# myshell-ai/OpenVoice

Measured on AMD Instinct MI355X. Metric: real_time_factor, higher is better.
Workload: dtype f32; 1 GPU; ToneColorConverter.convert path, 32 x 10 s @ 22.05 kHz per GPU (T=861 frames), fp32, calibrated random weights; batch_per_gpu=32, global_batch=32, parallelism=dp1 (utterance sharding, RCCL broadcast of src/tgt se)

## Files before the change

include/openvoice_amd.h:

```cpp
#ifndef OPENVOICE_AMD_H
#define OPENVOICE_AMD_H

#include <stddef.h>
#include <stdint.h>

#ifdef __cplusplus
extern "C" {
#endif

typedef void* ov_stream_t;

enum {
  OV_OK = 0,
  OV_E_BADARG = -1,
  OV_E_UNSUPPORTED = -2,
  OV_E_ALIGN = -3,
  OV_E_LAUNCH = -4
};

enum {
  OV_EPI_LINEAR = 0,
  OV_EPI_GATE = 1,
  OV_EPI_RESSKIP = 2,
  OV_EPI_COUPLE = 3,
  OV_EPI_POSTERIOR = 4,
  OV_EPI_CONVT = 5,
  OV_EPI_MAGNITUDE = 6
};

enum {
  OV_F_MASK_V = 1,
  OV_F_OUT2_INIT = 2,
  OV_F_CONVT_GROUPED = 4,
  OV_F_NO_XCD_MAP = 8
};

typedef struct ov_conv1d_params {
  const float* x;
  const float* w;
  const float* bias;
  const float* bias_b;
  float* out;
  const float* res;
  const float* add;
  float* out2;
  const float* mask;
  int64_t x_bstride;
  int64_t out_bstride;
  int64_t res_bstride;
  int64_t add_bstride;
  int64_t out2_bstride;
  int64_t bias_b_bstride;
  int64_t mask_bstride;
  int32_t B, Cin, L;
  int32_t x_ld;
  int32_t out_ld;
  int32_t M;
  int32_t Cout;
  int32_t K, dil;
  int32_t epi, flags, split, phase_s;
  int32_t tiles_per_wg;
  int32_t tile;
  int32_t loaders;
  int32_t chunk;
  float in_slope;
  float scale;
  const int32_t* col_limit;
  int32_t col_limit_scale;
  int32_t reserved0;
} ov_conv1d_params;


size_t ov_conv1d_pack_size(int Cout, int Cin, int K);
int ov_conv1d_pack_rows(int Cout);
int ov_conv1d_pack_f32(const float* w, int Cout, int Cin, int K, float* dst);


int ov_conv1d_f32(const ov_conv1d_params* p, ov_stream_t stream);

typedef struct ov_respair_params {
  const float* x;
  const float* w1;
  const float* b1;
  const float* w2;
  const float* b2;
  float* out;
  const float* add;
  int64_t x_bstride, out_bstride, add_bstride;
  int32_t B, C, L;
  int32_t ld;
  int32_t K, dil;
  int32_t nwg;
  float slope;
  float scale;
  unsigned long long* dbg;
  const int32_t* col_limit;
  int32_t col_limit_scale;
  int32_t reserved0;
} ov_respair_params;
int ov_resblock_pair_f32(const ov_respair_params* p, ov_stream_t stream);
int ov_resblock_pair_supported(int C, int K, int dil);

typedef struct ov_wn_layer_params {
  const float* x;
  float* out;
  float* skip;
  const float* w_in;
  const float* b_in;
  const float* cond;
  const float* w_rs;
  const float* b_rs;
  const float* mask;
  int64_t bstride;
  int64_t cond_bstride;
  int64_t mask_bstride;
  int32_t B, H, T;
  int32_t ld;
  int32_t K;
  int32_t first;
  int32_t last;
  int32_t width;
  int32_t ntile;
  int32_t row_split;
  unsigned long long* dbg;
  float* acts;
} ov_wn_layer_params;
int ov_wn_layer_f32(const ov_wn_layer_params* p, ov_stream_t stream);
int ov_wn_layer_supported(int H, int K);
size_t ov_wn_pack_size(int rows, int cin, int K);
int ov_wn_pack_f32(const float* w, int rows, int cin, int K, float* dst);
int ov_wn_layer_tile(int B, int T, int width);

int ov_wn_layer_wino_f32(const ov_wn_layer_params* p, ov_stream_t stream);
int ov_wn_layer_wino_tile(void);
size_t ov_wn_wino_pack_size(int rows, int cin, int K);
int ov_wn_wino_pack_f32(const float* w, int rows, int cin, int K, float* dst);

int ov_frame_hops_f32(const float* wave, float* hops, int B, int N, int hop, int pad, int U, int ld,
                      ov_stream_t stream);

int ov_frame_hops_windows_f32(const float* wave, int64_t n_samples, const int64_t* first_frame, int W, int hop, int pad,
                              int U, int ld, float* hops, ov_stream_t stream);
int ov_frame_hops_multi_f32(const float* pool, int64_t pool_len, const int64_t* records, int W, int hop, int pad, int U,
                            int ld, float* hops, ov_stream_t stream);
int ov_stitch_window_cores_f32(const float* o_hat, const int64_t* windows, int W, int Tw, int spf, float* out,
                               int64_t out_len, int64_t out_frame0, ov_stream_t stream);
int ov_carry_rows_f32(const int64_t* records, int n_records, const float* src_base, int64_t src_elems, float* dst_base,
                      int64_t dst_elems, ov_stream_t stream);
int ov_rows_f32_to_cl_bf16(const float* src, int64_t src_bs, int src_ld, uint16_t* dst, int B, int C, int L,
                           ov_stream_t stream);
int ov_cl_bf16_to_rows_f32(const uint16_t* src, float* dst, int64_t dst_bs, int dst_ld, int B, int C, int L,
                           ov_stream_t stream);

int ov_vad_frame_energy_f32(const float* pool, int64_t pool_len, const int64_t* records, int R, int H, int ldT,
                            float* energy, ov_stream_t stream);
int ov_vad_segments_i32(const float* energy, const int64_t* records, int R, int H, int ldT, float floor_lin,
                        float range_lin, int min_silence_frames, int min_speech_frames, int pad_frames, int32_t* mask,
                        int64_t* offsets, int64_t* n_active, ov_stream_t stream);
int ov_vad_compact_f32(const float* pool, int64_t pool_len, const int64_t* records, int R, int H, int ldT,
                       const int32_t* mask, const int64_t* offsets, const int64_t* out_bases, float* out,
                       int64_t out_len, ov_stream_t stream);

int ov_join_segments_f32(const float* src, int64_t src_elems, const int64_t* records, int R, float* dst,
                         int64_t dst_elems, int64_t max_span, ov_stream_t stream);

int ov_pack_groups_cl_bf16(const float* src, int64_t src_len, const int64_t* records, int n, int C, uint16_t* dst,
                           int64_t dst_len, ov_stream_t stream);
int ov_unpack_groups_f32(const float* src, int64_t src_len, const int64_t* records, int n, float* dst, int64_t dst_len,
                         ov_stream_t stream);

int ov_normal_philox_f32(const int64_t* records, int R, int C, float* dst, int64_t dst_elems, int64_t max_frames,
                         ov_stream_t stream);

int ov_polyphase_fir_f32(const float* x, const double* h, float* y, int64_t n_in, int64_t n_out, int P, int Q, int taps,
                         ov_stream_t stream);

int ov_polyphase_fir_rows_f32(const int64_t* records, int n_records, const float* src_base, int64_t src_elems,
                              const double* h_base, int64_t h_elems, float* dst_base, int64_t dst_elems, int64_t max_out,
                              ov_stream_t stream);

int ov_conv_post_tanh_f32(const float* x, const float* w, float* out, int B, int C, int L, int K,
                          float in_slope, ov_stream_t stream);
int ov_conv_post_tanh_limited_f32(const float* x, const float* w, float* out, int B, int C, int L, int K,
                                  float in_slope, const int32_t* col_limit, int col_limit_scale, ov_stream_t stream);
int ov_frame_limits_i32(const int64_t* lengths, int32_t* limits, int B, int T, int margin, ov_stream_t stream);

int ov_linear_f32(const float* x, const float* w, const float* bias, float* y, int B, int M, int Kdim,
                  ov_stream_t stream);

int ov_sequence_mask_f32(const int64_t* lengths, float* mask, int B, int T, int ld, ov_stream_t stream);
int ov_unpad_rows_f32(const float* src, float* dst, int rows, int T, int ld, ov_stream_t stream);


int ov_layernorm_freq_f32(const float* x, const float* gamma, const float* beta, float* y, int N, int F, int T,
                          float eps, ov_stream_t stream);

int ov_conv2d_s2_relu_f32(const float* x, const float* w, const float* bias, float* y, int N, int Cin, int Cout,
                          int Fi, int Ti, ov_stream_t stream);

int ov_gru_f32(const float* gi, const float* whh_t, const float* bhh, float* h_out, int N, int H, int T,
               ov_stream_t stream);


int ov_layernorm_freq_ragged_f32(const float* x, const float* gamma, const float* beta, const int32_t* lens, float* y,
                                 int N, int F, int ld, float eps, ov_stream_t stream);

int ov_conv2d_s2_relu_ragged_f32(const float* x, const float* w, const float* bias, const int32_t* lens_in, float* y,
                                 int N, int Cin, int Cout, int Fi, int ld_in, int ld_out, ov_stream_t stream);

int ov_gru_ragged_f32(const float* gi, const float* whh_t, const float* bhh, const int32_t* lens, float* h_out, int N,
                      int H, int ld, ov_stream_t stream);


int ov_embed_f32(const int64_t* tokens, const float* emb, const int64_t* lengths, float* out, int B, int T, int H,
                 int V, int ld, float scale, ov_stream_t stream);

enum {
  OV_LN_PRE_RELU = 1,
  OV_LN_POST_GELU = 2
};
int ov_layernorm_ch_f32(const float* x, const float* res, const float* gamma, const float* beta, const float* res2,
                        const float* mask, float* out, int B, int C, int T, int ld, float eps, int flags,
                        ov_stream_t stream);

int ov_rel_attention_f32(const float* q, const float* k, const float* v, const float* emb_k, const float* emb_v,
                         const float* mask, float* out, int64_t qkv_bstride, int64_t out_bstride, int B, int n_heads,
                         int dk, int T, int ld, int window, ov_stream_t stream);

int ov_dwconv1d_f32(const float* x, const float* w, const float* bias, const float* mask, float* out, int B, int C,
                    int T, int ld, int K, int dil, ov_stream_t stream);

int ov_expand1_f32(const float* x0, int64_t x0_bstride, const float* w, const float* bias, const float* g, float* out,
                   int B, int C, int T, int ld, ov_stream_t stream);

int ov_add_bias_mask_f32(const float* x, const float* bias_b, const float* mask, float* out, int B, int C, int T,
                         int ld, ov_stream_t stream);

int ov_rq_spline_inverse_f32(float* z, int64_t z_bstride, int c0, int c1, const float* h, int64_t h_bstride,
                             const float* mask, int B, int T, int ld, int num_bins, int filter_channels,
                             float tail_bound, ov_stream_t stream);

int ov_duration_f32(const float* z_sdp, int64_t z_bstride, float ea_m, float ea_logs, const float* dp,
                    int64_t dp_bstride, const float* mask, float* logw, int32_t* cum, int64_t* y_len, int B, int T,
                    int ld, float sdp_ratio, float length_scale, ov_stream_t stream);

int ov_expand_prior_f32(const float* m_tok, const float* logs_tok, int64_t tok_bstride, int ldx, const int32_t* cum,
                        const int64_t* x_len, const int64_t* y_len, const float* noise, int64_t noise_bstride, int ldn, float* z_p,
                        float* m_p, float* logs_p, float* attn, int B, int C, int Tx, int Ty, int ldy,
                        float noise_scale, ov_stream_t stream);

typedef struct ov_conv1d_bf16_params {
  const uint16_t* x;
  const uint16_t* w;
  const float* bias;
  uint16_t* out;
  const uint16_t* res;
  const uint16_t* add;
  int32_t B, L, Cin, Cout, K, dil;
  int32_t phase_s;
  int32_t bias_bstride;
  int32_t layout;
  float in_slope;
  float scale;
  float out_slope;
  unsigned long long* dbg;
} ov_conv1d_bf16_params;

size_t ov_conv1d_bf16_pack_size(int Cout, int Cin, int K);
int ov_conv1d_bf16_pack(const float* w, int Cout, int Cin, int K, uint16_t* dst);
int ov_conv1d_bf16cl(const ov_conv1d_bf16_params* p, ov_stream_t stream);
int ov_conv_post_tanh_bf16(const uint16_t* x, const float* w, float* out, int B, int C, int L, int K, float in_slope,
                           ov_stream_t stream);

typedef struct ov_respair_bf16_params {
  const uint16_t* x;
  const uint16_t* w1;
  const float* b1;
  const uint16_t* w2;
  const float* b2;
  uint16_t* out;
  const uint16_t* add;
  int32_t B, L, C, K, dil;
  int32_t nwg;
  float slope, scale;
  unsigned long long* dbg;
} ov_respair_bf16_params;
int ov_resblock_pair_bf16cl(const ov_respair_bf16_params* p, ov_stream_t stream);
int ov_resblock_pair_bf16_supported(int C, int K, int dil);

typedef struct ov_respair2_bf16_params {
  const uint16_t* x;
  const uint16_t* w1;
  const float* b1;
  const uint16_t* w2;
  const float* b2;
  uint16_t* out;
  const uint16_t* add;
  int32_t B, L, C, K, dil;
  int32_t nwg;
  float slope;
  float scale;
  float out_slope;
  int32_t exp_flags;
  unsigned long long* dbg;
} ov_respair2_bf16_params;
int ov_resblock_pair2_bf16cl(const ov_respair2_bf16_params* p, ov_stream_t stream);
int ov_conv1d_bf16_pack16(const float* w, int Cout, int Cin, int K, uint16_t* dst);
int ov_resblock_pair2_bf16_supported(int C, int K, int dil);

typedef struct ov_conv1d_split3_params {
  const uint16_t* x;
  const uint16_t* w;
  const float* bias;
  uint16_t* out;
  const uint16_t* res;
  int64_t x_plane, out_plane, res_plane;
  int32_t B, L, Cin, Cout, K, dil;
  int32_t nwg;
  int32_t products;
  float res_slope;
  float out_slope;
  float scale;
  int32_t col_limit_scale;
  unsigned long long* dbg;
  const int32_t* col_limit;
} ov_conv1d_split3_params;
int ov_conv1d_split3(const ov_conv1d_split3_params* p, ov_stream_t stream);
size_t ov_conv1d_split3_pack_size(int Cout, int Cin, int K);
int ov_conv1d_split3_pack(const float* w, int Cout, int Cin, int K, uint16_t* dst);
int ov_conv1d_split3_supported(int Cin, int Cout, int K, int dil);
int ov_split3_from_f32(const float* x, uint16_t* planes, int64_t plane_stride, int B, int C, int L, float slope,
                       ov_stream_t stream);
int ov_split3_to_f32(const uint16_t* a, const uint16_t* b, const uint16_t* c, int64_t plane_stride, float* out, int B,
                     int C, int L, float in_slope, float scale, ov_stream_t stream);

typedef struct ov_conv1d_wino_params {
  const float* x;
  const float* w;
  const float* bias;
  float* out;
  const float* res;
  const float* add;
  int64_t x_bstride, out_bstride, res_bstride, add_bstride;
  int32_t B, Cin, Cout, L;
  int32_t x_ld, out_ld;
  int32_t K, dil;
  int32_t nwg;
  int32_t frags;
  float in_slope;
  float scale;
  unsigned long long* dbg;
  const int32_t* col_limit;
  int32_t col_limit_scale;
  float out_slope;
} ov_conv1d_wino_params;
int ov_conv1d_wino_f32(const ov_conv1d_wino_params* p, ov_stream_t stream);
int ov_conv1d_wino_supported(int Cin, int Cout, int K, int dil);
int ov_conv1d_wino_chunk(int K, int Cout);
size_t ov_conv1d_wino_pack_size(int Cout, int Cin, int K);
int ov_conv1d_wino_pack_f32(const float* w, int Cout, int Cin, int K, float* dst);

int ov_version(void);
#define OV_ABI_VERSION 212
int ov_build_experiment(void);

#ifdef __cplusplus
}
#endif
#endif
```

openvoice_amd/_lib.py:

```python
import ctypes
import os

_HERE = os.path.dirname(os.path.abspath(__file__))
LIB_PATH = os.environ.get("OPENVOICE_AMD_LIB") or os.path.join(_HERE, "libopenvoice_amd.so")

OV_OK = 0
MIN_VERSION = 212
OV_ERRORS = {-1: "OV_E_BADARG", -2: "OV_E_UNSUPPORTED", -3: "OV_E_ALIGN", -4: "OV_E_LAUNCH"}

EPI_LINEAR, EPI_GATE, EPI_RESSKIP, EPI_COUPLE, EPI_POSTERIOR, EPI_CONVT, EPI_MAGNITUDE = range(7)
F_MASK_V = 1
F_OUT2_INIT = 2
F_CONVT_GROUPED = 4
F_NO_XCD_MAP = 8

_fp = ctypes.c_void_p
_i = ctypes.c_int
_i64 = ctypes.c_int64
LN_PRE_RELU, LN_POST_GELU = 1, 2


class ConvParams(ctypes.Structure):
    _fields_ = [
        ("x", _fp), ("w", _fp), ("bias", _fp), ("bias_b", _fp), ("out", _fp), ("res", _fp),
        ("add", _fp), ("out2", _fp), ("mask", _fp),
        ("x_bstride", ctypes.c_int64), ("out_bstride", ctypes.c_int64), ("res_bstride", ctypes.c_int64),
        ("add_bstride", ctypes.c_int64), ("out2_bstride", ctypes.c_int64), ("bias_b_bstride", ctypes.c_int64),
        ("mask_bstride", ctypes.c_int64),
        ("B", ctypes.c_int32), ("Cin", ctypes.c_int32), ("L", ctypes.c_int32),
        ("x_ld", ctypes.c_int32), ("out_ld", ctypes.c_int32), ("M", ctypes.c_int32),
        ("Cout", ctypes.c_int32), ("K", ctypes.c_int32), ("dil", ctypes.c_int32), ("epi", ctypes.c_int32),
        ("flags", ctypes.c_int32), ("split", ctypes.c_int32), ("phase_s", ctypes.c_int32),
        ("tiles_per_wg", ctypes.c_int32), ("tile", ctypes.c_int32), ("loaders", ctypes.c_int32),
        ("chunk", ctypes.c_int32),
        ("in_slope", ctypes.c_float), ("scale", ctypes.c_float),
        ("col_limit", _fp), ("col_limit_scale", ctypes.c_int32), ("reserved0", ctypes.c_int32),
    ]


class ConvBf16Params(ctypes.Structure):
    _fields_ = [("x", _fp), ("w", _fp), ("bias", _fp), ("out", _fp), ("res", _fp), ("add", _fp),
                ("B", ctypes.c_int32), ("L", ctypes.c_int32), ("Cin", ctypes.c_int32), ("Cout", ctypes.c_int32),
                ("K", ctypes.c_int32), ("dil", ctypes.c_int32), ("phase_s", ctypes.c_int32), ("bias_bstride", ctypes.c_int32), ("layout", ctypes.c_int32),
                ("in_slope", ctypes.c_float), ("scale", ctypes.c_float), ("out_slope", ctypes.c_float), ("dbg", _fp)]


class RespairParams(ctypes.Structure):
    _fields_ = [("x", _fp), ("w1", _fp), ("b1", _fp), ("w2", _fp), ("b2", _fp), ("out", _fp), ("add", _fp),
                ("x_bstride", ctypes.c_int64), ("out_bstride", ctypes.c_int64), ("add_bstride", ctypes.c_int64),
                ("B", ctypes.c_int32), ("C", ctypes.c_int32), ("L", ctypes.c_int32), ("ld", ctypes.c_int32),
                ("K", ctypes.c_int32), ("dil", ctypes.c_int32), ("nwg", ctypes.c_int32),
                ("slope", ctypes.c_float), ("scale", ctypes.c_float), ("dbg", _fp),
                ("col_limit", _fp), ("col_limit_scale", ctypes.c_int32), ("reserved0", ctypes.c_int32)]


class RespairBf16Params(ctypes.Structure):
    _fields_ = [("x", _fp), ("w1", _fp), ("b1", _fp), ("w2", _fp), ("b2", _fp), ("out", _fp), ("add", _fp),
                ("B", ctypes.c_int32), ("L", ctypes.c_int32), ("C", ctypes.c_int32), ("K", ctypes.c_int32),
                ("dil", ctypes.c_int32), ("nwg", ctypes.c_int32), ("slope", ctypes.c_float), ("scale", ctypes.c_float),
                ("dbg", _fp)]


class Respair2Bf16Params(ctypes.Structure):
    _fields_ = [("x", _fp), ("w1", _fp), ("b1", _fp), ("w2", _fp), ("b2", _fp), ("out", _fp), ("add", _fp),
                ("B", ctypes.c_int32), ("L", ctypes.c_int32), ("C", ctypes.c_int32), ("K", ctypes.c_int32),
                ("dil", ctypes.c_int32), ("nwg", ctypes.c_int32), ("slope", ctypes.c_float), ("scale", ctypes.c_float),
                ("out_slope", ctypes.c_float), ("exp_flags", ctypes.c_int32), ("dbg", _fp)]


class ConvSplit3Params(ctypes.Structure):
    _fields_ = [("x", _fp), ("w", _fp), ("bias", _fp), ("out", _fp), ("res", _fp),
                ("x_plane", ctypes.c_int64), ("out_plane", ctypes.c_int64), ("res_plane", ctypes.c_int64),
                ("B", ctypes.c_int32), ("L", ctypes.c_int32), ("Cin", ctypes.c_int32), ("Cout", ctypes.c_int32),
                ("K", ctypes.c_int32), ("dil", ctypes.c_int32), ("nwg", ctypes.c_int32), ("products", ctypes.c_int32),
                ("res_slope", ctypes.c_float), ("out_slope", ctypes.c_float), ("scale", ctypes.c_float),
                ("col_limit_scale", ctypes.c_int32), ("dbg", _fp), ("col_limit", _fp)]


class ConvWinoParams(ctypes.Structure):
    _fields_ = [("x", _fp), ("w", _fp), ("bias", _fp), ("out", _fp), ("res", _fp), ("add", _fp),
                ("x_bstride", ctypes.c_int64), ("out_bstride", ctypes.c_int64), ("res_bstride", ctypes.c_int64),
                ("add_bstride", ctypes.c_int64),
                ("B", ctypes.c_int32), ("Cin", ctypes.c_int32), ("Cout", ctypes.c_int32), ("L", ctypes.c_int32),
                ("x_ld", ctypes.c_int32), ("out_ld", ctypes.c_int32), ("K", ctypes.c_int32), ("dil", ctypes.c_int32),
                ("nwg", ctypes.c_int32), ("frags", ctypes.c_int32),
                ("in_slope", ctypes.c_float), ("scale", ctypes.c_float), ("dbg", _fp),
                ("col_limit", _fp), ("col_limit_scale", ctypes.c_int32), ("out_slope", ctypes.c_float)]


class WnLayerParams(ctypes.Structure):
    _fields_ = [("x", _fp), ("out", _fp), ("skip", _fp), ("w_in", _fp), ("b_in", _fp), ("cond", _fp), ("w_rs", _fp),
                ("b_rs", _fp), ("mask", _fp),
                ("bstride", ctypes.c_int64), ("cond_bstride", ctypes.c_int64), ("mask_bstride", ctypes.c_int64),
                ("B", ctypes.c_int32), ("H", ctypes.c_int32), ("T", ctypes.c_int32), ("ld", ctypes.c_int32),
                ("K", ctypes.c_int32), ("first", ctypes.c_int32), ("last", ctypes.c_int32), ("width", ctypes.c_int32),
                ("ntile", ctypes.c_int32), ("row_split", ctypes.c_int32), ("dbg", _fp), ("acts", _fp)]


SIGNATURES = {
    "ov_version": (ctypes.c_int, []),
    "ov_build_experiment": (ctypes.c_int, []),
    "ov_conv1d_pack_size": (ctypes.c_size_t, [ctypes.c_int, ctypes.c_int, ctypes.c_int]),
    "ov_conv1d_pack_rows": (ctypes.c_int, [ctypes.c_int]),
    "ov_conv1d_pack_f32": (ctypes.c_int, [_fp, ctypes.c_int, ctypes.c_int, ctypes.c_int, _fp]),
    "ov_conv1d_f32": (ctypes.c_int, [ctypes.POINTER(ConvParams), _fp]),
    "ov_resblock_pair_f32": (ctypes.c_int, [ctypes.POINTER(RespairParams), _fp]),
    "ov_resblock_pair_supported": (ctypes.c_int, [_i, _i, _i]),
    "ov_wn_layer_f32": (ctypes.c_int, [ctypes.POINTER(WnLayerParams), _fp]),
    "ov_wn_layer_supported": (ctypes.c_int, [_i, _i]),
    "ov_wn_pack_size": (ctypes.c_size_t, [_i, _i, _i]),
    "ov_wn_pack_f32": (ctypes.c_int, [_fp, _i, _i, _i, _fp]),
    "ov_wn_layer_tile": (ctypes.c_int, [_i, _i, _i]),
    "ov_wn_layer_wino_f32": (ctypes.c_int, [ctypes.POINTER(WnLayerParams), _fp]),
    "ov_wn_layer_wino_tile": (ctypes.c_int, []),
    "ov_wn_wino_pack_size": (ctypes.c_size_t, [_i, _i, _i]),
    "ov_wn_wino_pack_f32": (ctypes.c_int, [_fp, _i, _i, _i, _fp]),
    "ov_conv_post_tanh_f32": (ctypes.c_int, [_fp, _fp, _fp, ctypes.c_int, ctypes.c_int, ctypes.c_int,
                                             ctypes.c_int, ctypes.c_float, _fp]),
    "ov_conv_post_tanh_limited_f32": (ctypes.c_int, [_fp, _fp, _fp, ctypes.c_int, ctypes.c_int, ctypes.c_int,
                                                     ctypes.c_int, ctypes.c_float, _fp, ctypes.c_int, _fp]),
    "ov_frame_limits_i32": (ctypes.c_int, [_fp, _fp, _i, _i, _i, _fp]),
    "ov_linear_f32": (ctypes.c_int, [_fp, _fp, _fp, _fp, ctypes.c_int, ctypes.c_int, ctypes.c_int, _fp]),
    "ov_sequence_mask_f32": (ctypes.c_int, [_fp, _fp, ctypes.c_int, ctypes.c_int, ctypes.c_int, _fp]),
    "ov_unpad_rows_f32": (ctypes.c_int, [_fp, _fp, ctypes.c_int, ctypes.c_int, ctypes.c_int, _fp]),
    "ov_polyphase_fir_f32": (ctypes.c_int, [_fp, _fp, _fp, ctypes.c_int64, ctypes.c_int64, _i, _i, _i, _fp]),
    "ov_polyphase_fir_rows_f32": (ctypes.c_int, [_fp, _i, _fp, _i64, _fp, _i64, _fp, _i64, _i64, _fp]),
    "ov_layernorm_freq_f32": (ctypes.c_int, [_fp, _fp, _fp, _fp, ctypes.c_int, ctypes.c_int, ctypes.c_int,
                                             ctypes.c_float, _fp]),
    "ov_conv2d_s2_relu_f32": (ctypes.c_int, [_fp, _fp, _fp, _fp, ctypes.c_int, ctypes.c_int, ctypes.c_int,
                                             ctypes.c_int, ctypes.c_int, _fp]),
    "ov_gru_f32": (ctypes.c_int, [_fp, _fp, _fp, _fp, ctypes.c_int, ctypes.c_int, ctypes.c_int, _fp]),
    "ov_layernorm_freq_ragged_f32": (ctypes.c_int, [_fp, _fp, _fp, _fp, _fp, _i, _i, _i, ctypes.c_float, _fp]),
    "ov_conv2d_s2_relu_ragged_f32": (ctypes.c_int, [_fp, _fp, _fp, _fp, _fp, _i, _i, _i, _i, _i, _i, _fp]),
    "ov_gru_ragged_f32": (ctypes.c_int, [_fp, _fp, _fp, _fp, _fp, _i, _i, _i, _fp]),
    "ov_conv1d_bf16_pack_size": (ctypes.c_size_t, [_i, _i, _i]),
    "ov_conv1d_bf16_pack": (ctypes.c_int, [_fp, _i, _i, _i, _fp]),
    "ov_conv1d_bf16_pack16": (ctypes.c_int, [_fp, _i, _i, _i, _fp]),
    "ov_conv1d_bf16cl": (ctypes.c_int, [ctypes.POINTER(ConvBf16Params), _fp]),
    "ov_resblock_pair_bf16cl": (ctypes.c_int, [ctypes.POINTER(RespairBf16Params), _fp]),
    "ov_resblock_pair_bf16_supported": (ctypes.c_int, [_i, _i, _i]),
    "ov_resblock_pair2_bf16cl": (ctypes.c_int, [ctypes.POINTER(Respair2Bf16Params), _fp]),
    "ov_resblock_pair2_bf16_supported": (ctypes.c_int, [_i, _i, _i]),
    "ov_conv_post_tanh_bf16": (ctypes.c_int, [_fp, _fp, _fp, _i, _i, _i, _i, ctypes.c_float, _fp]),
    "ov_conv1d_split3": (ctypes.c_int, [ctypes.POINTER(ConvSplit3Params), _fp]),
    "ov_conv1d_split3_pack_size": (ctypes.c_size_t, [_i, _i, _i]),
    "ov_conv1d_split3_pack": (ctypes.c_int, [_fp, _i, _i, _i, _fp]),
    "ov_conv1d_split3_supported": (ctypes.c_int, [_i, _i, _i, _i]),
    "ov_split3_from_f32": (ctypes.c_int, [_fp, _fp, _i64, _i, _i, _i, ctypes.c_float, _fp]),
    "ov_split3_to_f32": (ctypes.c_int, [_fp, _fp, _fp, _i64, _fp, _i, _i, _i, ctypes.c_float, ctypes.c_float, _fp]),
    "ov_conv1d_wino_f32": (ctypes.c_int, [ctypes.POINTER(ConvWinoParams), _fp]),
    "ov_conv1d_wino_supported": (ctypes.c_int, [_i, _i, _i, _i]),
    "ov_conv1d_wino_chunk": (ctypes.c_int, [_i, _i]),
    "ov_conv1d_wino_pack_size": (ctypes.c_size_t, [_i, _i, _i]),
    "ov_conv1d_wino_pack_f32": (ctypes.c_int, [_fp, _i, _i, _i, _fp]),
    "ov_frame_hops_f32": (ctypes.c_int, [_fp, _fp, _i, _i, _i, _i, _i, _i, _fp]),
    "ov_frame_hops_windows_f32": (ctypes.c_int, [_fp, _i64, _fp, _i, _i, _i, _i, _i, _fp, _fp]),
    "ov_frame_hops_multi_f32": (ctypes.c_int, [_fp, _i64, _fp, _i, _i, _i, _i, _i, _fp, _fp]),
    "ov_stitch_window_cores_f32": (ctypes.c_int, [_fp, _fp, _i, _i, _i, _fp, _i64, _i64, _fp]),
    "ov_carry_rows_f32": (ctypes.c_int, [_fp, _i, _fp, _i64, _fp, _i64, _fp]),
    "ov_rows_f32_to_cl_bf16": (ctypes.c_int, [_fp, _i64, _i, _fp, _i, _i, _i, _fp]),
    "ov_cl_bf16_to_rows_f32": (ctypes.c_int, [_fp, _fp, _i64, _i, _i, _i, _i, _fp]),
    "ov_vad_frame_energy_f32": (ctypes.c_int, [_fp, _i64, _fp, _i, _i, _i, _fp, _fp]),
    "ov_vad_segments_i32": (ctypes.c_int, [_fp, _fp, _i, _i, _i, ctypes.c_float, ctypes.c_float, _i, _i, _i, _fp, _fp, _fp,
                                           _fp]),
    "ov_vad_compact_f32": (ctypes.c_int, [_fp, _i64, _fp, _i, _i, _i, _fp, _fp, _fp, _fp, _i64, _fp]),
    "ov_join_segments_f32": (ctypes.c_int, [_fp, _i64, _fp, _i, _fp, _i64, _i64, _fp]),
    "ov_pack_groups_cl_bf16": (ctypes.c_int, [_fp, _i64, _fp, _i, _i, _fp, _i64, _fp]),
    "ov_unpack_groups_f32": (ctypes.c_int, [_fp, _i64, _fp, _i, _fp, _i64, _fp]),
    "ov_normal_philox_f32": (ctypes.c_int, [_fp, _i, _i, _fp, _i64, _i64, _fp]),
    "ov_embed_f32": (ctypes.c_int, [_fp, _fp, _fp, _fp, _i, _i, _i, _i, _i, ctypes.c_float, _fp]),
    "ov_layernorm_ch_f32": (ctypes.c_int, [_fp, _fp, _fp, _fp, _fp, _fp, _fp, _i, _i, _i, _i, ctypes.c_float, _i, _fp]),
    "ov_rel_attention_f32": (ctypes.c_int, [_fp, _fp, _fp, _fp, _fp, _fp, _fp, _i64, _i64, _i, _i, _i, _i, _i, _i,
                                            _fp]),
    "ov_add_bias_mask_f32": (ctypes.c_int, [_fp, _fp, _fp, _fp, _i, _i, _i, _i, _fp]),
    "ov_dwconv1d_f32": (ctypes.c_int, [_fp, _fp, _fp, _fp, _fp, _i, _i, _i, _i, _i, _i, _fp]),
    "ov_expand1_f32": (ctypes.c_int, [_fp, _i64, _fp, _fp, _fp, _fp, _i, _i, _i, _i, _fp]),
    "ov_rq_spline_inverse_f32": (ctypes.c_int, [_fp, _i64, _i, _i, _fp, _i64, _fp, _i, _i, _i, _i, _i,
                                                ctypes.c_float, _fp]),
    "ov_duration_f32": (ctypes.c_int, [_fp, _i64, ctypes.c_float, ctypes.c_float, _fp, _i64, _fp, _fp, _fp, _fp,
                                       _i, _i, _i, ctypes.c_float, ctypes.c_float, _fp]),
    "ov_expand_prior_f32": (ctypes.c_int, [_fp, _fp, _i64, _i, _fp, _fp, _fp, _fp, _i64, _i, _fp, _fp, _fp, _fp,
                                           _i, _i, _i, _i, _i, ctypes.c_float, _fp]),
}

_lib = None


class OvError(RuntimeError):
    pass


GENERATORS = ("fp32", "bf16")


def check_generator(generator, optional=False):
    if generator is None and optional:
        return None
    if not isinstance(generator, str) or generator not in GENERATORS:
        raise OvError(f"generator must be 'fp32' or 'bf16'{' (or None)' if optional else ''}, got {generator!r}")
    return generator


def generator_kw(generator):
    return {} if generator is None else {"generator": generator}


def load():
    global _lib
    if _lib is None:
        if not os.path.exists(LIB_PATH):
            raise OvError(f"{LIB_PATH} not found: build the HIP extension first "
                          f"(python -c 'import __graft_entry__ as g; g.build()'); there is no CPU fallback")
        lib = ctypes.CDLL(LIB_PATH)
        lib.ov_version.restype, lib.ov_version.argtypes = ctypes.c_int, []
        if lib.ov_version() < MIN_VERSION:
            raise OvError(f"{LIB_PATH} is version {lib.ov_version()}, this package needs >= {MIN_VERSION}: rebuild it "
                          f"(make -C openvoice_amd/csrc)")
        for name, (restype, argtypes) in SIGNATURES.items():
            try:
                fn = getattr(lib, name)
            except AttributeError:
                raise OvError(f"{LIB_PATH} lacks {name}: it was built from older source, rebuild it "
                              f"(make -C openvoice_amd/csrc)") from None
            fn.restype = restype
            fn.argtypes = argtypes
        exp = lib.ov_build_experiment()
        if exp != 0 and os.environ.get("OPENVOICE_AMD_ALLOW_EXPERIMENT") != "1":
            raise OvError(f"{LIB_PATH} is a measurement build (OV_EXP={exp}: kernels with loads / barriers compiled "
                          f"out, results meaningless); rebuild with `make -C openvoice_amd/csrc clean all`")
        _lib = lib
    return _lib


def torch_op(name, *args):
    try:
        return getattr(torch_ops(), name)(*args)
    except RuntimeError as exc:
        if isinstance(exc, OvError):
            raise
        raise OvError(str(exc).split("\n")[0]) from None


def check(code, what):
    if code != OV_OK:
        raise OvError(f"{what} failed: {OV_ERRORS.get(code, code)}")


SHIM_PATH = os.path.join(_HERE, "libopenvoice_amd_torch.so")
_ops = None
VALUE_FUNCS = {"ov_version", "ov_build_experiment", "ov_conv1d_pack_size", "ov_conv1d_pack_rows", "ov_wn_pack_size",
               "ov_conv1d_bf16_pack_size", "ov_resblock_pair_supported", "ov_wn_layer_supported", "ov_wn_layer_tile",
               "ov_resblock_pair_bf16_supported", "ov_resblock_pair2_bf16_supported", "ov_conv1d_split3_pack_size",
               "ov_conv1d_split3_supported", "ov_conv1d_wino_supported", "ov_conv1d_wino_chunk", "ov_conv1d_wino_pack_size",
               "ov_wn_layer_wino_tile", "ov_wn_wino_pack_size"}


def binding():
    b = os.environ.get("OPENVOICE_AMD_BINDING", "ctypes" if os.environ.get("OPENVOICE_AMD_LIB") else "torch")
    if b not in ("torch", "ctypes"):
        raise OvError(f"OPENVOICE_AMD_BINDING={b!r}: expected 'torch' or 'ctypes'")
    return b


def use_torch_binding():
    return binding() == "torch"


def torch_ops():
    global _ops
    if _ops is None:
        import torch
        for path in (LIB_PATH, SHIM_PATH):
            if not os.path.exists(path):
                raise OvError(f"{path} not found: build the HIP extension first (python -c 'import __graft_entry__ "
                              f"as g; g.build()'); there is no CPU fallback (OPENVOICE_AMD_BINDING=ctypes needs only "
                              f"libopenvoice_amd.so)")
        torch.ops.load_library(SHIM_PATH)
        ops = torch.ops.openvoice_amd
        if ops.version() < MIN_VERSION:
            raise OvError(f"{LIB_PATH} is version {ops.version()}, this package needs >= {MIN_VERSION}: rebuild it "
                          f"(make -C openvoice_amd/csrc)")
        exp = ops.build_experiment()
        if exp != 0 and os.environ.get("OPENVOICE_AMD_ALLOW_EXPERIMENT") != "1":
            raise OvError(f"{LIB_PATH} is a measurement build (OV_EXP={exp}); rebuild with "
                          f"`make -C openvoice_amd/csrc clean all`")
        _ops = ops
    return _ops


def _flat_view(t, off):
    start = t.storage_offset() + off
    n = t.untyped_storage().nbytes() // t.element_size() - start
    return t.as_strided((n,), (1,), start)


def call(name, *args):
    if use_torch_binding():
        targs = [_flat_view(*a) if type(a) is tuple else a for a in args]
        try:
            return getattr(torch_ops(), name[3:])(*targs)
        except RuntimeError as exc:
            if isinstance(exc, OvError):
                raise
            raise OvError(str(exc).split("\n")[0]) from None
    import torch
    lib = load()
    fn = getattr(lib, name)
    cargs, dev = [], None
    for a in args:
        off = 0
        if type(a) is tuple:
            a, off = a
        if isinstance(a, torch.Tensor):
            if dev is None and a.is_cuda:
                dev = a.device
            a = ctypes.c_void_p(a.data_ptr() + off * a.element_size())
        cargs.append(a)
    if len(fn.argtypes) == len(cargs) + 1:
        if dev is None:
            raise OvError(f"{name}: no device tensor among the arguments")
        cargs.append(ctypes.c_void_p(torch.cuda.current_stream(dev).cuda_stream))
    rc = fn(*cargs)
    if name in VALUE_FUNCS:
        return rc
    check(rc, name)
```

openvoice_amd/csrc/conv1d_wino.h:

```cpp
#pragma once
#include <hip/hip_runtime.h>

#include <atomic>
#include <type_traits>

#include "conv1d_mfma.h"
#include "openvoice_amd.h"

namespace ovkw {

using ovk::f32x16;
using ovk::f32x2;
using ovk::f32x4;

__device__ __forceinline__ uint32_t lds_addr(const void* ptr) {
  return (uint32_t)(uintptr_t)(const __attribute__((address_space(3))) void*)ptr;
}

__device__ __forceinline__ void lds_barrier() { asm volatile("s_waitcnt lgkmcnt(0)\n\ts_barrier" ::: "memory"); }

template <int OFF>
__device__ __forceinline__ void lds_write_b32(uint32_t addr, float v) {
  static_assert(OFF >= 0 && OFF < 65536, "DS immediate offset");
  asm volatile("ds_write_b32 %0, %1 offset:%2" ::"v"(addr), "v"(v), "n"(OFF) : "memory");
}
template <int O0, int O1>
__device__ __forceinline__ void lds_write2st64_b32(uint32_t addr, float a, float b) {
  static_assert(O0 >= 0 && O0 < 256 && O1 >= 0 && O1 < 256, "DS write2st64 offsets are 8-bit, in units of 64 dwords");
  asm volatile("ds_write2st64_b32 %0, %1, %2 offset0:%3 offset1:%4" ::"v"(addr), "v"(a), "v"(b), "n"(O0), "n"(O1) : "memory");
}
template <int I, int N, class F>
__device__ __forceinline__ void static_for(F&& f) {
  if constexpr (I < N) {
    f(std::integral_constant<int, I>{});
    static_for<I + 1, N>(f);
  }
}

constexpr int REC = 256;

constexpr int wino_lead(int K) { return K == 7 ? 1 : 0; }
constexpr int wino_trail(int K) { return (K + 2) / 3 * 3 - K - wino_lead(K); }
constexpr bool wino_zero_product(int K, int g, int pt) {
  return (pt == 0 && g == 0 && wino_lead(K) >= 1) || (pt == 5 && g == (K + 2) / 3 - 1 && wino_trail(K) >= 1);
}
constexpr int wino_products(int K) {
  int n = 0;
  for (int g = 0; g < (K + 2) / 3; ++g)
    for (int pt = 0; pt < 6; ++pt) n += wino_zero_product(K, g, pt) ? 0 : 1;
  return n;
}
static_assert(wino_products(3) == 6 && wino_products(7) == 16 && wino_products(11) == 23, "executed products per tile");
constexpr int MAX_COUT = 512;

template <int K, int DIL, int NF>
struct GeoD {
  static constexpr int G = (K + 2) / 3;
  static constexpr int NT = 32 * NF;
  static constexpr int J = NT / DIL;
  static constexpr int NCOL = 4 * J * DIL;
  static constexpr int PADD = ((K - 1) / 2 + wino_lead(K)) * DIL;
  static constexpr int PADA = (PADD + 3) / 4 * 4;
  static constexpr int NV = 3 * (G - 1) + 6;
  static constexpr int RW = (PADA - PADD + DIL - 1 + DIL * (4 * (J - 1) + NV - 1) + 1 + 3) / 4 * 4;
  static_assert(DIL == 3 || DIL == 5, "dilated instances: 3 and 5");
};

template <int K>
struct Geo {
  static constexpr int G = (K + 2) / 3;
  static constexpr int PAD = (K - 1) / 2 + wino_lead(K);
  static constexpr int OFF0 = 8 - PAD;
  static constexpr int WSTART = OFF0 / 4 * 4;
  static constexpr int WLEN = OFF0 - WSTART + 3 * (G - 1) + 6;
  static constexpr int NB128 = (WLEN + 3) / 4;
  static_assert(PAD <= 8 && WSTART + 4 * NB128 <= 20, "input window exceeds the raw row (128 NF + 16 floats)");
};

__host__ __device__ inline size_t wino_pack_floats(int Cout, int Cin, int K, int CI) {
  const int G = (K + 2) / 3;
  return ((size_t)(Cout / 32) * (Cin / CI) * (CI * G / 4) * 3 + 3) * REC;
}

#ifndef OVW_EXP
#define OVW_EXP 0
#endif
#define OVW_MARK(q)                                                \
  if constexpr (DBG) {                                             \
    const unsigned long long now_ = __builtin_readcyclecounter(); \
    tph[q] += now_ - tlast;                                        \
    tlast = now_;                                                  \
  }

template <int K, int DIL, int CI, int NF, int MW, bool DBG>
__global__ __launch_bounds__(64 * (4 + 2 * NF), NF == 1 ? 3 : 2) void conv1d_wino_kernel(const ov_conv1d_wino_params p) {
  using Ge = Geo<K>;
  using Gd = GeoD<K, DIL == 1 ? 3 : DIL, NF>;
  constexpr int G = Ge::G, KR = CI * G, NSTEP = KR / 2, NPAIR = NSTEP / 2;
  constexpr int NB = 4 / MW;
  constexpr int NTS = 32 * NF;
  constexpr int NT = NTS * NB;
  constexpr int NCOLS = DIL == 1 ? 4 * NTS : Gd::NCOL;
  constexpr int NCOL = NCOLS * NB;
  constexpr int RW = (DIL == 1 ? NCOLS + 16 : Gd::RW) + (NB - 1) * NCOLS;
  static_assert(MW == 4 || ((MW == 2 || MW == 1) && NF == 2), "two- and one-row-fragment workgroups run two fragments per wave");
  constexpr int ORG = DIL == 1 ? 8 : Gd::PADA;
  constexpr int RW4 = RW / 4;
  constexpr int NHELP = 2 * NF;
  static_assert(DIL == 1 || NF == 2, "dilated instances run two fragments per wave");
  static_assert(KR % 4 == 0 && CI % 2 == 0, "k-rows in whole k-step pairs");
  constexpr int NPR = CI / 2;
  constexpr int NITEM = NPR * RW4;
  constexpr int RAWBUF = CI * RW;
  constexpr int VBUF = KR * NT * 6;
  __shared__ __attribute__((aligned(16))) float raw[2 * RAWBUF];
  __shared__ __attribute__((aligned(16))) float Vs[2 * VBUF];
  __shared__ __attribute__((aligned(16))) float bias_s[MAX_COUT];
  constexpr int OST = 256;
  __shared__ __attribute__((aligned(16))) float ostage[DIL == 1 ? 4 : 4 * 8 * OST];

  const int tid = threadIdx.x;
  const int lane = tid & 63;
  const int wave = __builtin_amdgcn_readfirstlane(tid >> 6);
  const int L = p.L;
  const int nchunks = p.Cin / CI;
  const int ntiles = (L + NCOL - 1) / NCOL;
  const int mblocks = p.Cout / (32 * MW);
  int total = ntiles * mblocks * p.B;
  __shared__ int lim_pref[ovk::LIMIT_MAX_BATCH + 1];
  const bool limited = p.col_limit != nullptr;
  if (limited) {
    if (wave == 0) {
      int carry = 0;
      for (int base = 0; base < p.B; base += 64) {
        const int bb = base + lane;
        int nb = 0;
        if (bb < p.B) {
          long long c = (long long)p.col_limit[bb] * p.col_limit_scale;
          c = c < 0 ? 0 : (c > L ? L : c);
          nb = ((int)c + NCOL - 1) / NCOL;
        }
        int sc = nb;
#pragma unroll
        for (int d = 1; d < 64; d <<= 1) {
          const int v = __shfl_up(sc, d, 64);
          if (lane >= d) sc += v;
        }
        if (bb < p.B) lim_pref[bb + 1] = carry + sc;
        carry += __shfl(sc, 63, 64);
      }
      if (lane == 0) lim_pref[0] = 0;
    }
    __syncthreads();
    total = __builtin_amdgcn_readfirstlane(lim_pref[p.B]) * mblocks;
  }
  auto decode = [&](int w, int& ub, int& utile, int& umblk) {
    const int g = w / mblocks;
    umblk = w - g * mblocks;
    if (!limited) {
      ub = g / ntiles;
      utile = g - ub * ntiles;
      return;
    }
    int lo = 0, hi = p.B;
    while (hi - lo > 1) {
      const int mid = (lo + hi) >> 1;
      if (__builtin_amdgcn_readfirstlane(lim_pref[mid]) <= g) lo = mid; else hi = mid;
    }
    ub = lo;
    utile = g - __builtin_amdgcn_readfirstlane(lim_pref[lo]);
  };
  int wid0 = blockIdx.x, wend = total, wstride = gridDim.x;
  if ((gridDim.x & 7u) == 0) {
    const int xcd = blockIdx.x & 7;
    const int lo = (int)(((long long)xcd * total) >> 3);
    wend = (int)(((long long)(xcd + 1) * total) >> 3);
    wid0 = lo + (int)(blockIdx.x >> 3);
    wstride = gridDim.x >> 3;
  }
  if (wid0 >= wend) return;
  const int nitems = (wend - wid0 + wstride - 1) / wstride;
  const int nstream = nitems * nchunks;
  for (int i = tid; i < p.Cout; i += 64 * (4 + NHELP)) bias_s[i] = p.bias[i];

  const bool is_helper = wave >= 4;
  if (is_helper) {
    __builtin_amdgcn_s_setprio(3);
    const float slope = p.in_slope;
    const uint32_t ldx = (uint32_t)p.x_ld;
    const int hl = (wave - 4) * 64 + lane;
    constexpr int NLOAD = (NITEM + 64 * NHELP - 1) / (64 * NHELP);
    f32x4 sa[2][NLOAD], sb[2][NLOAD];
    uint32_t sbyte[NLOAD];
    int scol[NLOAD];
    uint32_t hasbits = 0, okbits[2] = {0, 0};
    bool edge[2] = {false, false};
#pragma unroll
    for (int i = 0; i < NLOAD; ++i) {
      const int idx = i * (64 * NHELP) + hl;
      const int pr = idx / RW4, c4 = idx - pr * RW4;
      const bool has = idx < NITEM;
      hasbits |= (has ? 1u : 0u) << i;
      scol[i] = 4 * c4;
      sbyte[i] = has ? 4u * (2u * (uint32_t)pr * ldx + 4u * (uint32_t)c4) : 0u;
    }
    const uint32_t raw_lds = lds_addr(raw) + 32u * (uint32_t)hl;
    const uint32_t v_lds = lds_addr(Vs);
    int lwid = wid0, lchunk = 0, lpos = 0;
    int lb, ltile, lmblk;
    decode(lwid, lb, ltile, lmblk);

    auto issue_loads = [&](auto setc) {
      constexpr int S = decltype(setc)::value;
      const bool live = lpos < nstream;
      const int tb = ltile * NCOL - ORG;
      const float* __restrict__ xrow = p.x + (int64_t)lb * p.x_bstride + (int64_t)(lchunk * CI) * ldx;
      edge[S] = !(live && tb >= 0 && tb + RW <= L);
      if (!edge[S]) {
        const char* b0 = reinterpret_cast<const char*>(xrow + tb);
        const char* b1 = reinterpret_cast<const char*>(xrow + tb + ldx);
#pragma unroll
        for (int i = 0; i < NLOAD; ++i) {
          sa[S][i] = *reinterpret_cast<const f32x4*>(b0 + sbyte[i]);
          sb[S][i] = *reinterpret_cast<const f32x4*>(b1 + sbyte[i]);
        }
      } else {
        const char* b0 = reinterpret_cast<const char*>(xrow);
        const char* b1 = reinterpret_cast<const char*>(xrow + ldx);
        uint32_t okb = 0;
#pragma unroll
        for (int i = 0; i < NLOAD; ++i) {
          const int t = tb + scol[i];
          const bool ok = live && ((hasbits >> i) & 1u) && t >= 0 && t < L;
          const uint32_t off = ok ? sbyte[i] + 4u * (uint32_t)tb : 0u;
          okb |= (ok ? 1u : 0u) << i;
          sa[S][i] = *reinterpret_cast<const f32x4*>(b0 + off);
          sb[S][i] = *reinterpret_cast<const f32x4*>(b1 + off);
        }
        okbits[S] = okb;
      }
      ++lpos;
      if (++lchunk == nchunks) {
        lchunk = 0;
        lwid += wstride;
        if (lwid < wend) decode(lwid, lb, ltile, lmblk);
      }
    };
    auto act2 = [&](f32x2 v) {
      const f32x2 sv = v * f32x2{slope, slope};
      f32x2 r;
      asm("v_max_f32 %0, %1, %2" : "=v"(r[0]) : "v"(v[0]), "v"(sv[0]));
      asm("v_max_f32 %0, %1, %2" : "=v"(r[1]) : "v"(v[1]), "v"(sv[1]));
      return r;
    };
    auto write_raw = [&](int buf, auto setc) {
      constexpr int S = decltype(setc)::value;
      const uint32_t base = raw_lds + (uint32_t)buf * (RAWBUF * 4);
#pragma unroll
      for (int i = 0; i < NLOAD; ++i) {
        if ((hasbits >> i) & 1u) {
          f32x2 a01 = {sa[S][i][0], sa[S][i][1]}, a23 = {sa[S][i][2], sa[S][i][3]};
          f32x2 b01 = {sb[S][i][0], sb[S][i][1]}, b23 = {sb[S][i][2], sb[S][i][3]};
          if (slope != 1.f) {
            a01 = act2(a01); a23 = act2(a23); b01 = act2(b01); b23 = act2(b23);
          }
          if (edge[S] && !((okbits[S] >> i) & 1u)) a01 = a23 = b01 = b23 = f32x2{0.f, 0.f};
          const uint32_t ad = base + (uint32_t)i * (64 * NHELP * 32);
          asm volatile("ds_write2_b32 %0, %1, %2 offset1:1" ::"v"(ad), "v"(a01[0]), "v"(b01[0]) : "memory");
          asm volatile("ds_write2_b32 %0, %1, %2 offset0:2 offset1:3" ::"v"(ad), "v"(a01[1]), "v"(b01[1]) : "memory");
          asm volatile("ds_write2_b32 %0, %1, %2 offset0:4 offset1:5" ::"v"(ad), "v"(a23[0]), "v"(b23[0]) : "memory");
          asm volatile("ds_write2_b32 %0, %1, %2 offset0:6 offset1:7" ::"v"(ad), "v"(a23[1]), "v"(b23[1]) : "memory");
        }
      }
    };
    constexpr int ROUNDS = NPR * NT / (64 * NHELP);
    static_assert(NPR * NT % (64 * NHELP) == 0, "whole rounds of helper lanes");
    uint32_t tsrc[ROUNDS], vadr[2][ROUNDS][6];
    static_assert((NT * 24) % 256 == 0 && (CI * NT * 24) % 256 == 0, "channel / group record distances in 256-byte units");
#pragma unroll
    for (int r = 0; r < ROUNDS; ++r) {
      const int idx = r * (64 * NHELP) + hl;
      const int tile = idx & (NT - 1), pr = idx / NT;
      if constexpr (DIL == 1) {
        tsrc[r] = 8u * (uint32_t)(pr * RW + Ge::WSTART + 4 * tile);
      } else {
        const int sub = tile / NTS, tl = tile - sub * NTS;
        const int rc0 = tl / Gd::J, rc = rc0 < DIL ? rc0 : 0, jt = rc0 < DIL ? tl - rc0 * Gd::J : 0;
        tsrc[r] = 8u * (uint32_t)(pr * RW + (Gd::PADA - Gd::PADD) + sub * NCOLS + rc + 4 * DIL * jt);
      }
#pragma unroll
      for (int bf = 0; bf < 2; ++bf)
#pragma unroll
        for (int q = 0; q < 6; ++q) vadr[bf][r][q] = v_lds + (uint32_t)bf * (VBUF * 4) + 24u * (uint32_t)(2 * pr * NT + tile) + 4u * q;
    }
    auto transform = [&](auto bufc) {
      constexpr int buf = decltype(bufc)::value;
      const char* src = reinterpret_cast<const char*>(raw) + buf * (RAWBUF * 4);
#pragma unroll
      for (int r = 0; r < ROUNDS; ++r) {
        constexpr int NWIN = DIL == 1 ? 4 * Ge::NB128 : Gd::NV;
        f32x2 win[NWIN];
        if constexpr (DIL == 1) {
#pragma unroll
          for (int q = 0; q < 2 * Ge::NB128; ++q) {
            const f32x4 v = *reinterpret_cast<const f32x4*>(src + tsrc[r] + 16 * q);
            win[2 * q] = f32x2{v[0], v[1]};
            win[2 * q + 1] = f32x2{v[2], v[3]};
          }
        } else {
#pragma unroll
          for (int u = 0; u < Gd::NV; ++u) win[u] = *reinterpret_cast<const f32x2*>(src + tsrc[r] + 8 * DIL * u);
        }
        static_for<0, G>([&](auto gc) {
          constexpr int g = decltype(gc)::value;
          constexpr int o = (DIL == 1 ? Ge::OFF0 - Ge::WSTART : 0) + 3 * g;
          const f32x2 d0 = win[o], d1 = win[o + 1], d2 = win[o + 2], d3 = win[o + 3], d4 = win[o + 4], d5 = win[o + 5];
          const f32x2 c4 = {4.f, 4.f}, m4 = {-4.f, -4.f}, m5 = {-5.f, -5.f}, c2 = {2.f, 2.f}, m2 = {-2.f, -2.f};
          const f32x2 t1 = __builtin_elementwise_fma(m4, d2, d4), t2 = __builtin_elementwise_fma(m4, d1, d3);
          const f32x2 t3 = d4 - d2, t4 = d3 - d1;
          constexpr bool Z0 = wino_zero_product(K, g, 0), Z5 = wino_zero_product(K, g, 5);
          const f32x2 v1 = t1 + t2;
          const f32x2 v2 = t1 - t2;
          const f32x2 v3 = __builtin_elementwise_fma(c2, t4, t3);
          const f32x2 v4 = __builtin_elementwise_fma(m2, t4, t3);
          constexpr int OA = g * CI * NT * 24 / 256, OB = OA + NT * 24 / 256;
          constexpr int bf = buf;
          if constexpr (!Z0) {
            const f32x2 v0 = __builtin_elementwise_fma(c4, d0, __builtin_elementwise_fma(m5, d2, d4));
            lds_write2st64_b32<OA, OB>(vadr[bf][r][0], v0[0], v0[1]);
          }
          lds_write2st64_b32<OA, OB>(vadr[bf][r][1], v1[0], v1[1]);
          lds_write2st64_b32<OA, OB>(vadr[bf][r][2], v2[0], v2[1]);
          lds_write2st64_b32<OA, OB>(vadr[bf][r][3], v3[0], v3[1]);
          lds_write2st64_b32<OA, OB>(vadr[bf][r][4], v4[0], v4[1]);
          if constexpr (!Z5) {
            const f32x2 v5 = __builtin_elementwise_fma(c4, d1, __builtin_elementwise_fma(m5, d3, d5));
            lds_write2st64_b32<OA, OB>(vadr[bf][r][5], v5[0], v5[1]);
          }
        });
      }
    };
    auto hand_over = [&]() { lds_barrier(); };

    unsigned long long tph[8] = {0, 0, 0, 0, 0, 0, 0, 0};
    unsigned long long tlast = DBG ? __builtin_readcyclecounter() : 0ull;
    using S0 = std::integral_constant<int, 0>;
    using S1 = std::integral_constant<int, 1>;
    issue_loads(S0{});
    write_raw(0, S0{});
    issue_loads(S1{});
    hand_over();
    transform(std::integral_constant<int, 0>{});
    write_raw(1, S1{});
    issue_loads(S0{});
    hand_over();
    OVW_MARK(4)
    auto period = [&](int i, auto par) {
      constexpr int P = decltype(par)::value;
      if (OVW_EXP < 6) issue_loads(std::integral_constant<int, 1 - P>{});
      OVW_MARK(0)
      if (OVW_EXP != 2 && OVW_EXP < 6 && i + 1 < nstream) transform(std::integral_constant<int, 1 - P>{});
      OVW_MARK(1)
      if (OVW_EXP < 6) write_raw(P, par);
      OVW_MARK(2)
      if (OVW_EXP < 7) hand_over();
      OVW_MARK(3)
    };
    for (int i = 0; i < nstream; i += 2) {
      period(i, S0{});
      if (i + 1 < nstream) period(i + 1, S1{});
    }
    if constexpr (DBG) {
      if (lane == 0) {
        unsigned long long* d = p.dbg + ((size_t)blockIdx.x * 8 + wave) * 8;
        tph[7] = (unsigned long long)nstream;
#pragma unroll
        for (int q = 0; q < 8; ++q) d[q] = tph[q];
      }
    }
    return;
  }

  const int half = lane >> 5, n = lane & 31;
  const f32x4* __restrict__ wbase = reinterpret_cast<const f32x4*>(p.w);
  const uint32_t LD = (uint32_t)p.out_ld;
  int wid = wid0, b, tile, mblk;
  decode(wid, b, tile, mblk);
  const int wrow = MW == 4 ? wave : (MW == 2 ? (wave & 1) : 0), wsub = MW == 4 ? 0 : (MW == 2 ? (wave >> 1) : wave);
  int mtile = mblk * MW + wrow;
  uint32_t rec = (uint32_t)mtile * (uint32_t)nchunks * (uint32_t)(NPAIR * 3);
  f32x4 a_cur[3], a_nxt[3];
#pragma unroll
  for (int j = 0; j < 3; ++j) a_cur[j] = wbase[(size_t)(rec + j) * 64 + lane];
  const int voffB = (half * NT + wsub * NTS + n) * 6;

  __syncthreads();
  __syncthreads();
  unsigned long long tph[8] = {0, 0, 0, 0, 0, 0, 0, 0};
  unsigned long long tlast = DBG ? __builtin_readcyclecounter() : 0ull;
  int it = 0;
  while (true) {
    f32x16 acc[6][NF];
#pragma unroll
    for (int q = 0; q < 6; ++q)
#pragma unroll
      for (int f = 0; f < NF; ++f)
#pragma unroll
        for (int r = 0; r < 16; ++r) acc[q][f][r] = 0.f;
#pragma unroll
    for (int i = 0; i < 4; ++i) {
      const f32x4 bq = *reinterpret_cast<const f32x4*>(bias_s + mtile * 32 + 4 * half + 8 * i);
#pragma unroll
      for (int f = 0; f < NF; ++f) {
        acc[1][f][4 * i] = bq[0]; acc[1][f][4 * i + 1] = bq[1]; acc[1][f][4 * i + 2] = bq[2]; acc[1][f][4 * i + 3] = bq[3];
      }
    }

    OVW_MARK(3)
    f32x2 bq[NF][3];
#pragma unroll
    for (int f = 0; f < NF; ++f)
#pragma unroll
      for (int qq = 0; qq < 3; ++qq) bq[f][qq] = *reinterpret_cast<const f32x2*>(Vs + (it & 1) * VBUF + voffB + f * (32 * 6) + 2 * qq);
    for (int chunk = 0; chunk < nchunks; ++chunk, ++it) {
      const float* vb = Vs + (it & 1) * VBUF + voffB;
      const float* vbn = Vs + ((it + 1) & 1) * VBUF + voffB;
      const bool more_chunks = chunk + 1 < nchunks;
#pragma unroll
      for (int s = 0; s < NSTEP; ++s) {
        const int s2 = s & 1;
        if (s == NSTEP - 1) {
          OVW_MARK(0)
          if (OVW_EXP < 7) lds_barrier();
          OVW_MARK(1)
        }
        if (s2 == 0) {
          rec += 3;
#pragma unroll
          for (int j = 0; j < 3; ++j) a_nxt[j] = (OVW_EXP == 3 || OVW_EXP == 8) ? a_cur[j] : wbase[(size_t)(rec + j) * 64 + lane];
        }
#pragma unroll
        for (int qq = 0; qq < 3; ++qq) {
          __builtin_amdgcn_sched_barrier(0);
#pragma unroll
          for (int t = 0; t < 2; ++t) {
            const int q = 2 * qq + t, e = s2 * 6 + q;
            if (wino_zero_product(K, 2 * s / CI, q)) continue;
#pragma unroll
            for (int f = 0; f < NF; ++f) {
#if OVW_EXP == 1
              acc[q][f][0] += a_cur[e >> 2][e & 3] * bq[f][qq][t];
#else
              acc[q][f] = __builtin_amdgcn_mfma_f32_32x32x2f32(a_cur[e >> 2][e & 3], bq[f][qq][t], acc[q][f], 0, 0, 0);
#endif
            }
          }
          __builtin_amdgcn_sched_barrier(0);
          if (OVW_EXP != 5 && OVW_EXP != 8 && (s + 1 < NSTEP || more_chunks)) {
#pragma unroll
            for (int f = 0; f < NF; ++f)
              bq[f][qq] = *reinterpret_cast<const f32x2*>((s + 1 < NSTEP ? vb + (s + 1) * (2 * NT * 6) : vbn) + f * (32 * 6) + 2 * qq);
          }
        }
        if (s2 == 1) {
#pragma unroll
          for (int j = 0; j < 3; ++j) a_cur[j] = a_nxt[j];
        }
      }
    }

    const int nwid = wid + wstride;
    const bool more = nwid < wend;
    int nb = 0, ntile = 0, nmblk = 0;
    if (more) decode(nwid, nb, ntile, nmblk);
    const int nmtile = nmblk * MW + wrow;
    const int ob = b, otile = tile, omtile = mtile;
    if (more) {
      rec = (uint32_t)nmtile * (uint32_t)nchunks * (uint32_t)(NPAIR * 3);
#pragma unroll
      for (int j = 0; j < 3; ++j) a_cur[j] = wbase[(size_t)(rec + j) * 64 + lane];
      wid = nwid; b = nb; tile = ntile; mblk = nmblk; mtile = nmtile;
    }

    {
      const float scale = p.scale;
      const float oslope = p.out_slope;
      const bool act_out = oslope < 1.f;
      float* outb = p.out + (int64_t)ob * p.out_bstride;
      const float* resb = p.res ? p.res + (int64_t)ob * p.res_bstride : nullptr;
      const float* addb = p.add ? p.add + (int64_t)ob * p.add_bstride : nullptr;
      const uint32_t rbase = (uint32_t)omtile * 32u + 4u * (uint32_t)half;
      auto at4 = [&](int f, int r) {
        const float y0 = acc[0][f][r], y1 = acc[1][f][r], y2 = acc[2][f][r], y3 = acc[3][f][r], y4 = acc[4][f][r],
                    y5 = acc[5][f][r];
        const float s1 = y1 + y2, d1 = y1 - y2, s2 = y3 + y4, d2 = y3 - y4;
        f32x4 o;
        o[0] = (y0 + s1) + s2;
        o[1] = __builtin_fmaf(2.f, d2, d1);
        o[2] = __builtin_fmaf(4.f, s2, s1);
        o[3] = __builtin_fmaf(8.f, d2, d1) + y5;
        return o;
      };
      if constexpr (DIL == 1) {
        auto run = [&](auto has_res, auto has_add) {
          constexpr bool HR = decltype(has_res)::value, HA = decltype(has_add)::value;
          constexpr int NGRP = 16 * NF;
          uint32_t voff[NF];
          bool colok[NF];
#pragma unroll
          for (int f = 0; f < NF; ++f) {
            const uint32_t col = (uint32_t)otile * NCOL + (uint32_t)(wsub * NCOLS) + 128u * f + 4u * (uint32_t)n;
            colok[f] = col < (uint32_t)L;
            voff[f] = 4u * (uint32_t)half * LD + (colok[f] ? col : 0u);
          }
          const size_t mrow = (size_t)omtile * 32u;
          constexpr int DEPTH = (HR && HA) ? 4 : 8;
          f32x4 rv[HR ? DEPTH : 1], av[HA ? DEPTH : 1];
          auto load = [&](int g) {
            const int f = g / 16, r = g % 16;
            const size_t rowb = (mrow + (size_t)((r & 3) + 8 * (r >> 2))) * LD;
            if constexpr (HR) rv[g % DEPTH] = *reinterpret_cast<const f32x4*>(resb + rowb + voff[f]);
            if constexpr (HA) av[g % DEPTH] = *reinterpret_cast<const f32x4*>(addb + rowb + voff[f]);
          };
          if constexpr (HR || HA) {
#pragma unroll
            for (int g = 0; g < DEPTH - 1; ++g) load(g);
          }
#pragma unroll
          for (int g = 0; g < NGRP; ++g) {
            if constexpr (HR || HA) {
              if (g + DEPTH - 1 < NGRP) load(g + DEPTH - 1);
            }
            const int f = g / 16, r = g % 16;
            f32x4 o = at4(f, r);
            if constexpr (HR) o += rv[g % DEPTH];
            if constexpr (HA) o += av[g % DEPTH];
            o *= scale;
            if constexpr (!HR && !HA) {
              if (act_out) {
#pragma unroll
                for (int e = 0; e < 4; ++e) o[e] = ovk::lrelu(o[e], oslope);
              }
            }
            if (colok[f] && (OVW_EXP != 4 || o[0] == 12345.f))
              *reinterpret_cast<f32x4*>(outb + (mrow + (size_t)((r & 3) + 8 * (r >> 2))) * LD + voff[f]) = o;
          }
        };
        using T = std::true_type;
        using F = std::false_type;
        if (resb && addb) run(T{}, T{});
        else if (resb) run(T{}, F{});
        else if (addb) run(F{}, T{});
        else run(F{}, F{});
      } else {
        float* ost = ostage + wave * (8 * OST);
        const uint32_t c0 = (uint32_t)otile * NCOL + (uint32_t)(wsub * NCOLS);
        int cbase[NF];
#pragma unroll
        for (int f = 0; f < NF; ++f) {
          const int tl = 32 * f + n, rc0 = tl / Gd::J;
          cbase[f] = rc0 < DIL ? rc0 + 4 * DIL * (tl - rc0 * Gd::J) : -1;
        }
        const uint32_t col = c0 + 4u * (uint32_t)lane;
        const bool colok = 4 * lane < NCOLS && col < (uint32_t)L;
        const uint32_t ccol = colok ? col : 0u;
        auto run = [&](auto has_res, auto has_add) {
          constexpr bool HR = decltype(has_res)::value, HA = decltype(has_add)::value;
          constexpr int DEPTH = (HR && HA) ? 2 : 3;
          f32x4 rv[HR ? DEPTH : 1][2], av[HA ? DEPTH : 1][2];
          auto row0 = [&](int g) { return (uint32_t)omtile * 32u + 8u * (g / 4) + 2u * (g % 4); };
          auto load = [&](int g) {
#pragma unroll
            for (int j = 0; j < 2; ++j) {
              if constexpr (HR) rv[g % DEPTH][j] = *reinterpret_cast<const f32x4*>(resb + (size_t)(row0(g) + j) * LD + ccol);
              if constexpr (HA) av[g % DEPTH][j] = *reinterpret_cast<const f32x4*>(addb + (size_t)(row0(g) + j) * LD + ccol);
            }
          };
          if constexpr (HR || HA) {
#pragma unroll
            for (int g = 0; g < DEPTH - 1; ++g) load(g);
          }
#pragma unroll
          for (int rg = 0; rg < 4; ++rg) {
#pragma unroll
            for (int j = 0; j < 4; ++j)
#pragma unroll
              for (int f = 0; f < NF; ++f) {
                const f32x4 o = at4(f, 4 * rg + j);
                if (cbase[f] >= 0) {
                  float* od = ost + (4 * half + j) * OST + cbase[f];
                  od[0] = o[0]; od[DIL] = o[1]; od[2 * DIL] = o[2]; od[3 * DIL] = o[3];
                }
              }
#pragma unroll
            for (int q = 0; q < 4; ++q) {
              const int g = 4 * rg + q;
              if constexpr (HR || HA) {
                if (g + DEPTH - 1 < 16) load(g + DEPTH - 1);
              }
#pragma unroll
              for (int j = 0; j < 2; ++j) {
                f32x4 o = *reinterpret_cast<const f32x4*>(ost + (2 * q + j) * OST + 4 * lane);
                if constexpr (HR) o += rv[g % DEPTH][j];
                if constexpr (HA) o += av[g % DEPTH][j];
                o *= scale;
                if constexpr (!HR && !HA) {
                  if (act_out) {
#pragma unroll
                    for (int e = 0; e < 4; ++e) o[e] = ovk::lrelu(o[e], oslope);
                  }
                }
                if (colok) *reinterpret_cast<f32x4*>(outb + (size_t)(row0(g) + j) * LD + col) = o;
              }
            }
          }
        };
        using T = std::true_type;
        using F = std::false_type;
        if (resb && addb) run(T{}, T{});
        else if (resb) run(T{}, F{});
        else if (addb) run(F{}, T{});
        else run(F{}, F{});
      }
    }
    OVW_MARK(2)
    if (!more) break;
  }
  if constexpr (DBG) {
    if (lane == 0) {
      unsigned long long* d = p.dbg + ((size_t)blockIdx.x * 8 + wave) * 8;
      tph[7] = (unsigned long long)it;
#pragma unroll
      for (int q = 0; q < 8; ++q) d[q] = tph[q];
    }
  }
}

template <int K, int DIL, int CI, int NF, int MW, bool DBG>
int wino_launch(const ov_conv1d_wino_params* p, hipStream_t stream) {
  constexpr int NCOL = (DIL == 1 ? 128 * NF : GeoD<K, DIL == 1 ? 3 : DIL, NF>::NCOL) * (4 / MW), NHELP = 2 * NF;
  const int ntiles = (p->L + NCOL - 1) / NCOL;
  const long total = (long)ntiles * (p->Cout / (32 * MW)) * p->B;
  auto kernel = conv1d_wino_kernel<K, DIL, CI, NF, MW, DBG>;
  static std::atomic<int> slot_cache[ovk::OV_MAX_DEVICES];
  const int slots = ovk::resident_workgroups(reinterpret_cast<const void*>(kernel), 64 * (4 + NHELP), slot_cache);
  long nwg = p->nwg > 0 ? p->nwg : slots;
  if (nwg > total) nwg = total;
  if (nwg >= 8) nwg = (nwg + 7) / 8 * 8;
  hipLaunchKernelGGL(kernel, dim3((unsigned)nwg), dim3(64 * (4 + NHELP)), 0, stream, *p);
  return hipGetLastError() == hipSuccess ? OV_OK : OV_E_LAUNCH;
}

constexpr int wino_ci(int K, int mw = 4) {
  return mw == 1 ? (K == 11 ? 2 : 0) : K == 3 ? (mw == 4 ? 16 : 8) : (K == 7 || K == 11) ? (mw == 4 ? 8 : 4) : 0;
}
constexpr int wino_mw(int Cout) { return Cout % 128 == 0 ? 4 : (Cout % 64 == 0 ? 2 : (Cout % 32 == 0 ? 1 : 0)); }

int wino_dispatch_k3(const ov_conv1d_wino_params* p, int nf, hipStream_t stream);
int wino_dispatch_k7(const ov_conv1d_wino_params* p, int nf, hipStream_t stream);
int wino_dispatch_k11(const ov_conv1d_wino_params* p, int nf, hipStream_t stream);

#define OVW_DISPATCH_MW(KK, MWV)                                                                                        \
  {                                                                                                                      \
    constexpr int CI = ovkw::wino_ci(KK, MWV);                                                                           \
    if constexpr (MWV == 4) {                                                                                            \
      if (p->dil == 1 && nf == 1)                                                                                        \
        return dbg ? wino_launch<KK, 1, CI, 1, 4, true>(p, st) : wino_launch<KK, 1, CI, 1, 4, false>(p, st);              \
    }                                                                                                                    \
    if (p->dil == 1) return dbg ? wino_launch<KK, 1, CI, 2, MWV, true>(p, st) : wino_launch<KK, 1, CI, 2, MWV, false>(p, st); \
    if (p->dil == 3) return dbg ? wino_launch<KK, 3, CI, 2, MWV, true>(p, st) : wino_launch<KK, 3, CI, 2, MWV, false>(p, st); \
    if (p->dil == 5) return dbg ? wino_launch<KK, 5, CI, 2, MWV, true>(p, st) : wino_launch<KK, 5, CI, 2, MWV, false>(p, st); \
    return OV_E_UNSUPPORTED;                                                                                             \
  }
#define OVW_DEFINE_DISPATCH(KK)                                                                                          \
  int ovkw::wino_dispatch_k##KK(const ov_conv1d_wino_params* p, int nf, hipStream_t st) {                                \
    const bool dbg = p->dbg != nullptr;                                                                                  \
    if (ovkw::wino_mw(p->Cout) == 4) OVW_DISPATCH_MW(KK, 4)                                                              \
    if (nf != 2) return OV_E_UNSUPPORTED;                                                                                \
    if (ovkw::wino_mw(p->Cout) == 2) OVW_DISPATCH_MW(KK, 2)                                                              \
    if constexpr (ovkw::wino_ci(KK, 1) != 0) OVW_DISPATCH_MW(KK, 1)                                                      \
    return OV_E_UNSUPPORTED;                                                                                             \
  }

}
```

openvoice_amd/csrc/conv1d_wino.hip:

```cpp
#include "conv1d_wino.h"

#include <cstring>

using namespace ovkw;

namespace {

const double kG[6][3] = {{1.0 / 4, 0, 0},           {-1.0 / 6, -1.0 / 6, -1.0 / 6}, {-1.0 / 6, 1.0 / 6, -1.0 / 6},
                         {1.0 / 24, 1.0 / 12, 1.0 / 6}, {1.0 / 24, -1.0 / 12, 1.0 / 6},  {0, 0, 1}};

}

extern "C" {

int ov_conv1d_wino_chunk(int K, int Cout) { return Cout > 0 && wino_mw(Cout) ? wino_ci(K, wino_mw(Cout)) : 0; }

int ov_conv1d_wino_supported(int Cin, int Cout, int K, int dil) {
  const int ci = ov_conv1d_wino_chunk(K, Cout);
  if (ci == 0 || (dil != 1 && dil != 3 && dil != 5)) return 0;
  return (Cin > 0 && Cin % ci == 0 && Cout <= MAX_COUT) ? 1 : 0;
}

size_t ov_conv1d_wino_pack_size(int Cout, int Cin, int K) {
  const int ci = ov_conv1d_wino_chunk(K, Cout);
  if (ci == 0 || Cin <= 0 || Cin % ci != 0) return 0;
  return wino_pack_floats(Cout, Cin, K, ci);
}

int ov_conv1d_wino_pack_f32(const float* w, int Cout, int Cin, int K, float* dst) {
  const size_t nfl = ov_conv1d_wino_pack_size(Cout, Cin, K);
  if (!w || !dst || nfl == 0) return OV_E_BADARG;
  const int CI = ov_conv1d_wino_chunk(K, Cout), G = (K + 2) / 3, KR = CI * G, NPAIR = KR / 4, nchunks = Cin / CI;
  std::memset(dst, 0, nfl * sizeof(float));
  for (int mt = 0; mt < Cout / 32; ++mt)
    for (int c = 0; c < nchunks; ++c)
      for (int sp = 0; sp < NPAIR; ++sp)
        for (int lane = 0; lane < 64; ++lane)
          for (int e = 0; e < 12; ++e) {
            const int kstep = 2 * sp + e / 6, pt = e % 6;
            const int kk = 2 * kstep + (lane >> 5);
            const int g = kk / CI, ci = c * CI + kk % CI;
            const int co = 32 * mt + (lane & 31);
            double u = 0.0;
            for (int k = 0; k < 3; ++k) {
              const int tap = 3 * g + k - wino_lead(K);
              if (tap >= 0 && tap < K) u += kG[pt][k] * (double)w[((size_t)co * Cin + ci) * K + tap];
            }
            const size_t sub = (((size_t)mt * nchunks + c) * NPAIR + sp) * 3 + e / 4;
            dst[sub * REC + (size_t)lane * 4 + e % 4] = (float)u;
          }
  return OV_OK;
}

int ov_conv1d_wino_f32(const ov_conv1d_wino_params* pin, ov_stream_t stream) {
  if (!pin) return OV_E_BADARG;
  ov_conv1d_wino_params q = *pin;
  if (!q.x || !q.w || !q.bias || !q.out) return OV_E_BADARG;
  if (q.B <= 0 || q.L <= 0 || q.nwg < 0) return OV_E_BADARG;
  if (q.col_limit && (q.col_limit_scale <= 0 || (reinterpret_cast<uintptr_t>(q.col_limit) & 3))) return OV_E_BADARG;
  if (q.col_limit && q.B > ovk::LIMIT_MAX_BATCH) q.col_limit = nullptr;
  if (q.x_ld == 0) q.x_ld = q.L;
  if (q.out_ld == 0) q.out_ld = q.L;
  if (q.x_ld < q.L || q.out_ld < q.L) return OV_E_BADARG;
  if (!ov_conv1d_wino_supported(q.Cin, q.Cout, q.K, q.dil)) return OV_E_UNSUPPORTED;
  if (!(q.in_slope > 0.f && q.in_slope <= 1.f)) return OV_E_UNSUPPORTED;
  if (q.out_slope == 0.f) q.out_slope = 1.f;
  if (!(q.out_slope > 0.f && q.out_slope <= 1.f)) return OV_E_UNSUPPORTED;
  if (q.out_slope != 1.f && (q.res || q.add)) return OV_E_UNSUPPORTED;
  if (q.out == q.x) return OV_E_BADARG;
  auto mis = [](const void* ptr) { return (reinterpret_cast<uintptr_t>(ptr) & 15) != 0; };
  if (mis(q.x) || mis(q.w) || mis(q.out) || (q.res && mis(q.res)) || (q.add && mis(q.add)) || (q.L & 3) || (q.x_ld & 3) ||
      (q.out_ld & 3) || (q.x_bstride & 3) || (q.out_bstride & 3) || (q.res && (q.res_bstride & 3)) ||
      (q.add && (q.add_bstride & 3)))
    return OV_E_ALIGN;
  if ((int64_t)q.Cin * q.x_ld >= (1LL << 31) || (int64_t)q.Cout * q.out_ld >= (1LL << 31)) return OV_E_BADARG;
  if ((int64_t)ov_conv1d_wino_chunk(q.K, q.Cout) * q.x_ld >= (1LL << 30)) return OV_E_BADARG;
  if (q.B > 1 && (q.x_bstride < (int64_t)q.Cin * q.x_ld || q.out_bstride < (int64_t)q.Cout * q.out_ld ||
                  (q.res && q.res_bstride < (int64_t)q.Cout * q.out_ld) || (q.add && q.add_bstride < (int64_t)q.Cout * q.out_ld)))
    return OV_E_BADARG;
  hipStream_t st = static_cast<hipStream_t>(stream);
  if (q.frags < 0 || q.frags > 2) return OV_E_BADARG;
  const int nf = q.frags ? q.frags : 2;
  if (q.dil != 1 && nf != 2) return OV_E_UNSUPPORTED;
  switch (q.K) {
    case 3: return wino_dispatch_k3(&q, nf, st);
    case 7: return wino_dispatch_k7(&q, nf, st);
    case 11: return wino_dispatch_k11(&q, nf, st);
  }
  return OV_E_UNSUPPORTED;
}

}
```

openvoice_amd/csrc/torch_shim.cpp:

```cpp
#include <ATen/ATen.h>
#include <ATen/hip/impl/HIPGuardImplMasqueradingAsCUDA.h>
#include <c10/hip/HIPStream.h>
#include <torch/library.h>

#include <string>
#include <type_traits>

#include "openvoice_amd.h"

namespace {

const char* ov_strerror(int rc) {
  switch (rc) {
    case OV_E_BADARG: return "OV_E_BADARG";
    case OV_E_UNSUPPORTED: return "OV_E_UNSUPPORTED";
    case OV_E_ALIGN: return "OV_E_ALIGN";
    case OV_E_LAUNCH: return "OV_E_LAUNCH";
    default: return "unknown error";
  }
}

using OptTensor = c10::optional<at::Tensor>;

struct Ctx {
  const char* name;
  bool host;
  bool have_dev = false;
  c10::Device dev{c10::kCPU};
  void see(const at::Tensor& t, int index) {
    if (host) {
      TORCH_CHECK(t.device().is_cpu(), name, ": argument ", index, " must be a HOST (CPU) tensor");
      return;
    }
    TORCH_CHECK(t.is_cuda(), name, ": argument ", index, " must be on a ROCm device (there is no CPU path)");
    if (!have_dev) { dev = t.device(); have_dev = true; }
    TORCH_CHECK(t.device() == dev, name, ": argument ", index, " is on ", t.device(), ", expected ", dev);
  }
  ov_stream_t stream() const {
    TORCH_CHECK(have_dev, name, ": no device tensor among the arguments");
    return static_cast<ov_stream_t>(c10::hip::getCurrentHIPStream(dev.index()).stream());
  }
};

struct DeviceScope {
  c10::hip::OptionalHIPGuardMasqueradingAsCUDA guard;
  explicit DeviceScope(const Ctx& c) { if (c.have_dev) guard.set_device(c.dev); }
};

template <typename E> bool dtype_ok(at::ScalarType s);
template <> bool dtype_ok<float>(at::ScalarType s) { return s == at::kFloat; }
template <> bool dtype_ok<double>(at::ScalarType s) { return s == at::kDouble; }
template <> bool dtype_ok<int64_t>(at::ScalarType s) { return s == at::kLong; }
template <> bool dtype_ok<int32_t>(at::ScalarType s) { return s == at::kInt; }
template <> bool dtype_ok<uint16_t>(at::ScalarType s) { return s == at::kBFloat16 || s == at::kShort || s == at::kUInt16; }
template <> bool dtype_ok<unsigned long long>(at::ScalarType s) { return s == at::kLong || s == at::kUInt64; }
template <typename E> const char* dtype_name();
template <> const char* dtype_name<float>() { return "float32"; }
template <> const char* dtype_name<double>() { return "float64"; }
template <> const char* dtype_name<int64_t>() { return "int64"; }
template <> const char* dtype_name<int32_t>() { return "int32"; }
template <> const char* dtype_name<uint16_t>() { return "bfloat16 (or int16 bit patterns)"; }
template <> const char* dtype_name<unsigned long long>() { return "int64 (tick counters)"; }

template <typename E> E* tensor_ptr(const OptTensor& t, Ctx& c, int index) {
  if (!t.has_value() || !t->defined()) return nullptr;
  c.see(*t, index);
  TORCH_CHECK(dtype_ok<E>(t->scalar_type()), c.name, ": argument ", index, " must be ", dtype_name<E>(), ", got ",
              t->scalar_type());
  return static_cast<E*>(t->data_ptr());
}

template <typename C, typename = void> struct Arg;
template <typename E> struct Arg<const E*> {
  using torch_t = const OptTensor&;
  static std::string schema(int i) { return "Tensor? a" + std::to_string(i); }
  static const E* get(const OptTensor& t, Ctx& c, int i) { return tensor_ptr<E>(t, c, i); }
};
template <typename E> struct Arg<E*, std::enable_if_t<!std::is_const<E>::value>> {
  using torch_t = const OptTensor&;
  static std::string schema(int i) { return "Tensor(a" + std::to_string(i) + "!)? a" + std::to_string(i); }
  static E* get(const OptTensor& t, Ctx& c, int i) { return tensor_ptr<E>(t, c, i); }
};
template <> struct Arg<int> {
  using torch_t = int64_t;
  static std::string schema(int i) { return "int a" + std::to_string(i); }
  static int get(int64_t v, Ctx& c, int i) {
    TORCH_CHECK(v >= INT32_MIN && v <= INT32_MAX, c.name, ": argument ", i, " does not fit a 32-bit int");
    return static_cast<int>(v);
  }
};
template <> struct Arg<int64_t> {
  using torch_t = int64_t;
  static std::string schema(int i) { return "int a" + std::to_string(i); }
  static int64_t get(int64_t v, Ctx&, int) { return v; }
};
template <> struct Arg<float> {
  using torch_t = double;
  static std::string schema(int i) { return "float a" + std::to_string(i); }
  static float get(double v, Ctx&, int) { return static_cast<float>(v); }
};

template <typename... T> struct List {};
template <typename L, typename... Acc> struct DropLast;
template <typename T, typename... Acc> struct DropLast<List<T>, Acc...> { using type = List<Acc...>; using last = T; };
template <typename T, typename U, typename... R, typename... Acc>
struct DropLast<List<T, U, R...>, Acc...> : DropLast<List<U, R...>, Acc..., T> {};

template <typename... C> std::string schema_of(const char* name, bool returns_int) {
  std::string s = std::string(name) + "(";
  int i = 0;
  bool first = true;
  ((s += (first ? "" : ", ") + Arg<C>::schema(i++), first = false), ...);
  return s + (returns_int ? ") -> int" : ") -> ()");
}

template <int Kind, typename R, typename L> struct Wrap;
template <typename R, typename... C> struct Wrap<0, R, List<C...>> {
  template <R (*Fn)(C..., ov_stream_t)> struct On {
    static inline const char* name = "";
    static void call(typename Arg<C>::torch_t... a) {
      Ctx c{name, false};
      int i = 0;
      std::tuple<C...> v{Arg<C>::get(a, c, i++)...};
      DeviceScope scope(c);
      const int rc = std::apply([&](C... x) { return Fn(x..., c.stream()); }, v);
      TORCH_CHECK(rc == OV_OK, "ov_", name, " failed: ", ov_strerror(rc));
    }
    static void def(torch::Library& m, const char* n) { name = n; m.def(schema_of<C...>(n, false).c_str(), &call); }
  };
};
template <typename R, typename... C> struct Wrap<1, R, List<C...>> {
  template <R (*Fn)(C...)> struct On {
    static inline const char* name = "";
    static void call(typename Arg<C>::torch_t... a) {
      Ctx c{name, true};
      int i = 0;
      std::tuple<C...> v{Arg<C>::get(a, c, i++)...};
      const int rc = std::apply(Fn, v);
      TORCH_CHECK(rc == OV_OK, "ov_", name, " failed: ", ov_strerror(rc));
    }
    static void def(torch::Library& m, const char* n) { name = n; m.def(schema_of<C...>(n, false).c_str(), &call); }
  };
};
template <typename R, typename... C> struct Wrap<2, R, List<C...>> {
  template <R (*Fn)(C...)> struct On {
    static inline const char* name = "";
    static int64_t call(typename Arg<C>::torch_t... a) {
      Ctx c{name, true};
      int i = 0;
      std::tuple<C...> v{Arg<C>::get(a, c, i++)...};
      return static_cast<int64_t>(std::apply(Fn, v));
    }
    static void def(torch::Library& m, const char* n) { name = n; m.def(schema_of<C...>(n, true).c_str(), &call); }
  };
};

template <typename F> struct Sig;
template <typename R, typename... C> struct Sig<R (*)(C...)> { using ret = R; using args = List<C...>; };

template <auto Fn> void bind_device(torch::Library& m, const char* name) {
  using S = Sig<decltype(Fn)>;
  using D = DropLast<typename S::args>;
  static_assert(std::is_same<typename D::last, ov_stream_t>::value, "device entry points end with the stream");
  Wrap<0, typename S::ret, typename D::type>::template On<Fn>::def(m, name);
}
template <auto Fn> void bind_host(torch::Library& m, const char* name) {
  using S = Sig<decltype(Fn)>;
  Wrap<1, typename S::ret, typename S::args>::template On<Fn>::def(m, name);
}
template <auto Fn> void bind_value(torch::Library& m, const char* name) {
  using S = Sig<decltype(Fn)>;
  Wrap<2, typename S::ret, typename S::args>::template On<Fn>::def(m, name);
}

template <typename E> E* sptr(const OptTensor& t, Ctx& c, int index, int64_t off = 0) {
  E* p = tensor_ptr<E>(t, c, index);
  return p ? p + off : nullptr;
}
void finish(int rc, const char* what) { TORCH_CHECK(rc == OV_OK, what, " failed: ", ov_strerror(rc)); }

void conv1d_f32(const OptTensor& x, const OptTensor& w, const OptTensor& bias, const OptTensor& out, const OptTensor& res,
                const OptTensor& add, const OptTensor& out2, const OptTensor& mask, const OptTensor& bias_b,
                const OptTensor& col_limit, at::IntArrayRef ip, at::ArrayRef<double> fp) {
  TORCH_CHECK(ip.size() == 29 && fp.size() == 2, "openvoice_amd::conv1d_f32: 29 integer and 2 float parameters");
  Ctx c{"conv1d_f32", false};
  ov_conv1d_params p{};
  p.x = sptr<float>(x, c, 0, ip[24]);
  p.w = sptr<float>(w, c, 1);
  p.bias = sptr<float>(bias, c, 2);
  p.out = sptr<float>(out, c, 3, ip[25]);
  p.res = sptr<float>(res, c, 4, ip[26]);
  p.add = sptr<float>(add, c, 5);
  p.out2 = sptr<float>(out2, c, 6);
  p.mask = sptr<float>(mask, c, 7);
  p.bias_b = sptr<float>(bias_b, c, 8, ip[27]);
  p.col_limit = sptr<int32_t>(col_limit, c, 9);
  p.col_limit_scale = (int32_t)ip[28];
  p.B = (int32_t)ip[0]; p.Cin = (int32_t)ip[1]; p.L = (int32_t)ip[2]; p.x_ld = (int32_t)ip[3]; p.out_ld = (int32_t)ip[4];
  p.M = (int32_t)ip[5]; p.Cout = (int32_t)ip[6]; p.K = (int32_t)ip[7]; p.dil = (int32_t)ip[8]; p.epi = (int32_t)ip[9];
  p.flags = (int32_t)ip[10]; p.split = (int32_t)ip[11]; p.phase_s = (int32_t)ip[12]; p.tiles_per_wg = (int32_t)ip[13];
  p.tile = (int32_t)ip[14]; p.loaders = (int32_t)ip[15]; p.chunk = (int32_t)ip[16];
  p.x_bstride = ip[17]; p.out_bstride = ip[18]; p.res_bstride = ip[19]; p.add_bstride = ip[20];
  p.out2_bstride = ip[21]; p.bias_b_bstride = ip[22]; p.mask_bstride = ip[23];
  p.in_slope = (float)fp[0]; p.scale = (float)fp[1];
  DeviceScope scope(c);
  finish(ov_conv1d_f32(&p, c.stream()), "ov_conv1d_f32");
}

void resblock_pair_f32(const OptTensor& x, const OptTensor& w1, const OptTensor& b1, const OptTensor& w2,
                       const OptTensor& b2, const OptTensor& out, const OptTensor& add, const OptTensor& dbg,
                       const OptTensor& col_limit, at::IntArrayRef ip, at::ArrayRef<double> fp) {
  TORCH_CHECK(ip.size() == 11 && fp.size() == 2, "openvoice_amd::resblock_pair_f32: 11 integer and 2 float parameters");
  Ctx c{"resblock_pair_f32", false};
  ov_respair_params p{};
  p.x = sptr<float>(x, c, 0); p.w1 = sptr<float>(w1, c, 1); p.b1 = sptr<float>(b1, c, 2);
  p.w2 = sptr<float>(w2, c, 3); p.b2 = sptr<float>(b2, c, 4); p.out = sptr<float>(out, c, 5);
  p.add = sptr<float>(add, c, 6);
  p.dbg = sptr<unsigned long long>(dbg, c, 7);
  p.col_limit = sptr<int32_t>(col_limit, c, 8);
  p.B = (int32_t)ip[0]; p.C = (int32_t)ip[1]; p.L = (int32_t)ip[2]; p.ld = (int32_t)ip[3]; p.K = (int32_t)ip[4];
  p.dil = (int32_t)ip[5]; p.nwg = (int32_t)ip[6];
  p.x_bstride = ip[7]; p.out_bstride = ip[8]; p.add_bstride = ip[9]; p.col_limit_scale = (int32_t)ip[10];
  p.slope = (float)fp[0]; p.scale = (float)fp[1];
  DeviceScope scope(c);
  finish(ov_resblock_pair_f32(&p, c.stream()), "ov_resblock_pair_f32");
}

template <int (*FN)(const ov_wn_layer_params*, ov_stream_t)>
void wn_layer_any(const char* op, const char* entry, const OptTensor& x, const OptTensor& out, const OptTensor& skip,
                  const OptTensor& w_in, const OptTensor& b_in, const OptTensor& cond, const OptTensor& w_rs,
                  const OptTensor& b_rs, const OptTensor& mask, const OptTensor& dbg, const OptTensor& acts,
                  at::IntArrayRef ip) {
  TORCH_CHECK(ip.size() == 13, "openvoice_amd::", op, ": 13 integer parameters");
  Ctx c{op, false};
  ov_wn_layer_params p{};
  p.x = sptr<float>(x, c, 0); p.out = sptr<float>(out, c, 1); p.skip = sptr<float>(skip, c, 2);
  p.w_in = sptr<float>(w_in, c, 3); p.b_in = sptr<float>(b_in, c, 4); p.cond = sptr<float>(cond, c, 5, ip[11]);
  p.w_rs = sptr<float>(w_rs, c, 6); p.b_rs = sptr<float>(b_rs, c, 7); p.mask = sptr<float>(mask, c, 8);
  p.dbg = sptr<unsigned long long>(dbg, c, 9);
  p.acts = sptr<float>(acts, c, 10);
  p.B = (int32_t)ip[0]; p.H = (int32_t)ip[1]; p.T = (int32_t)ip[2]; p.ld = (int32_t)ip[3]; p.K = (int32_t)ip[4];
  p.first = (int32_t)ip[5]; p.last = (int32_t)ip[6]; p.width = (int32_t)ip[7];
  p.bstride = ip[8]; p.cond_bstride = ip[9]; p.mask_bstride = ip[10]; p.row_split = (int32_t)ip[12];
  DeviceScope scope(c);
  finish(FN(&p, c.stream()), entry);
}
void wn_layer_f32(const OptTensor& x, const OptTensor& out, const OptTensor& skip, const OptTensor& w_in,
                  const OptTensor& b_in, const OptTensor& cond, const OptTensor& w_rs, const OptTensor& b_rs,
                  const OptTensor& mask, const OptTensor& dbg, const OptTensor& acts, at::IntArrayRef ip) {
  wn_layer_any<&ov_wn_layer_f32>("wn_layer_f32", "ov_wn_layer_f32", x, out, skip, w_in, b_in, cond, w_rs, b_rs, mask, dbg, acts, ip);
}
void wn_layer_wino_f32(const OptTensor& x, const OptTensor& out, const OptTensor& skip, const OptTensor& w_in,
                       const OptTensor& b_in, const OptTensor& cond, const OptTensor& w_rs, const OptTensor& b_rs,
                       const OptTensor& mask, const OptTensor& dbg, const OptTensor& acts, at::IntArrayRef ip) {
  wn_layer_any<&ov_wn_layer_wino_f32>("wn_layer_wino_f32", "ov_wn_layer_wino_f32", x, out, skip, w_in, b_in, cond, w_rs, b_rs, mask, dbg,
                                      acts, ip);
}

void conv1d_bf16cl(const OptTensor& x, const OptTensor& w, const OptTensor& bias, const OptTensor& out,
                   const OptTensor& res, const OptTensor& add, const OptTensor& dbg, at::IntArrayRef ip,
                   at::ArrayRef<double> fp) {
  TORCH_CHECK(ip.size() == 9 && fp.size() == 3, "openvoice_amd::conv1d_bf16cl: 9 integer and 3 float parameters");
  Ctx c{"conv1d_bf16cl", false};
  ov_conv1d_bf16_params p{};
  p.x = sptr<uint16_t>(x, c, 0); p.w = sptr<uint16_t>(w, c, 1); p.bias = sptr<float>(bias, c, 2);
  p.out = sptr<uint16_t>(out, c, 3); p.res = sptr<uint16_t>(res, c, 4); p.add = sptr<uint16_t>(add, c, 5);
  p.dbg = sptr<unsigned long long>(dbg, c, 6);
  p.B = (int32_t)ip[0]; p.L = (int32_t)ip[1]; p.Cin = (int32_t)ip[2]; p.Cout = (int32_t)ip[3]; p.K = (int32_t)ip[4];
  p.dil = (int32_t)ip[5]; p.phase_s = (int32_t)ip[6]; p.bias_bstride = (int32_t)ip[7]; p.layout = (int32_t)ip[8];
  p.in_slope = (float)fp[0]; p.scale = (float)fp[1]; p.out_slope = (float)fp[2];
  DeviceScope scope(c);
  finish(ov_conv1d_bf16cl(&p, c.stream()), "ov_conv1d_bf16cl");
}

void resblock_pair_bf16cl(const OptTensor& x, const OptTensor& w1, const OptTensor& b1, const OptTensor& w2,
                          const OptTensor& b2, const OptTensor& out, const OptTensor& add, const OptTensor& dbg,
                          at::IntArrayRef ip, at::ArrayRef<double> fp) {
  TORCH_CHECK(ip.size() == 6 && fp.size() == 2, "openvoice_amd::resblock_pair_bf16cl: 6 integer and 2 float parameters");
  Ctx c{"resblock_pair_bf16cl", false};
  ov_respair_bf16_params p{};
  p.x = sptr<uint16_t>(x, c, 0); p.w1 = sptr<uint16_t>(w1, c, 1); p.b1 = sptr<float>(b1, c, 2);
  p.w2 = sptr<uint16_t>(w2, c, 3); p.b2 = sptr<float>(b2, c, 4); p.out = sptr<uint16_t>(out, c, 5);
  p.add = sptr<uint16_t>(add, c, 6);
  p.dbg = sptr<unsigned long long>(dbg, c, 7);
  p.B = (int32_t)ip[0]; p.L = (int32_t)ip[1]; p.C = (int32_t)ip[2]; p.K = (int32_t)ip[3]; p.dil = (int32_t)ip[4];
  p.nwg = (int32_t)ip[5];
  p.slope = (float)fp[0]; p.scale = (float)fp[1];
  DeviceScope scope(c);
  finish(ov_resblock_pair_bf16cl(&p, c.stream()), "ov_resblock_pair_bf16cl");
}

void resblock_pair2_bf16cl(const OptTensor& x, const OptTensor& w1, const OptTensor& b1, const OptTensor& w2,
                           const OptTensor& b2, const OptTensor& out, const OptTensor& add, const OptTensor& dbg,
                           at::IntArrayRef ip, at::ArrayRef<double> fp) {
  TORCH_CHECK(ip.size() == 7 && fp.size() == 3, "openvoice_amd::resblock_pair2_bf16cl: 7 integer and 3 float parameters");
  Ctx c{"resblock_pair2_bf16cl", false};
  ov_respair2_bf16_params p{};
  p.x = sptr<uint16_t>(x, c, 0); p.w1 = sptr<uint16_t>(w1, c, 1); p.b1 = sptr<float>(b1, c, 2);
  p.w2 = sptr<uint16_t>(w2, c, 3); p.b2 = sptr<float>(b2, c, 4); p.out = sptr<uint16_t>(out, c, 5);
  p.add = sptr<uint16_t>(add, c, 6);
  p.dbg = sptr<unsigned long long>(dbg, c, 7);
  p.B = (int32_t)ip[0]; p.L = (int32_t)ip[1]; p.C = (int32_t)ip[2]; p.K = (int32_t)ip[3]; p.dil = (int32_t)ip[4];
  p.nwg = (int32_t)ip[5]; p.exp_flags = (int32_t)ip[6];
  p.slope = (float)fp[0]; p.scale = (float)fp[1]; p.out_slope = (float)fp[2];
  DeviceScope scope(c);
  finish(ov_resblock_pair2_bf16cl(&p, c.stream()), "ov_resblock_pair2_bf16cl");
}

void conv1d_split3(const OptTensor& x, const OptTensor& w, const OptTensor& bias, const OptTensor& out, const OptTensor& res,
                   const OptTensor& dbg, const OptTensor& col_limit, at::IntArrayRef ip, at::ArrayRef<double> fp) {
  TORCH_CHECK(ip.size() == 12 && fp.size() == 3, "openvoice_amd::conv1d_split3: 12 integer and 3 float parameters");
  Ctx c{"conv1d_split3", false};
  ov_conv1d_split3_params p{};
  p.x = sptr<uint16_t>(x, c, 0); p.w = sptr<uint16_t>(w, c, 1); p.bias = sptr<float>(bias, c, 2);
  p.out = sptr<uint16_t>(out, c, 3); p.res = sptr<uint16_t>(res, c, 4);
  p.dbg = sptr<unsigned long long>(dbg, c, 5);
  p.col_limit = sptr<int32_t>(col_limit, c, 6);
  p.B = (int32_t)ip[0]; p.L = (int32_t)ip[1]; p.Cin = (int32_t)ip[2]; p.Cout = (int32_t)ip[3]; p.K = (int32_t)ip[4];
  p.dil = (int32_t)ip[5]; p.nwg = (int32_t)ip[6]; p.products = (int32_t)ip[7];
  p.x_plane = ip[8]; p.out_plane = ip[9]; p.res_plane = ip[10]; p.col_limit_scale = (int32_t)ip[11];
  p.res_slope = (float)fp[0]; p.out_slope = (float)fp[1]; p.scale = (float)fp[2];
  DeviceScope scope(c);
  finish(ov_conv1d_split3(&p, c.stream()), "ov_conv1d_split3");
}

void conv1d_wino_f32(const OptTensor& x, const OptTensor& w, const OptTensor& bias, const OptTensor& out, const OptTensor& res,
                     const OptTensor& add, const OptTensor& dbg, const OptTensor& col_limit, at::IntArrayRef ip,
                     at::ArrayRef<double> fp) {
  TORCH_CHECK(ip.size() == 15 && fp.size() == 3, "openvoice_amd::conv1d_wino_f32: 15 integer and 3 float parameters");
  Ctx c{"conv1d_wino_f32", false};
  ov_conv1d_wino_params p{};
  p.x = sptr<float>(x, c, 0); p.w = sptr<float>(w, c, 1); p.bias = sptr<float>(bias, c, 2);
  p.out = sptr<float>(out, c, 3); p.res = sptr<float>(res, c, 4); p.add = sptr<float>(add, c, 5);
  p.dbg = sptr<unsigned long long>(dbg, c, 6);
  p.col_limit = sptr<int32_t>(col_limit, c, 7); p.col_limit_scale = (int32_t)ip[14];
  p.B = (int32_t)ip[0]; p.Cin = (int32_t)ip[1]; p.Cout = (int32_t)ip[2]; p.L = (int32_t)ip[3];
  p.x_ld = (int32_t)ip[4]; p.out_ld = (int32_t)ip[5]; p.K = (int32_t)ip[6]; p.dil = (int32_t)ip[7]; p.nwg = (int32_t)ip[8];
  p.x_bstride = ip[9]; p.out_bstride = ip[10]; p.res_bstride = ip[11]; p.add_bstride = ip[12]; p.frags = (int32_t)ip[13];
  p.in_slope = (float)fp[0]; p.scale = (float)fp[1]; p.out_slope = (float)fp[2];
  DeviceScope scope(c);
  finish(ov_conv1d_wino_f32(&p, c.stream()), "ov_conv1d_wino_f32");
}

}

TORCH_LIBRARY(openvoice_amd, m) {
  m.def("conv1d_f32(Tensor? x, Tensor? w, Tensor? bias, Tensor(a!)? out, Tensor? res, Tensor? add, Tensor(b!)? out2, "
        "Tensor? mask, Tensor? bias_b, Tensor? col_limit, int[] ip, float[] fp) -> ()", &conv1d_f32);
  m.def("resblock_pair_f32(Tensor? x, Tensor? w1, Tensor? b1, Tensor? w2, Tensor? b2, Tensor(a!)? out, Tensor? add, "
        "Tensor(b!)? dbg, Tensor? col_limit, int[] ip, float[] fp) -> ()", &resblock_pair_f32);
  m.def("wn_layer_f32(Tensor? x, Tensor(a!)? out, Tensor(b!)? skip, Tensor? w_in, Tensor? b_in, Tensor? cond, Tensor? w_rs, "
        "Tensor? b_rs, Tensor? mask, Tensor(c!)? dbg, Tensor(d!)? acts, int[] ip) -> ()", &wn_layer_f32);
  m.def("wn_layer_wino_f32(Tensor? x, Tensor(a!)? out, Tensor(b!)? skip, Tensor? w_in, Tensor? b_in, Tensor? cond, Tensor? w_rs, "
        "Tensor? b_rs, Tensor? mask, Tensor(c!)? dbg, Tensor(d!)? acts, int[] ip) -> ()", &wn_layer_wino_f32);
  m.def("conv1d_bf16cl(Tensor? x, Tensor? w, Tensor? bias, Tensor(a!)? out, Tensor? res, Tensor? add, Tensor(b!)? dbg, "
        "int[] ip, float[] fp) -> ()", &conv1d_bf16cl);
  m.def("resblock_pair_bf16cl(Tensor? x, Tensor? w1, Tensor? b1, Tensor? w2, Tensor? b2, Tensor(a!)? out, Tensor? add, "
        "Tensor(b!)? dbg, int[] ip, float[] fp) -> ()", &resblock_pair_bf16cl);
  m.def("resblock_pair2_bf16cl(Tensor? x, Tensor? w1, Tensor? b1, Tensor? w2, Tensor? b2, Tensor(a!)? out, Tensor? add, "
        "Tensor(b!)? dbg, int[] ip, float[] fp) -> ()", &resblock_pair2_bf16cl);
  m.def("conv1d_split3(Tensor? x, Tensor? w, Tensor? bias, Tensor(a!)? out, Tensor? res, Tensor(b!)? dbg, "
        "Tensor? col_limit, int[] ip, float[] fp) -> ()", &conv1d_split3);
  m.def("conv1d_wino_f32(Tensor? x, Tensor? w, Tensor? bias, Tensor(a!)? out, Tensor? res, Tensor? add, Tensor(b!)? dbg, "
        "Tensor? col_limit, int[] ip, float[] fp) -> ()",
        &conv1d_wino_f32);
  bind_device<&ov_frame_hops_f32>(m, "frame_hops_f32");
  bind_device<&ov_frame_hops_windows_f32>(m, "frame_hops_windows_f32");
  bind_device<&ov_frame_hops_multi_f32>(m, "frame_hops_multi_f32");
  bind_device<&ov_carry_rows_f32>(m, "carry_rows_f32");
  bind_device<&ov_rows_f32_to_cl_bf16>(m, "rows_f32_to_cl_bf16");
  bind_device<&ov_cl_bf16_to_rows_f32>(m, "cl_bf16_to_rows_f32");
  bind_device<&ov_vad_frame_energy_f32>(m, "vad_frame_energy_f32");
  bind_device<&ov_vad_segments_i32>(m, "vad_segments_i32");
  bind_device<&ov_vad_compact_f32>(m, "vad_compact_f32");
  bind_device<&ov_join_segments_f32>(m, "join_segments_f32");
  bind_device<&ov_pack_groups_cl_bf16>(m, "pack_groups_cl_bf16");
  bind_device<&ov_unpack_groups_f32>(m, "unpack_groups_f32");
  bind_device<&ov_normal_philox_f32>(m, "normal_philox_f32");
  bind_device<&ov_stitch_window_cores_f32>(m, "stitch_window_cores_f32");
  bind_device<&ov_conv_post_tanh_f32>(m, "conv_post_tanh_f32");
  bind_device<&ov_conv_post_tanh_limited_f32>(m, "conv_post_tanh_limited_f32");
  bind_device<&ov_frame_limits_i32>(m, "frame_limits_i32");
  bind_device<&ov_linear_f32>(m, "linear_f32");
  bind_device<&ov_sequence_mask_f32>(m, "sequence_mask_f32");
  bind_device<&ov_unpad_rows_f32>(m, "unpad_rows_f32");
  bind_device<&ov_polyphase_fir_f32>(m, "polyphase_fir_f32");
  bind_device<&ov_polyphase_fir_rows_f32>(m, "polyphase_fir_rows_f32");
  bind_device<&ov_layernorm_freq_f32>(m, "layernorm_freq_f32");
  bind_device<&ov_conv2d_s2_relu_f32>(m, "conv2d_s2_relu_f32");
  bind_device<&ov_gru_f32>(m, "gru_f32");
  bind_device<&ov_layernorm_freq_ragged_f32>(m, "layernorm_freq_ragged_f32");
  bind_device<&ov_conv2d_s2_relu_ragged_f32>(m, "conv2d_s2_relu_ragged_f32");
  bind_device<&ov_gru_ragged_f32>(m, "gru_ragged_f32");
  bind_device<&ov_embed_f32>(m, "embed_f32");
  bind_device<&ov_layernorm_ch_f32>(m, "layernorm_ch_f32");
  bind_device<&ov_rel_attention_f32>(m, "rel_attention_f32");
  bind_device<&ov_dwconv1d_f32>(m, "dwconv1d_f32");
  bind_device<&ov_expand1_f32>(m, "expand1_f32");
  bind_device<&ov_add_bias_mask_f32>(m, "add_bias_mask_f32");
  bind_device<&ov_rq_spline_inverse_f32>(m, "rq_spline_inverse_f32");
  bind_device<&ov_duration_f32>(m, "duration_f32");
  bind_device<&ov_expand_prior_f32>(m, "expand_prior_f32");
  bind_device<&ov_conv_post_tanh_bf16>(m, "conv_post_tanh_bf16");
  bind_device<&ov_split3_from_f32>(m, "split3_from_f32");
  bind_device<&ov_split3_to_f32>(m, "split3_to_f32");
  bind_host<&ov_conv1d_pack_f32>(m, "conv1d_pack_f32");
  bind_host<&ov_wn_pack_f32>(m, "wn_pack_f32");
  bind_host<&ov_wn_wino_pack_f32>(m, "wn_wino_pack_f32");
  bind_value<&ov_wn_wino_pack_size>(m, "wn_wino_pack_size");
  bind_value<&ov_wn_layer_wino_tile>(m, "wn_layer_wino_tile");
  bind_host<&ov_conv1d_bf16_pack>(m, "conv1d_bf16_pack");
  bind_host<&ov_conv1d_bf16_pack16>(m, "conv1d_bf16_pack16");
  bind_host<&ov_conv1d_split3_pack>(m, "conv1d_split3_pack");
  bind_value<&ov_conv1d_split3_pack_size>(m, "conv1d_split3_pack_size");
  bind_value<&ov_conv1d_split3_supported>(m, "conv1d_split3_supported");
  bind_host<&ov_conv1d_wino_pack_f32>(m, "conv1d_wino_pack_f32");
  bind_value<&ov_conv1d_wino_pack_size>(m, "conv1d_wino_pack_size");
  bind_value<&ov_conv1d_wino_supported>(m, "conv1d_wino_supported");
  bind_value<&ov_conv1d_wino_chunk>(m, "conv1d_wino_chunk");
  bind_value<&ov_conv1d_pack_size>(m, "conv1d_pack_size");
  bind_value<&ov_conv1d_pack_rows>(m, "conv1d_pack_rows");
  bind_value<&ov_wn_pack_size>(m, "wn_pack_size");
  bind_value<&ov_conv1d_bf16_pack_size>(m, "conv1d_bf16_pack_size");
  bind_value<&ov_resblock_pair_supported>(m, "resblock_pair_supported");
  bind_value<&ov_wn_layer_supported>(m, "wn_layer_supported");
  bind_value<&ov_wn_layer_tile>(m, "wn_layer_tile");
  bind_value<&ov_resblock_pair_bf16_supported>(m, "resblock_pair_bf16_supported");
  bind_value<&ov_resblock_pair2_bf16_supported>(m, "resblock_pair2_bf16_supported");
  bind_value<&ov_version>(m, "version");
  bind_value<&ov_build_experiment>(m, "build_experiment");
}
```

openvoice_amd/engine.py:

```python
import ctypes
import os

import torch

from . import _lib
from . import noise as noise_mod
from ._lib import (ConvParams, EPI_CONVT, EPI_COUPLE, EPI_GATE, EPI_LINEAR, EPI_POSTERIOR, EPI_RESSKIP,
                   F_CONVT_GROUPED, F_MASK_V, F_OUT2_INIT)
from .generator import (FINAL_LRELU_SLOPE, GENERATOR_MARGIN, LRELU_SLOPE, conv_transpose_as_conv,
                        generator_margin_frames, generator_stages, resblock_convs, samples_per_frame, scratch_per_frame)
from .params import ENC_Q_LAYERS, FLOW_LAYERS, N_FLOWS, REF_ENC_FILTERS, REF_ENC_GRU, effective_weight

LIMIT_MAX_BATCH = 256


SUPPORTED_RESBLOCK_KERNELS = (3, 7, 11)
SUPPORTED_RESBLOCK_DILATIONS = (1, 3, 5)


def validate_config(cfg):
    def bad(field, value, why):
        raise _lib.OvError(f"config field {field!r} = {value!r} is not supported by the MI355X kernels: {why}")

    rb = str(cfg.get("resblock", "1"))
    if rb != "1":
        bad("resblock", cfg.get("resblock"), "only ResBlock1 ('1') is built (ResBlock2 is not; reference "
            "openvoice/models.py:242, modules.py:312-357)")
    kernels, dils = list(cfg["resblock_kernel_sizes"]), [list(d) for d in cfg["resblock_dilation_sizes"]]
    if len(kernels) != len(dils) or not kernels:
        bad("resblock_dilation_sizes", cfg["resblock_dilation_sizes"], f"one dilation list per entry of "
            f"resblock_kernel_sizes ({len(kernels)}) is required")
    for k in kernels:
        if k not in SUPPORTED_RESBLOCK_KERNELS:
            bad("resblock_kernel_sizes", kernels, f"kernel size {k} has no conv instance (built: "
                f"{SUPPORTED_RESBLOCK_KERNELS})")
    for d in dils:
        for v in d:
            if v not in SUPPORTED_RESBLOCK_DILATIONS:
                bad("resblock_dilation_sizes", dils, f"dilation {v} has no conv instance (built: "
                    f"{SUPPORTED_RESBLOCK_DILATIONS})")
    rates, uk = list(cfg["upsample_rates"]), list(cfg["upsample_kernel_sizes"])
    if len(rates) != len(uk) or not rates:
        bad("upsample_kernel_sizes", uk, f"one kernel size per entry of upsample_rates ({len(rates)}) is required")
    for (i, cin, ch, u, *_), k in zip(generator_stages(cfg), uk):
        if k != 2 * u:
            bad("upsample_kernel_sizes", uk, f"stage {i}: the transposed conv is built as a 3-tap phase conv, which needs "
                f"kernel == 2 * stride (got kernel {k}, stride {u})")
        if u <= 0 or 32 % u != 0:
            bad("upsample_rates", rates, f"stage {i}: stride {u} must divide 32 (phases are interleaved inside one "
                f"32-row fragment)")
        if cin % 2 != 0 or ch % 32 != 0:
            bad("upsample_initial_channel", cfg["upsample_initial_channel"], f"stage {i} would have {ch} channels; "
                f"every stage needs a multiple of 32 (whole MFMA fragments)")
    if cfg["hidden_channels"] % 32 != 0:
        bad("hidden_channels", cfg["hidden_channels"], "must be a multiple of 32 (the WaveNet gate rows are paired in "
            "32-row MFMA fragments)")
    if cfg["inter_channels"] % 64 != 0:
        bad("inter_channels", cfg["inter_channels"], "must be a multiple of 64 (the couplings split the channels in halves "
            "of whole 32-row fragments)")


def on_own_device(method):
    import functools

    @functools.wraps(method)
    def wrapper(self, *args, **kwargs):
        dev = getattr(self, "device", None)
        if dev is None:
            dev = (getattr(self, "engine", None) or kwargs.get("engine") or args[0]).device
        with torch.cuda.device(dev):
            return method(self, *args, **kwargs)
    return wrapper


def _ptr(t, offset_elems=0):
    return ctypes.c_void_p(t.data_ptr() + 4 * offset_elems)


class PackedConv:

    def __init__(self, w_dense, bias, device, K, dil=1, cout=None):
        w_dense = w_dense.detach().to(torch.float32).cpu().contiguous()
        rows, cin, k = w_dense.shape
        assert k == K
        self.rows = rows
        self.cout = rows if cout is None else cout
        self.cin, self.K, self.dil = cin, K, dil
        n = _lib.call("ov_conv1d_pack_size", rows, cin, K)
        packed = torch.empty(n, dtype=torch.float32)
        _lib.call("ov_conv1d_pack_f32", w_dense, rows, cin, K, packed)
        self.w = packed.to(device)
        pack_rows = _lib.call("ov_conv1d_pack_rows", rows)
        b = torch.zeros(pack_rows, dtype=torch.float32)
        if bias is not None:
            b[:rows] = bias.detach().float().cpu()
        self.has_bias = bias is not None
        self.bias = b.to(device)


def padded_frames(T):
    return (T + 3) // 4 * 4


def ref_enc_lengths(T, n_convs=len(REF_ENC_FILTERS)):
    T = int(T)
    if T < 1:
        raise ValueError(f"ref_enc_lengths: T must be >= 1, got {T}")
    out = [T]
    for _ in range(n_convs):
        out.append((out[-1] - 1) // 2 + 1)
    return out


def gate_row_order(hidden):
    assert hidden % 32 == 0
    idx = []
    for q in range(hidden // 32):
        idx += list(range(32 * q, 32 * q + 32)) + list(range(hidden + 32 * q, hidden + 32 * q + 32))
    return torch.tensor(idx, dtype=torch.long)


def convt_row_order(cout, stride):
    s = stride
    if s == 8 and cout % 8 == 0:
        per_tile = 8
    elif s == 2 and cout % 32 == 0:
        per_tile = 32
    else:
        return None
    idx = []
    for q in range(cout // per_tile):
        for grp in range(2):
            for c in range(per_tile):
                for ph in range(s // 2):
                    idx.append((q * per_tile + c) * s + grp * (s // 2) + ph)
    return torch.tensor(idx, dtype=torch.long)


_EXTRA_CONV_FLAGS = int(os.environ.get("OPENVOICE_AMD_CONV_FLAGS", "0"))
if _EXTRA_CONV_FLAGS & ~_lib.F_NO_XCD_MAP:
    raise _lib.OvError(f"OPENVOICE_AMD_CONV_FLAGS={_EXTRA_CONV_FLAGS}: only the measurement bit OV_F_NO_XCD_MAP "
                       f"({_lib.F_NO_XCD_MAP}) may be set from the environment")


def launch_conv(layer, x, x_off, x_bs, out, out_off, out_bs, B, L, epi=EPI_LINEAR, flags=0, in_slope=1.0,
                scale=1.0, res=None, res_off=0, res_bs=0, add=None, add_bs=0, out2=None, out2_bs=0, mask=None,
                bias_b=None, bias_b_off=0, bias_b_bs=0, split=0, phase_s=1, cin=None, rows=None, tiles_per_wg=0,
                x_ld=0, out_ld=0, mask_bs=0, tile=0, loaders=0, chunk=0, col_limit=None, col_limit_scale=1):
    flags |= _EXTRA_CONV_FLAGS
    if _lib.use_torch_binding():
        ip = [B, layer.cin if cin is None else cin, L, x_ld, out_ld, layer.rows if rows is None else rows, layer.cout,
              layer.K, layer.dil, epi, flags, split, phase_s, tiles_per_wg, tile, loaders, chunk,
              x_bs, out_bs, res_bs, add_bs, out2_bs, bias_b_bs, mask_bs, x_off, out_off, res_off, bias_b_off,
              col_limit_scale]
        _lib.torch_op("conv1d_f32", x, layer.w, layer.bias, out, res, add, out2, mask, bias_b, col_limit, ip,
                      [in_slope, scale])
        return
    p = ConvParams()
    p.x, p.w = _ptr(x, x_off), _ptr(layer.w)
    p.bias = _ptr(layer.bias)
    p.bias_b = _ptr(bias_b, bias_b_off) if bias_b is not None else None
    p.out = _ptr(out, out_off)
    p.res = _ptr(res, res_off) if res is not None else None
    p.add = _ptr(add) if add is not None else None
    p.out2 = _ptr(out2) if out2 is not None else None
    p.mask = _ptr(mask) if mask is not None else None
    p.x_bstride, p.out_bstride, p.res_bstride = x_bs, out_bs, res_bs
    p.add_bstride, p.out2_bstride, p.bias_b_bstride = add_bs, out2_bs, bias_b_bs
    p.B, p.Cin, p.L = B, layer.cin if cin is None else cin, L
    p.M = layer.rows if rows is None else rows
    p.Cout = layer.cout
    p.K, p.dil, p.epi, p.flags, p.split, p.phase_s = layer.K, layer.dil, epi, flags, split, phase_s
    p.in_slope, p.scale = in_slope, scale
    p.tiles_per_wg, p.tile, p.loaders, p.chunk = tiles_per_wg, tile, loaders, chunk
    p.x_ld, p.out_ld, p.mask_bstride = x_ld, out_ld, mask_bs
    p.col_limit = ctypes.c_void_p(col_limit.data_ptr()) if col_limit is not None else None
    p.col_limit_scale = col_limit_scale
    stream = ctypes.c_void_p(torch.cuda.current_stream(x.device).cuda_stream)
    _lib.check(_lib.load().ov_conv1d_f32(ctypes.byref(p), stream), "ov_conv1d_f32")


def launch_pair(c1, c2, x, x_bs, out, out_bs, B, L, add=None, add_bs=0, scale=1.0, slope=LRELU_SLOPE, ld=0, nwg=0,
                dbg=None, col_limit=None, col_limit_scale=1):
    if _lib.use_torch_binding():
        _lib.torch_op("resblock_pair_f32", x, c1.w, c1.bias, c2.w, c2.bias, out, add, dbg, col_limit,
                      [B, c1.cin, L, ld, c1.K, c1.dil, nwg, x_bs, out_bs, add_bs, col_limit_scale], [slope, scale])
        return
    p = _lib.RespairParams()
    p.x, p.w1, p.b1, p.w2, p.b2 = _ptr(x), _ptr(c1.w), _ptr(c1.bias), _ptr(c2.w), _ptr(c2.bias)
    p.out = _ptr(out)
    p.add = _ptr(add) if add is not None else None
    p.x_bstride, p.out_bstride, p.add_bstride = x_bs, out_bs, add_bs
    p.B, p.C, p.L, p.ld, p.K, p.dil, p.nwg = B, c1.cin, L, ld, c1.K, c1.dil, nwg
    p.slope, p.scale = slope, scale
    p.dbg = ctypes.c_void_p(dbg.data_ptr()) if dbg is not None else None
    p.col_limit = ctypes.c_void_p(col_limit.data_ptr()) if col_limit is not None else None
    p.col_limit_scale = col_limit_scale
    stream = ctypes.c_void_p(torch.cuda.current_stream(x.device).cuda_stream)
    _lib.check(_lib.load().ov_resblock_pair_f32(ctypes.byref(p), stream), "ov_resblock_pair_f32")


_pair_supported = {}


def pair_supported(C, K, dil):
    key = (C, K, dil)
    if key not in _pair_supported:
        _pair_supported[key] = bool(_lib.call("ov_resblock_pair_supported", C, K, dil))
    return _pair_supported[key]


PAIR_POLICY = {(32, 3), (32, 7)}


def wino_policy(C, K, dil):
    return C >= 64 or dil == 1


WINO_MIN_ITEMS = 136

SPLIT_MIN_CHANNELS = 128


def _wino_mw(cout):
    return 4 if cout % 128 == 0 else (2 if cout % 64 == 0 else 1)


def wino_ncol(cout, dil):
    return (256 if dil == 1 else 4 * (64 // dil) * dil) * (4 // _wino_mw(cout))


def wino_items(cout, dil, B, L):
    ncol = wino_ncol(cout, dil)
    return B * ((L + ncol - 1) // ncol) * (cout // (32 * _wino_mw(cout)))


DIRECT_MIN_NCOL = 128


def conv_reach(family, K, dil=1):
    if family in ("direct", "pair", "split3"):
        r = (K - 1) // 2 * dil
        return r, r
    if family == "wino":
        from . import wino
        G = (K + 2) // 3
        pad = (K - 1) // 2 + wino.LEAD_TAPS[K]
        return (pad + 2) * dil, (3 * (G - 1) + 4 - pad) * dil
    raise ValueError(f"unknown conv family {family!r}")


def resblock_families(C, K, dils, B, L, use_winograd=True, fuse_pairs=True):
    from . import wino
    if fuse_pairs and L % 4 == 0 and all((C, K) in PAIR_POLICY and pair_supported(C, K, d) for d in dils):
        return [("pair", "pair")] * len(dils)
    fam = lambda d: ("wino" if use_winograd and L % 4 == 0 and wino.supported(C, C, K, d) and wino_policy(C, K, d)
                     and wino_items(C, d, B, L) >= WINO_MIN_ITEMS else "direct")
    return [(fam(d), fam(1)) for d in dils]


def limit_margin_frames(cfg, B, T, use_winograd=True, fuse_pairs=True):
    stages = generator_stages(cfg)

    def chain_reach(i, k, dils):
        C, L = stages[i].ch, T * stages[i].rate_out
        fams = resblock_families(C, k, dils, B, L, use_winograd, fuse_pairs)
        return sum(conv_reach(f1, k, d)[1] + conv_reach(f2, k, 1)[1] for (f1, f2), d in zip(fams, dils))

    return max(GENERATOR_MARGIN, generator_margin_frames(cfg), generator_margin_frames(cfg, chain_reach=chain_reach))


def wn_fused_row_order(hidden):
    assert hidden % 8 == 0
    idx = []
    for q in range(hidden // 8):
        for j in range(4):
            a, b = 8 * q + j, 8 * q + j + 4
            idx += [a, b, hidden + a, hidden + b]
    return torch.tensor(idx, dtype=torch.long)


def wn_pack(w_dense, device):
    w_dense = w_dense.detach().to(torch.float32).cpu().contiguous()
    rows, cin, k = w_dense.shape
    n = _lib.call("ov_wn_pack_size", rows, cin, k)
    assert n > 0, (rows, cin, k)
    packed = torch.empty(n, dtype=torch.float32)
    _lib.call("ov_wn_pack_f32", w_dense, rows, cin, k, packed)
    return packed.to(device)


WN_WINO_MIN_ITEMS = 168
WN_WINO_ROUND = 256


def wn_wino_items(B, T):
    return B * ((T + 127) // 128)


def wn_wino_policy(B, T):
    items = wn_wino_items(B, T)
    rounds = (items + WN_WINO_ROUND - 1) // WN_WINO_ROUND
    return items >= WN_WINO_MIN_ITEMS * rounds


def wn_wino_pack(w_dense, device):
    w_dense = w_dense.detach().to(torch.float32).cpu().contiguous()
    rows, cin, k = w_dense.shape
    n = _lib.call("ov_wn_wino_pack_size", rows, cin, k)
    assert n > 0, (rows, cin, k)
    packed = torch.empty(n, dtype=torch.float32)
    _lib.call("ov_wn_wino_pack_f32", w_dense, rows, cin, k, packed)
    return packed.to(device)


def launch_wn_layer(layer, x, out, skip, mask, B, T, ld, cond=None, cond_off=0, cond_bs=0, first=False, last=False,
                    width=0, mask_bs=0, dbg=None, acts=None, row_split=0, winograd=False):
    entry, w_in = ("wn_layer_wino_f32", layer["w_in_wino"]) if winograd else ("wn_layer_f32", layer["w_in"])
    if _lib.use_torch_binding():
        H = layer["hidden"]
        _lib.torch_op(entry, x, out, skip, w_in, layer["b_in"], cond, layer["w_rs"], layer["b_rs"],
                      mask, dbg, acts, [B, H, T, ld, layer["K"], int(first), int(last), width, H * ld, cond_bs, mask_bs,
                                        cond_off, row_split])
        return
    p = _lib.WnLayerParams()
    p.x, p.out, p.skip = _ptr(x), _ptr(out), _ptr(skip)
    p.w_in, p.b_in, p.w_rs, p.b_rs = _ptr(w_in), _ptr(layer["b_in"]), _ptr(layer["w_rs"]), _ptr(layer["b_rs"])
    p.cond = _ptr(cond, cond_off) if cond is not None else None
    p.mask = _ptr(mask)
    H = layer["hidden"]
    p.bstride, p.cond_bstride, p.mask_bstride = H * ld, cond_bs, mask_bs
    p.B, p.H, p.T, p.ld, p.K = B, H, T, ld, layer["K"]
    p.first, p.last, p.width, p.row_split = int(first), int(last), width, row_split
    p.dbg = ctypes.c_void_p(dbg.data_ptr()) if dbg is not None else None
    p.acts = _ptr(acts) if acts is not None else None
    stream = ctypes.c_void_p(torch.cuda.current_stream(x.device).cuda_stream)
    _lib.check(getattr(_lib.load(), "ov_" + entry)(ctypes.byref(p), stream), "ov_" + entry)


class _WaveNet:

    def __init__(self, sd, prefix, n_layers, hidden, device):
        order = gate_row_order(hidden)
        self.hidden, self.n_layers = hidden, n_layers
        self.in_layers, self.rs_layers, self.fused_layers = [], [], []
        K = sd[f"{prefix}.in_layers.0.weight_v"].shape[2] if f"{prefix}.in_layers.0.weight_v" in sd else \
            sd[f"{prefix}.in_layers.0.weight"].shape[2]
        self.fused = bool(_lib.call("ov_wn_layer_supported", hidden, K))
        forder = wn_fused_row_order(hidden) if self.fused else None
        for i in range(n_layers):
            w_in = effective_weight(sd, f"{prefix}.in_layers.{i}")
            b_in = sd[f"{prefix}.in_layers.{i}.bias"].float()
            self.in_layers.append(PackedConv(w_in[order], b_in[order], device, K=w_in.shape[2], cout=hidden))
            w_rs = effective_weight(sd, f"{prefix}.res_skip_layers.{i}")
            b_rs = sd[f"{prefix}.res_skip_layers.{i}.bias"].float()
            self.rs_layers.append(PackedConv(w_rs, b_rs, device, K=1))
            if self.fused:
                if w_rs.shape[0] == hidden:
                    w_rs = torch.cat([torch.zeros_like(w_rs), w_rs])
                    b_rs = torch.cat([torch.zeros_like(b_rs), b_rs])
                self.fused_layers.append(dict(hidden=hidden, K=w_in.shape[2], w_in=wn_pack(w_in[forder], device),
                                              w_in_wino=wn_wino_pack(w_in[forder], device),
                                              b_in=b_in[forder].contiguous().to(device), w_rs=wn_pack(w_rs, device),
                                              b_rs=b_rs.contiguous().to(device)))
        wc = effective_weight(sd, prefix + ".cond_layer")[:, :, 0]
        bc = sd[prefix + ".cond_layer.bias"].float()
        full = torch.cat([order + 2 * hidden * i for i in range(n_layers)])
        self.cond_w = wc[full].contiguous().to(device)
        self.cond_b = bc[full].contiguous().to(device)
        if self.fused:
            full = torch.cat([forder + 2 * hidden * i for i in range(n_layers)])
            self.cond_w_fused = wc[full].contiguous().to(device)
            self.cond_b_fused = bc[full].contiguous().to(device)


_DEC_BUFFERS = 5


def _workspace_elems(cfg, B, T):
    H, C, Tp = cfg["hidden_channels"], cfg["inter_channels"], padded_frames(T)
    frame_rate = Tp + 4 * H * Tp + C * Tp + 3 * C * Tp + generator_stages(cfg)[0].cin * Tp
    return B * frame_rate, B * T * scratch_per_frame(cfg)


def _resblock_tree(sd, cfg, make, keep=lambda stage: True):
    convs = list(resblock_convs(cfg))
    layer = lambda c, name, d: make(c, effective_weight(sd, name), sd[name + ".bias"], d)
    return [[[(layer(c, f"{c.prefix}.convs1.{c.n}", c.dil), layer(c, f"{c.prefix}.convs2.{c.n}", 1))
              for c in convs if (c.stage, c.j) == (i, j)]
             for j in range(len(cfg["resblock_kernel_sizes"]))] if keep(i) else None
            for i in range(len(cfg["upsample_rates"]))]


class ConverterEngine:

    def __init__(self, state_dict, model_cfg, spec_channels, device, zero_g=False):
        self.device = torch.device(device)
        if self.device.type != "cuda":
            raise _lib.OvError("ConverterEngine needs a ROCm device ('cuda:N'); there is no CPU path")
        sd = {k: v.detach().float().cpu() for k, v in state_dict.items()}
        cfg = dict(model_cfg.items()) if hasattr(model_cfg, "items") else dict(model_cfg)
        validate_config(cfg)
        self.cfg = cfg
        self.zero_g = bool(zero_g)
        self.inter = cfg["inter_channels"]
        self.hidden = cfg["hidden_channels"]
        self.gin = cfg.get("gin_channels", 256)
        self.spec_channels = spec_channels
        dev = self.device
        H, C = self.hidden, self.inter
        half = C // 2
        self.q_pre = PackedConv(sd["enc_q.pre.weight"], sd["enc_q.pre.bias"], dev, K=1)
        self.q_wn = _WaveNet(sd, "enc_q.enc", ENC_Q_LAYERS, H, dev)
        order = gate_row_order(C)
        self.q_proj = PackedConv(sd["enc_q.proj.weight"][order], sd["enc_q.proj.bias"][order], dev, K=1, cout=C)
        self.couplings = []
        for f in range(N_FLOWS):
            p = f"flow.flows.{2 * f}"
            flipped = f % 2 == 1
            w_pre, w_post, b_post = sd[p + ".pre.weight"], sd[p + ".post.weight"], sd[p + ".post.bias"]
            if flipped:
                w_pre = torch.flip(w_pre, [1])
                w_post, b_post = torch.flip(w_post, [0]), torch.flip(b_post, [0])
            self.couplings.append(dict(
                flipped=flipped,
                pre=PackedConv(w_pre, sd[p + ".pre.bias"], dev, K=1),
                wn=_WaveNet(sd, p + ".enc", FLOW_LAYERS, H, dev),
                post=PackedConv(w_post, b_post, dev, K=1)))
        self.half = half
        self.conv_pre = PackedConv(sd["dec.conv_pre.weight"], sd["dec.conv_pre.bias"], dev, K=7)
        self.dec_cond_w = sd["dec.cond.weight"][:, :, 0].contiguous().to(dev)
        self.dec_cond_b = sd["dec.cond.bias"].contiguous().to(dev)
        self.stages = generator_stages(cfg)
        self.ups = []
        for i, _, ch, u, *_ in self.stages:
            wc = conv_transpose_as_conv(effective_weight(sd, f"dec.ups.{i}"), u)
            bias = sd[f"dec.ups.{i}.bias"].repeat_interleave(u)
            order = convt_row_order(ch, u)
            if order is not None:
                wc, bias = wc[order], bias[order]
            self.ups.append(dict(conv=PackedConv(wc, bias, dev, K=3, cout=ch), stride=u,
                                 flags=F_CONVT_GROUPED if order is not None else 0))
        self.resblocks = _resblock_tree(sd, cfg, lambda c, w, b, d: PackedConv(w, b, dev, K=c.K, dil=d))
        from . import wino as _wino
        self.wino_resblocks = _resblock_tree(sd, cfg, lambda c, w, b, d: _wino.PackedConvWino(w, b, dev, dil=d)
                                             if _wino.supported(c.ch, c.ch, c.K, d) and wino_policy(c.ch, c.K, d) else None)
        self.final_channels = self.stages[-1].ch
        self.post_w = sd["dec.conv_post.weight"][0].contiguous().to(dev)
        self.total_upsample = samples_per_frame(cfg)
        self.ref_enc = None
        if "ref_enc.gru.weight_ih_l0" in sd:
            convs = [(effective_weight(sd, f"ref_enc.convs.{i}").contiguous().to(dev),
                      sd[f"ref_enc.convs.{i}.bias"].contiguous().to(dev)) for i in range(len(REF_ENC_FILTERS))]
            w_ih = sd["ref_enc.gru.weight_ih_l0"]
            self.ref_enc = dict(
                ln_w=sd["ref_enc.layernorm.weight"].contiguous().to(dev),
                ln_b=sd["ref_enc.layernorm.bias"].contiguous().to(dev),
                convs=convs,
                gru_in=PackedConv(w_ih.unsqueeze(-1), sd["ref_enc.gru.bias_ih_l0"], dev, K=1),
                whh_t=sd["ref_enc.gru.weight_hh_l0"].t().contiguous().to(dev),
                bhh=sd["ref_enc.gru.bias_hh_l0"].contiguous().to(dev),
                proj_w=sd["ref_enc.proj.weight"].contiguous().to(dev),
                proj_b=sd["ref_enc.proj.bias"].contiguous().to(dev))
        self._ws, self._graphs, self._limit_margins = {}, {}, {}
        self._live_ws, self._live_ws_bf16, self.live_ws_builds = {}, {}, 0
        self.resident_workspaces = 1
        self.profile = None
        self.chain_streams = 1
        self.chain_streams_max_batch = 8
        self._streams = []
        self._zeros = {}
        self.generator_margin = max(GENERATOR_MARGIN, generator_margin_frames(self.cfg))
        self.fuse_wn = True
        self.wn_row_split = 0
        self.fuse_pairs = True
        self.use_winograd = True
        self._state_dict_for_bf16 = sd
        self.generator_bf16 = None
        self._bf16_on = False
        self._split3_on = False
        self.split3_products = 6
        self.split_resblocks = None

    def _stream(self):
        return ctypes.c_void_p(torch.cuda.current_stream(self.device).cuda_stream)

    def _timed(self, tag, flops, fn, *extra):
        if self.profile is None:
            return fn()
        e0, e1 = torch.cuda.Event(enable_timing=True), torch.cuda.Event(enable_timing=True)
        e0.record()
        out = fn()
        e1.record()
        self.profile.append((tag, flops, e0, e1) + extra)
        return out

    def _conv(self, layer, x, x_off, x_bs, out, out_off, out_bs, B, L, tag="conv", alg_flops=None, **kwargs):
        if alg_flops is None:
            alg_flops = 2.0 * layer.rows * (kwargs.get("cin") or layer.cin) * layer.K * L * B
        self._timed(tag, alg_flops, lambda: launch_conv(layer, x, x_off, x_bs, out, out_off, out_bs, B, L, **kwargs))

    def _wino(self, layer, x, out, bs, B, L, res=None, add=None, scale=1.0, in_slope=LRELU_SLOPE, out_slope=1.0, **lim):
        from . import wino
        kw = dict(in_slope=in_slope, out_slope=out_slope, scale=scale, res=res, res_bs=bs if res is not None else 0, add=add,
                  add_bs=bs if add is not None else 0, **lim)
        alg = 2.0 * layer.cout * layer.cin * layer.K * L * B
        self._timed("mrf", alg, lambda: wino.launch_conv_wino(layer, x, bs, out, bs, B, L, **kw),
                    alg * wino.PRODUCTS_PER_TILE[layer.K] / (4.0 * layer.K))

    def _pair(self, c1, c2, x, out, bs, B, L, add, scale, **lim):
        self._timed("mrf", 2 * 2.0 * c1.rows * c1.cin * c1.K * L * B,
                    lambda: launch_pair(c1, c2, x, bs, out, bs, B, L, add=add, add_bs=bs, scale=scale, **lim))

    def _linear(self, x2d, w, b):
        Bg, Kd = x2d.shape
        M = w.shape[0]
        y = torch.empty(Bg, M, dtype=torch.float32, device=self.device)
        _lib.call("ov_linear_f32", x2d, w, b, y, Bg, M, Kd)
        return y

    def _wn_cond(self, wn, g):
        if self.fuse_wn and wn.fused:
            return self._linear(g, wn.cond_w_fused, wn.cond_b_fused)
        return self._linear(g, wn.cond_w, wn.cond_b)

    def _workspace(self, B, T):
        key = (B, T)
        ws = self._ws.pop(key, None)
        if ws is not None:
            self._ws[key] = ws
        else:
            while self._ws and len(self._ws) >= max(1, int(self.resident_workspaces)):
                self._ws.pop(next(iter(self._ws)))
            dev, H, C = self.device, self.hidden, self.inter
            Tp = padded_frames(T)
            f = lambda *shape: torch.zeros(*shape, dtype=torch.float32, device=dev)
            lat = f(3, B, C, Tp)
            ws = dict(Tp=Tp, mask=f(B, Tp), h=f(B, H, Tp), h2=f(B, H, Tp), acts=f(B, H, Tp), skip=f(B, H, Tp), noise=f(B, C, Tp),
                      lat=lat, z=lat[0], z_p=lat[1], z_hat=lat[2])
            ws["pre"] = f(B, self.stages[0].cin, Tp)
            dec = _workspace_elems(self.cfg, B, T)[1]
            ws["dec"] = [torch.empty(dec, dtype=torch.float32, device=dev) for _ in range(_DEC_BUFFERS)]
            self._ws[key] = ws
        return ws

    def workspace_bytes(self, B, T):
        frame_rate, dec = _workspace_elems(self.cfg, B, T)
        return 4 * (frame_rate + _DEC_BUFFERS * dec)

    def _zeros_like_cached(self, t):
        key = tuple(t.shape)
        z = self._zeros.get(key)
        if z is None:
            z = self._zeros[key] = torch.zeros_like(t)
        return z

    def _side_streams(self, n):
        while len(self._streams) < n:
            self._streams.append(torch.cuda.Stream(self.device))
        return self._streams[:n]

    def _chain_scratch(self, ws, n):
        extra = ws.setdefault("dec_extra", [])
        while len(extra) < n:
            extra.append(torch.empty_like(ws["dec"][0]))
        return extra

    def _wavenet(self, wn, ws, B, T, cond, mask):
        H, Tp = wn.hidden, ws["Tp"]
        cbs = 0 if cond.shape[0] == 1 else cond.shape[1]
        if self.fuse_wn and wn.fused:
            src, dst = ws["h"], ws["h2"]
            winograd = self.use_winograd and wn_wino_policy(B, T)
            for i in range(wn.n_layers):
                layer = wn.fused_layers[i]
                args = dict(cond=cond, cond_off=2 * H * i, cond_bs=cbs, first=i == 0, last=i == wn.n_layers - 1,
                            mask_bs=Tp, acts=ws["acts"], row_split=self.wn_row_split, winograd=winograd)
                rs_rows = H if args["last"] else 2 * H
                self._timed("wn_layer", 2.0 * (2 * H * H * layer["K"] + rs_rows * H) * T * B,
                            lambda: launch_wn_layer(layer, src, dst, ws["skip"], mask, B, T, Tp, **args))
                src, dst = dst, src
            return
        for i in range(wn.n_layers):
            self._conv(wn.in_layers[i], ws["h"], 0, H * Tp, ws["acts"], 0, H * Tp, B, T, epi=EPI_GATE,
                       bias_b=cond, bias_b_off=2 * H * i, bias_b_bs=cbs, rows=2 * H, x_ld=Tp, out_ld=Tp, tag="wn_in")
            last = i == wn.n_layers - 1
            self._conv(wn.rs_layers[i], ws["acts"], 0, H * Tp, ws["h"], 0, H * Tp, B, T, epi=EPI_RESSKIP,
                       flags=F_OUT2_INIT if i == 0 else 0, out2=ws["skip"], out2_bs=H * Tp, mask=mask, mask_bs=Tp,
                       split=0 if last else H, x_ld=Tp, out_ld=Tp, tag="wn_rs")

    def _flow(self, src, buf, ws, B, T, conds, mask, reverse):
        C, half, H, Tp = self.inter, self.half, self.hidden, ws["Tp"]
        order = range(N_FLOWS - 1, -1, -1) if reverse else range(N_FLOWS)
        for n, f in enumerate(order):
            cp = self.couplings[f]
            x0_off = half * Tp if cp["flipped"] else 0
            x1_off = 0 if cp["flipped"] else half * Tp
            self._conv(cp["pre"], src if n == 0 else buf, x0_off, C * Tp, ws["h"], 0, H * Tp, B, T, flags=F_MASK_V,
                       mask=mask, mask_bs=Tp, x_ld=Tp, out_ld=Tp, tag="cpl_pre")
            self._wavenet(cp["wn"], ws, B, T, conds[f], mask)
            self._conv(cp["post"], ws["skip"], 0, H * Tp, buf, x1_off, C * Tp, B, T, epi=EPI_COUPLE, mask=mask,
                       mask_bs=Tp, x_ld=Tp, out_ld=Tp, scale=-1.0 if reverse else 1.0, tag="cpl_post",
                       res=src if n < 2 else None, res_off=x1_off, res_bs=C * Tp)

    @torch.no_grad()
    @on_own_device
    def voice_conversion(self, spec, spec_lengths, sid_src, sid_tgt, tau=1.0, noise=None, skip_padding=False, *,
                         seed=None, generator=None):
        use_bf16 = self._bf16_on
        if _lib.check_generator(generator, optional=True) is not None:
            use_bf16 = generator == "bf16"
        dev = self.device
        spec = spec.to(dev, torch.float32)
        B, F, T = spec.shape
        assert F == self.spec_channels
        if not (spec.stride(2) == 1 and spec.stride(1) >= T and spec.stride(0) >= F * spec.stride(1)):
            spec = spec.contiguous()
        C = self.inter
        lengths = spec_lengths.to(dev, torch.int64).contiguous()
        g_src = sid_src.to(dev, torch.float32).reshape(sid_src.shape[0], -1).contiguous()
        g_tgt = sid_tgt.to(dev, torch.float32).reshape(sid_tgt.shape[0], -1).contiguous()
        noise_mod.exclusive(seed, noise=noise)
        ws = self._workspace(B, T)
        Tp, mask = ws["Tp"], ws["mask"]
        if seed is not None:
            self.seed_noise(ws["noise"], seed, B, T, Tp)
        elif noise is None:
            ws["noise"][:, :, :T].normal_()
        else:
            ws["noise"][:, :, :T].copy_(noise.to(dev, torch.float32))
        _lib.call("ov_sequence_mask_f32", lengths, mask, B, T, Tp)
        conds = self._conds(g_src, g_tgt)
        self._frames(ws, 0, B, spec, conds, tau)
        z, z_p, z_hat = ws["z"], ws["z_p"], ws["z_hat"]
        if use_bf16:
            g_d = self._zeros_like_cached(g_tgt) if self.zero_g else g_tgt
            o_hat = self._timed("gen_bf16", 0.0, lambda: self.bf16_generator().decode(z_hat[:, :, :T], g_d.unsqueeze(-1)))
            if skip_padding:
                keep_samples = (lengths.clamp(max=T) * self.total_upsample).view(B, 1, 1)
                o_hat.masked_fill_(torch.arange(o_hat.shape[2], device=dev).view(1, 1, -1) >= keep_samples, 0.0)
        else:
            limits = self.frame_limits(lengths, T) if skip_padding else None
            o_hat = self.decode(z_hat, conds["d"], ws, T=T, limits=limits)
        dense = torch.empty(3, B, C, T, dtype=torch.float32, device=dev)
        _lib.call("ov_unpad_rows_f32", ws["lat"], dense, 3 * B * C, T, Tp)
        y_mask = torch.empty(B, 1, T, dtype=torch.float32, device=dev)
        _lib.call("ov_unpad_rows_f32", mask, y_mask, B, T, Tp)
        return o_hat, y_mask, (dense[0], dense[1], dense[2])

    def seed_noise(self, dst, seed, B, T, ld, purpose=noise_mod.PURPOSE_POSTERIOR):
        C = self.inter
        noise_mod.fill([(s, k, purpose, f0, T, b * C * ld, ld) for b, (s, k, f0) in enumerate(noise_mod.rows(seed, B))],
                       C, dst)

    def _frames(self, ws, b0, b1, spec, conds, tau):
        nb, T, Tp = b1 - b0, spec.shape[2], ws["Tp"]
        C, H = self.inter, self.hidden
        sub = {k: (v[b0:b1] if torch.is_tensor(v) else v) for k, v in ws.items() if k != "dec"}
        rows = lambda t: t if t.shape[0] == 1 else t[b0:b1]
        mask = sub["mask"]
        x = spec[b0:b1]
        self._conv(self.q_pre, x, 0, spec.stride(0), sub["h"], 0, H * Tp, nb, T, flags=F_MASK_V, mask=mask, mask_bs=Tp,
                   x_ld=spec.stride(1), out_ld=Tp, tag="q_pre")
        self._wavenet(self.q_wn, sub, nb, T, rows(conds["q"]), mask)
        z, z_p, z_hat = sub["z"], sub["z_p"], sub["z_hat"]
        self._conv(self.q_proj, sub["skip"], 0, H * Tp, z, 0, C * Tp, nb, T, epi=EPI_POSTERIOR, res=sub["noise"],
                   res_bs=C * Tp, scale=float(tau), mask=mask, mask_bs=Tp, rows=2 * C, x_ld=Tp, out_ld=Tp, tag="q_proj")
        self._flow(z, z_p, sub, nb, T, [rows(c) for c in conds["src"]], mask, reverse=False)
        self._flow(z_p, z_hat, sub, nb, T, [rows(c) for c in conds["tgt"]], mask, reverse=True)

    def graphed(self, B, T, tau, src_rows=1, tgt_rows=1, max_cached=4, skip_padding=False):
        key = (int(B), int(T), float(tau), int(src_rows), int(tgt_rows), self._bf16_on,
               bool(skip_padding), bool(self._split3_on), self.split3_products)
        cache = self._graphs
        g = cache.pop(key, None)
        if g is None:
            g = GraphedConversion(self, B, T, tau, src_rows, tgt_rows, skip_padding=skip_padding)
            while len(cache) >= max_cached:
                cache.pop(next(iter(cache)))
        cache[key] = g
        return g

    def use_bf16_generator(self, enable=True):
        if enable:
            self.bf16_generator()
        self._bf16_on = bool(enable)
        return self

    def bf16_generator(self):
        if self.generator_bf16 is None:
            from .bf16 import GeneratorBf16
            self.generator_bf16 = GeneratorBf16(self._state_dict_for_bf16, self.cfg, self.device)
        return self.generator_bf16

    def use_split_bf16x3(self, enable=True, products=6):
        if products not in (6, 3):
            raise _lib.OvError(f"use_split_bf16x3: products must be 6 or 3, got {products!r}")
        if enable and self.split_resblocks is None:
            from . import split3
            convs = list(resblock_convs(self.cfg))
            keep = lambda i: all(c.ch >= SPLIT_MIN_CHANNELS and split3.supported(c.ch, c.ch, c.K, c.dil)
                                 and split3.supported(c.ch, c.ch, c.K, 1) for c in convs if c.stage == i)
            self.split_resblocks = _resblock_tree(self._state_dict_for_bf16, self.cfg, lambda c, w, b, d:
                                                  split3.PackedConvSplit3(w, b, self.device, dil=d), keep)
        self._split3_on = bool(enable)
        self.split3_products = products
        self._graphs.clear()
        return self

    def _split_buffers(self, ws, B, st, L):
        nk = len(self.cfg["resblock_kernel_sizes"])
        need = 3 * B * L * st.ch
        bufs = ws.get("split3")
        if bufs is None:
            if torch.cuda.is_current_stream_capturing():
                raise _lib.OvError("split-precision plane buffers must exist before graph capture: run one eager conversion "
                                   "of this (batch, frames) shape first")
            frames = L // st.rate_out
            largest = max([need] + [3 * B * frames * o.rate_out * o.ch for o in self.stages
                                    if self.split_resblocks[o.index] is not None])
            bufs = ws["split3"] = [torch.empty(largest, dtype=torch.bfloat16, device=self.device) for _ in range(4 + nk)]
        assert bufs[0].numel() >= need
        return [b[:need].view(3, B, L, st.ch) for b in bufs]

    def _mrf_split(self, st, u, acc, ws, B, L, limits=None):
        from . import split3
        stage, ch = self.split_resblocks[st.index], st.ch
        nk = len(stage)
        bufs = self._split_buffers(ws, B, st, L)
        xa, t, ping, pong, results = bufs[0], bufs[1], bufs[2], bufs[3], bufs[4:]
        prod = self.split3_products
        lim = dict(col_limit=limits, col_limit_scale=st.rate_out) if limits is not None else {}
        timed = self._timed
        uv = u[:B * ch * L].view(B, ch, L)
        timed("split_layout", 0.0, lambda: split3.to_planes(uv, LRELU_SLOPE, out=xa))
        for j, pairs in enumerate(stage):
            cur = xa
            for n, (c1, c2) in enumerate(pairs):
                last = n == len(pairs) - 1
                flops = 2.0 * ch * ch * c1.K * L * B
                timed("mrf_split", flops, lambda: split3.launch_conv_split3(c1, cur, t, out_slope=LRELU_SLOPE, products=prod, **lim))
                dst = results[j] if last else (pong if cur is ping else ping)
                timed("mrf_split", flops, lambda: split3.launch_conv_split3(c2, t, dst, res=cur, res_slope=LRELU_SLOPE,
                                                                             out_slope=1.0 if last else LRELU_SLOPE,
                                                                             products=prod, **lim))
                cur = dst
        ops = list(results[:nk]) + [None] * (3 - nk)
        if nk > 3:
            raise _lib.OvError("split-precision MRF: at most 3 ResBlocks per stage")
        av = acc[:B * ch * L].view(B, ch, L)
        timed("split_layout", 0.0, lambda: split3.from_planes(ops[0], ops[1], ops[2], in_slope=1.0, scale=1.0 / nk, out=av))

    def limit_margin(self, B, T):
        key = (int(B), int(T), bool(self.use_winograd), bool(self.fuse_pairs))
        cache = self._limit_margins
        if key not in cache:
            cache[key] = max(self.generator_margin, limit_margin_frames(self.cfg, *key))
        return cache[key]

    def frame_limits(self, lengths, T):
        B = lengths.shape[0]
        lim = torch.empty(2, B, dtype=torch.int32, device=self.device)
        _lib.call("ov_frame_limits_i32", lengths, lim[0], B, int(T), self.limit_margin(B, T))
        _lib.call("ov_frame_limits_i32", lengths, lim[1], B, int(T), 0)
        return lim

    def _upsample(self, i, x, x_ld, u, B, L, cin, ch, **lim):
        up = self.ups[i]
        s = up["stride"]
        self._conv(up["conv"], x, 0, cin * x_ld, u, 0, ch * L * s, B, L, epi=EPI_CONVT, in_slope=LRELU_SLOPE,
                   flags=up["flags"], phase_s=s, x_ld=x_ld, tag="ups", alg_flops=2.0 * cin * ch * 2 * s * L * B, **lim)

    def _mrf(self, i, u, t1, ra, acc, ws, B, ch, L, limits, rate):
        cfg = self.cfg
        nk = len(cfg["resblock_kernel_sizes"])
        lim = lambda scale: dict(col_limit=limits, col_limit_scale=scale) if limits is not None else {}
        bs = ch * L
        concurrent = (self.chain_streams > 1 and nk > 1 and B <= self.chain_streams_max_batch and self.profile is None
                      and not (torch.cuda.is_current_stream_capturing() and len(ws.get("dec_extra", [])) < 2 * (nk - 1)))
        scratch = [(t1, ra)]
        if concurrent:
            extra = self._chain_scratch(ws, 2 * (nk - 1))
            scratch += [(extra[2 * j], extra[2 * j + 1]) for j in range(nk - 1)]

        def chain(j, pairs):
            t1_, ra_ = scratch[j if concurrent else 0]
            cur = u
            fams = resblock_families(ch, pairs[0][0].K, [c1.dil for c1, _ in pairs], B, L, self.use_winograd,
                                     self.fuse_pairs)
            fused = fams[0][0] == "pair"
            wn = self.wino_resblocks[i][j]
            for n, (c1, c2) in enumerate(pairs):
                last = n == len(pairs) - 1
                if last and concurrent and j > 0:
                    torch.cuda.current_stream(self.device).wait_event(done[j - 1])
                add = acc if (last and j > 0) else None
                scale = 1.0 / nk if (last and j == nk - 1) else 1.0
                if fused:
                    dst = acc if last else (t1_ if cur is ra_ else ra_)
                    self._pair(c1, c2, cur, dst, bs, B, L, add, scale, **lim(rate))
                else:
                    w1, w2 = (w if f == "wino" else None for w, f in zip(wn[n], fams[n]))
                    if w1 is not None:
                        self._wino(w1, cur, t1_, bs, B, L, out_slope=LRELU_SLOPE, **lim(rate))
                    else:
                        self._conv(c1, cur, 0, bs, t1_, 0, bs, B, L, in_slope=LRELU_SLOPE, tag="mrf", **lim(rate))
                    c2_slope = 1.0 if w1 is not None else LRELU_SLOPE
                    dst = acc if last else ra_
                    if w2 is not None:
                        self._wino(w2, t1_, dst, bs, B, L, res=cur, add=add, scale=scale, in_slope=c2_slope, **lim(rate))
                    else:
                        self._conv(c2, t1_, 0, bs, dst, 0, bs, B, L, in_slope=c2_slope, res=cur, res_bs=bs,
                                   add=add, add_bs=bs, scale=scale, tag="mrf", **lim(rate))
                cur = dst

        if not concurrent:
            for j, pairs in enumerate(self.resblocks[i]):
                chain(j, pairs)
        else:
            main = torch.cuda.current_stream(self.device)
            side = self._side_streams(nk)
            fork = torch.cuda.Event()
            fork.record(main)
            done = [None] * nk
            for j, pairs in enumerate(self.resblocks[i]):
                with torch.cuda.stream(side[j]):
                    side[j].wait_event(fork)
                    chain(j, pairs)
                    done[j] = torch.cuda.Event()
                    done[j].record(side[j])
            for j in range(nk):
                main.wait_event(done[j])

    def _stage(self, st, x, x_ld, x_bs, bufs, out, ws, B, L, cond_d=None, limits=None, keep=None):
        lim = lambda scale: dict(col_limit=limits, col_limit_scale=scale) if limits is not None else {}
        if st.index == 0:
            Tp = ws["Tp"]
            self._conv(self.conv_pre, x, 0, x_bs, ws["pre"], 0, st.cin * Tp, B, L, bias_b=cond_d,
                       bias_b_bs=0 if cond_d.shape[0] == 1 else cond_d.shape[1], x_ld=x_ld, out_ld=Tp, tag="conv_pre",
                       **lim(1))
            x, x_ld = ws["pre"], Tp
        u, t1, ra, acc = bufs
        self._upsample(st.index, x, x_ld, u, B, L, st.cin, st.ch, **lim(st.rate_in))
        L *= st.stride
        if t1 is None:
            self._mrf_split(st, u, acc, ws, B, L, limits=limits)
        else:
            self._mrf(st.index, u, t1, ra, acc, ws, B, st.ch, L, limits, st.rate_out)
        if st.last and keep is not None:
            _lib.call("ov_conv_post_tanh_limited_f32", acc, self.post_w, out, B, st.ch, L, self.post_w.shape[1],
                      FINAL_LRELU_SLOPE, keep, st.rate_out)
        elif st.last:
            _lib.call("ov_conv_post_tanh_f32", acc, self.post_w, out, B, st.ch, L, self.post_w.shape[1], FINAL_LRELU_SLOPE)

    def decode(self, z_hat, cond_d, ws=None, T=None, limits=None):
        B, C, ld = z_hat.shape
        T = ld if T is None else T
        if ws is None:
            ws = self._workspace(B, T)
        keep = None
        if limits is not None:
            limits, keep = limits[0], limits[1]
            if B > LIMIT_MAX_BATCH:
                limits = None
        o_hat = torch.empty(B, 1, T * self.total_upsample, dtype=torch.float32, device=self.device)
        x, x_ld, x_bs = z_hat, ld, C * ld
        free = list(ws["dec"])
        for st in self.stages:
            u = free.pop()
            if st.index > 0:
                free.append(x)
            split = self._split3_on and self.split_resblocks[st.index] is not None
            t1, ra = (None, None) if split else (free.pop(), free.pop())
            acc = free.pop()
            self._stage(st, x, x_ld, x_bs, (u, t1, ra, acc), o_hat, ws, B, T * st.rate_in, cond_d, limits, keep)
            free += [u] if split else [u, t1, ra]
            x, x_ld = acc, T * st.rate_out
        return o_hat

    def live_workspace(self, key, B, width, stage=None):
        cache = self._live_ws
        ws = cache.get((key, B))
        if ws is not None:
            assert ws["width"] >= width, "live unit wider than its workspace"
            return ws
        self.live_ws_builds += 1
        dev, H = self.device, self.hidden
        z = lambda *shape: torch.zeros(*shape, dtype=torch.float32, device=dev)
        Tp = padded_frames(width)
        if stage is None:
            ws = dict(Tp=Tp, mask=z(B, Tp), mask_len=-1, h=z(B, H, Tp), h2=z(B, H, Tp), acts=z(B, H, Tp),
                      skip=z(B, H, Tp))
        else:
            st = self.stages[stage]
            n = B * st.ch * width * st.stride
            ws = dict(Tp=Tp, dec=[z(n) for _ in range(3)])
            if stage == 0:
                ws["pre"] = z(B, st.cin, Tp)
            if st.last:
                ws["acc"] = z(n)
        ws["width"] = width
        cache[(key, B)] = ws
        return ws

    def _conds(self, g_src, g_tgt):
        g_q = self._zeros_like_cached(g_src) if self.zero_g else g_src
        g_d = self._zeros_like_cached(g_tgt) if self.zero_g else g_tgt
        return dict(q=self._wn_cond(self.q_wn, g_q), src=[self._wn_cond(cp["wn"], g_src) for cp in self.couplings],
                    tgt=[self._wn_cond(cp["wn"], g_tgt) for cp in self.couplings],
                    d=self._linear(g_d, self.dec_cond_w, self.dec_cond_b))

    live_conds = _conds

    def _live_mask(self, ws, B, L):
        if ws["mask_len"] != L:
            lengths = torch.full((B,), L, dtype=torch.int64, device=self.device)
            _lib.call("ov_sequence_mask_f32", lengths, ws["mask"], B, L, ws["Tp"])
            ws["mask_len"] = L
        return ws["mask"]

    @torch.no_grad()
    @on_own_device
    def live_posterior(self, spec, spec_ld, spec_bs, noise, noise_bs, out, ld, bs, B, L, cond_q, tau, ws):
        H, C, Tp = self.hidden, self.inter, ws["Tp"]
        mask = self._live_mask(ws, B, L)
        self._conv(self.q_pre, spec, 0, spec_bs, ws["h"], 0, H * Tp, B, L, flags=F_MASK_V, mask=mask, mask_bs=Tp,
                   x_ld=spec_ld, out_ld=Tp, tag="q_pre")
        self._wavenet(self.q_wn, ws, B, L, cond_q, mask)
        self._conv(self.q_proj, ws["skip"], 0, H * Tp, out, 0, bs, B, L, epi=EPI_POSTERIOR, res=noise, res_bs=noise_bs,
                   scale=float(tau), mask=mask, mask_bs=Tp, rows=2 * C, x_ld=Tp, out_ld=ld, tag="q_proj")

    @torch.no_grad()
    @on_own_device
    def live_flow(self, src, dst, B, L, conds, reverse, ws):
        self._flow(src, dst, ws, B, L, conds, self._live_mask(ws, B, L), reverse)

    @torch.no_grad()
    @on_own_device
    def live_generator_stage(self, i, x, x_ld, x_bs, out, B, L, ws, cond_d=None):
        if self._bf16_on or self._split3_on:
            raise _lib.OvError("live streams run the fp32 generator only (use_bf16_generator / split_bf16x3 are off)")
        st = self.stages[i]
        u, t1, ra = ws["dec"]
        self._stage(st, x, x_ld, x_bs, (u, t1, ra, ws["acc"] if st.last else out), out, ws, B, L, cond_d)

    @torch.no_grad()
    @on_own_device
    def live_cond_bf16(self, g_tgt):
        g_d = self._zeros_like_cached(g_tgt) if self.zero_g else g_tgt
        return self.bf16_generator().cond_rows(g_d)

    def live_workspace_bf16(self, key, B, width, stage):
        cache = self._live_ws_bf16
        ws = cache.get((key, B))
        if ws is not None:
            assert ws["width"] >= width, "live unit wider than its workspace"
            return ws
        self.live_ws_builds += 1
        f = lambda n: torch.empty(n, dtype=torch.bfloat16, device=self.device)
        st = self.stages[stage]
        n = self.bf16_generator().stage_scratch_elems(stage, B, width)
        ws = dict(width=width, xin=f(B * width * (self.inter if stage == 0 else st.cin)), out=None if st.last else f(n),
                  bufs=[f(n) for _ in range(4 if st.last else 3)], pre=f(B * width * st.cin) if stage == 0 else None)
        cache[(key, B)] = ws
        return ws

    @torch.no_grad()
    @on_own_device
    def live_generator_stage_bf16(self, i, x, x_ld, x_bs, out, B, L, ws, cond_d=None):
        if self._bf16_on or self._split3_on:
            raise _lib.OvError("a live unit's generator is chosen by its pool (use_bf16_generator / split_bf16x3 are off)")
        gen, st = self.bf16_generator(), self.stages[i]
        cin, s = self.inter if i == 0 else st.cin, st.stride
        xin = ws["xin"][: B * L * cin].view(B, L, cin)
        _lib.call("ov_rows_f32_to_cl_bf16", x, x_bs, x_ld, xin, B, cin, L)
        bufs = list(ws["bufs"])
        if st.last:
            gen.stage(i, xin, out[: B * L * s].view(B, 1, L * s), B, L, cond=cond_d, bufs=bufs, pre=ws["pre"])
            return
        o = ws["out"][: B * L * s * st.ch].view(B, L * s, st.ch)
        gen.stage(i, xin, o, B, L, cond=cond_d, bufs=bufs, pre=ws["pre"])
        _lib.call("ov_cl_bf16_to_rows_f32", o, out, st.ch * L * s, L * s, B, st.ch, L * s)

    @torch.no_grad()
    @on_own_device
    def reference_encoder(self, spec_t):
        re = self.ref_enc
        if re is None:
            raise _lib.OvError("this checkpoint has no ref_enc.* weights")
        dev = self.device
        x = spec_t.to(dev, torch.float32).transpose(1, 2).contiguous()
        N, F, T = x.shape
        assert F == self.spec_channels
        cur = torch.empty_like(x)
        _lib.call("ov_layernorm_freq_f32", x, re["ln_w"], re["ln_b"], cur, N, F, T, 1e-5)
        cin = 1
        for w, b in re["convs"]:
            cout = w.shape[0]
            Fo, To = (F - 1) // 2 + 1, (T - 1) // 2 + 1
            nxt = torch.empty(N, cout, Fo, To, dtype=torch.float32, device=dev)
            _lib.call("ov_conv2d_s2_relu_f32", cur, w, b, nxt, N, cin, cout, F, T)
            cur, cin, F, T = nxt, cout, Fo, To
        feat = cin * F
        H = REF_ENC_GRU
        gi = torch.empty(N, 3 * H, T, dtype=torch.float32, device=dev)
        self._conv(re["gru_in"], cur, 0, feat * T, gi, 0, 3 * H * T, N, T, tag="gru_in")
        h = torch.empty(N, H, dtype=torch.float32, device=dev)
        _lib.call("ov_gru_f32", gi, re["whh_t"], re["bhh"], h, N, H, T)
        return self._linear(h, re["proj_w"], re["proj_b"])

    @torch.no_grad()
    @on_own_device
    def reference_encoder_ragged(self, spec, frames):
        re = self.ref_enc
        cur, steps, L = self._reference_encoder_ragged_stack(spec, frames)
        P, H = cur.shape[0], REF_ENC_GRU
        feat = cur.shape[1] * cur.shape[2]
        gi = torch.empty(P, 3 * H, L, dtype=torch.float32, device=self.device)
        self._conv(re["gru_in"], cur, 0, feat * L, gi, 0, 3 * H * L, P, L, tag="gru_in")
        h = torch.empty(P, H, dtype=torch.float32, device=self.device)
        _lib.call("ov_gru_ragged_f32", gi, re["whh_t"], re["bhh"], steps, h, P, H, L)
        return self._linear(h, re["proj_w"], re["proj_b"])

    @torch.no_grad()
    @on_own_device
    def _reference_encoder_ragged_stack(self, spec, frames):
        re = self.ref_enc
        if re is None:
            raise _lib.OvError("this checkpoint has no ref_enc.* weights")
        dev = self.device
        x = spec.to(dev, torch.float32)
        if x.dim() != 3:
            raise ValueError(f"reference_encoder_ragged: spec must be [P, n_freq, W], got {tuple(x.shape)}")
        P, F, W = x.shape
        assert F == self.spec_channels
        frames = [int(f) for f in frames]
        if len(frames) != P or P < 1:
            raise ValueError(f"reference_encoder_ragged: {len(frames)} lengths for {P} items")
        if min(frames) < 1 or max(frames) > W:
            raise ValueError(f"reference_encoder_ragged: every length must be in [1, {W}], got {frames}")
        ld = x.stride(1)
        if x.stride() != (F * ld, ld, 1) or ld < W:
            x = x.contiguous()
            ld = W
        n_convs = len(re["convs"])
        table = torch.tensor([list(col) for col in zip(*(ref_enc_lengths(f, n_convs) for f in frames))],
                             dtype=torch.int32).to(dev)
        lds = ref_enc_lengths(ld, n_convs)
        cur = torch.empty(P, F, ld, dtype=torch.float32, device=dev)
        _lib.call("ov_layernorm_freq_ragged_f32", x, re["ln_w"], re["ln_b"], table[0], cur, P, F, ld, 1e-5)
        cin = 1
        for k, (w, b) in enumerate(re["convs"]):
            cout = w.shape[0]
            Fo = (F - 1) // 2 + 1
            nxt = torch.empty(P, cout, Fo, lds[k + 1], dtype=torch.float32, device=dev)
            _lib.call("ov_conv2d_s2_relu_ragged_f32", cur, w, b, table[k], nxt, P, cin, cout, F, lds[k], lds[k + 1])
            cur, cin, F = nxt, cout, Fo
        return cur, table[n_convs], lds[-1]


class GraphedConversion:

    @on_own_device
    def __init__(self, engine, B, T, tau, src_rows=1, tgt_rows=1, skip_padding=False):
        dev = engine.device
        self.engine, self.B, self.T, self.tau = engine, int(B), int(T), float(tau)
        f = lambda *shape: torch.zeros(*shape, dtype=torch.float32, device=dev)
        self.spec = f(B, engine.spec_channels, padded_frames(T))[:, :, :T]
        self.lengths = torch.full((B,), T, dtype=torch.int64, device=dev)
        self.g_src, self.g_tgt = f(src_rows, engine.gin, 1), f(tgt_rows, engine.gin, 1)
        self.noise = f(B, engine.inter, T)
        run = lambda: engine.voice_conversion(self.spec, self.lengths, self.g_src, self.g_tgt, tau=self.tau,
                                              noise=self.noise, skip_padding=skip_padding)
        saved, engine.profile = engine.profile, None
        try:
            side = torch.cuda.Stream(dev)
            side.wait_stream(torch.cuda.current_stream(dev))
            with torch.cuda.stream(side):
                run()
            torch.cuda.current_stream(dev).wait_stream(side)
            self.workspace = engine._workspace(B, T)
            self.graph = torch.cuda.CUDAGraph()
            with torch.cuda.graph(self.graph):
                self.out = run()
        finally:
            engine.profile = saved

    @torch.no_grad()
    @on_own_device
    def __call__(self, spec, spec_lengths, sid_src, sid_tgt, noise=None, *, seed=None):
        noise_mod.exclusive(seed, noise=noise)
        if tuple(spec.shape) != (self.B, self.engine.spec_channels, self.T):
            raise _lib.OvError(f"graph captured for spec {(self.B, self.engine.spec_channels, self.T)}, got {tuple(spec.shape)}")
        self.spec.copy_(spec)
        self.lengths.copy_(spec_lengths)
        self.g_src.copy_(sid_src.reshape(self.g_src.shape))
        self.g_tgt.copy_(sid_tgt.reshape(self.g_tgt.shape))
        if seed is not None:
            self.engine.seed_noise(self.noise, seed, self.B, self.T, self.T)
        elif noise is None:
            self.noise.normal_()
        else:
            self.noise.copy_(noise)
        self.graph.replay()
        return self.out
```

openvoice_amd/wino.py:

```python
import ctypes

import torch

from . import _lib

BT = ((4, 0, -5, 0, 1, 0), (0, -4, -4, 1, 1, 0), (0, 4, -4, -1, 1, 0), (0, -2, -1, 2, 1, 0), (0, 2, -1, -2, 1, 0),
      (0, 4, 0, -5, 0, 1))
G = ((1 / 4, 0, 0), (-1 / 6, -1 / 6, -1 / 6), (-1 / 6, 1 / 6, -1 / 6), (1 / 24, 1 / 12, 1 / 6), (1 / 24, -1 / 12, 1 / 6),
     (0, 0, 1))
AT = ((1, 1, 1, 1, 1, 0), (0, 1, -1, 2, -2, 0), (0, 1, 1, 4, 4, 0), (0, 1, -1, 8, -8, 1))


LEAD_TAPS = {3: 0, 7: 1, 11: 0}
PRODUCTS_PER_TILE = {3: 6, 7: 16, 11: 23}


def supported(cin, cout, K, dil):
    return bool(_lib.call("ov_conv1d_wino_supported", cin, cout, K, dil))


class PackedConvWino:

    def __init__(self, w_dense, bias, device, dil=1):
        w = w_dense.detach().to(torch.float32).cpu().contiguous()
        self.cout, self.cin, self.K = w.shape
        self.dil = dil
        if not supported(self.cin, self.cout, self.K, dil):
            raise _lib.OvError(f"ov_conv1d_wino_f32: no instance for Cin={self.cin} Cout={self.cout} K={self.K} dil={dil}")
        n = _lib.call("ov_conv1d_wino_pack_size", self.cout, self.cin, self.K)
        packed = torch.empty(n, dtype=torch.float32)
        _lib.call("ov_conv1d_wino_pack_f32", w, self.cout, self.cin, self.K, packed)
        self.w = packed.to(device)
        b = torch.zeros(self.cout) if bias is None else bias.detach().float().cpu()
        self.bias = b.contiguous().to(device)


def launch_conv_wino(layer, x, x_bs, out, out_bs, B, L, in_slope=1.0, scale=1.0, res=None, res_bs=0, add=None, add_bs=0,
                     x_ld=0, out_ld=0, nwg=0, dbg=None, frags=0, col_limit=None, col_limit_scale=1, out_slope=1.0):
    if _lib.use_torch_binding():
        _lib.torch_op("conv1d_wino_f32", x, layer.w, layer.bias, out, res, add, dbg, col_limit,
                      [B, layer.cin, layer.cout, L, x_ld, out_ld, layer.K, layer.dil, nwg, x_bs, out_bs, res_bs, add_bs, frags, col_limit_scale],
                      [in_slope, scale, out_slope])
        return
    p = _lib.ConvWinoParams()
    vp = lambda t: ctypes.c_void_p(t.data_ptr()) if t is not None else None
    p.x, p.w, p.bias, p.out, p.res, p.add = vp(x), vp(layer.w), vp(layer.bias), vp(out), vp(res), vp(add)
    p.x_bstride, p.out_bstride, p.res_bstride, p.add_bstride = x_bs, out_bs, res_bs, add_bs
    p.B, p.Cin, p.Cout, p.L, p.x_ld, p.out_ld = B, layer.cin, layer.cout, L, x_ld, out_ld
    p.K, p.dil, p.nwg, p.frags = layer.K, layer.dil, nwg, frags
    p.in_slope, p.scale, p.out_slope = in_slope, scale, out_slope
    p.dbg = vp(dbg)
    p.col_limit, p.col_limit_scale = vp(col_limit), col_limit_scale
    stream = ctypes.c_void_p(torch.cuda.current_stream(x.device).cuda_stream)
    _lib.check(_lib.load().ov_conv1d_wino_f32(ctypes.byref(p), stream), "ov_conv1d_wino_f32")
```

Before: 3105 x real-time (audio s / wall s).

## Fuse the three MRF resblock Winograd convs into one persistent multi-segment launch

```diff
diff --git a/include/openvoice_amd.h b/include/openvoice_amd.h
--- a/include/openvoice_amd.h
+++ b/include/openvoice_amd.h
@@ -355,6 +355,7 @@
   float out_slope;
 } ov_conv1d_wino_params;
 int ov_conv1d_wino_f32(const ov_conv1d_wino_params* p, ov_stream_t stream);
+int ov_conv1d_wino_multi_f32(const ov_conv1d_wino_params* convs, int n, ov_stream_t stream);
 int ov_conv1d_wino_supported(int Cin, int Cout, int K, int dil);
 int ov_conv1d_wino_chunk(int K, int Cout);
 size_t ov_conv1d_wino_pack_size(int Cout, int Cin, int K);
diff --git a/openvoice_amd/_lib.py b/openvoice_amd/_lib.py
--- a/openvoice_amd/_lib.py
+++ b/openvoice_amd/_lib.py
@@ -149,6 +149,7 @@
     "ov_split3_from_f32": (ctypes.c_int, [_fp, _fp, _i64, _i, _i, _i, ctypes.c_float, _fp]),
     "ov_split3_to_f32": (ctypes.c_int, [_fp, _fp, _fp, _i64, _fp, _i, _i, _i, ctypes.c_float, ctypes.c_float, _fp]),
     "ov_conv1d_wino_f32": (ctypes.c_int, [ctypes.POINTER(ConvWinoParams), _fp]),
+    "ov_conv1d_wino_multi_f32": (ctypes.c_int, [ctypes.POINTER(ConvWinoParams), _i, _fp]),
     "ov_conv1d_wino_supported": (ctypes.c_int, [_i, _i, _i, _i]),
     "ov_conv1d_wino_chunk": (ctypes.c_int, [_i, _i]),
     "ov_conv1d_wino_pack_size": (ctypes.c_size_t, [_i, _i, _i]),
diff --git a/openvoice_amd/csrc/conv1d_wino.h b/openvoice_amd/csrc/conv1d_wino.h
--- a/openvoice_amd/csrc/conv1d_wino.h
+++ b/openvoice_amd/csrc/conv1d_wino.h
@@ -92,8 +92,62 @@
     tlast = now_;                                                  \
   }
 
+constexpr int wino_ci(int K, int mw = 4) {
+  return mw == 1 ? (K == 11 ? 2 : 0) : K == 3 ? (mw == 4 ? 16 : 8) : (K == 7 || K == 11) ? (mw == 4 ? 8 : 4) : 0;
+}
+constexpr int wino_mw(int Cout) { return Cout % 128 == 0 ? 4 : (Cout % 64 == 0 ? 2 : (Cout % 32 == 0 ? 1 : 0)); }
+
+template <int K, int DIL, int CI, int NF, int MW>
+struct WinoShape {
+  using Gd = GeoD<K, DIL == 1 ? 3 : DIL, NF>;
+  static constexpr int G = (K + 2) / 3, KR = CI * G;
+  static constexpr int NB = 4 / MW, NTS = 32 * NF, NT = NTS * NB;
+  static constexpr int NCOLS = DIL == 1 ? 4 * NTS : Gd::NCOL, NCOL = NCOLS * NB;
+  static constexpr int RW = (DIL == 1 ? NCOLS + 16 : Gd::RW) + (NB - 1) * NCOLS;
+  static constexpr int RAW_FLOATS = 2 * CI * RW;
+  static constexpr int V_FLOATS = 2 * KR * NT * 6;
+  static constexpr int OST_FLOATS = DIL == 1 ? 4 : 4 * 8 * 256;
+};
+
+template <int NCOL, int MW>
+__device__ __forceinline__ int wino_total(const ov_conv1d_wino_params& p, int* lim_pref) {
+  const int lane = threadIdx.x & 63;
+  const int wave = __builtin_amdgcn_readfirstlane(threadIdx.x >> 6);
+  const int L = p.L;
+  const int ntiles = (L + NCOL - 1) / NCOL;
+  const int mblocks = p.Cout / (32 * MW);
+  int total = ntiles * mblocks * p.B;
+  if (p.col_limit != nullptr) {
+    if (wave == 0) {
+      int carry = 0;
+      for (int base = 0; base < p.B; base += 64) {
+        const int bb = base + lane;
+        int nb = 0;
+        if (bb < p.B) {
+          long long c = (long long)p.col_limit[bb] * p.col_limit_scale;
+          c = c < 0 ? 0 : (c > L ? L : c);
+          nb = ((int)c + NCOL - 1) / NCOL;
+        }
+        int sc = nb;
+#pragma unroll
+        for (int d = 1; d < 64; d <<= 1) {
+          const int v = __shfl_up(sc, d, 64);
+          if (lane >= d) sc += v;
+        }
+        if (bb < p.B) lim_pref[bb + 1] = carry + sc;
+        carry += __shfl(sc, 63, 64);
+      }
+      if (lane == 0) lim_pref[0] = 0;
+    }
+    __syncthreads();
+    total = __builtin_amdgcn_readfirstlane(lim_pref[p.B]) * mblocks;
+  }
+  return total;
+}
+
 template <int K, int DIL, int CI, int NF, int MW, bool DBG>
-__global__ __launch_bounds__(64 * (4 + 2 * NF), NF == 1 ? 3 : 2) void conv1d_wino_kernel(const ov_conv1d_wino_params p) {
+__device__ __forceinline__ void wino_body(const ov_conv1d_wino_params& p, const int wid0, const int wend, const int wstride,
+                                          float* raw, float* Vs, float* bias_s, float* ostage, const int* lim_pref) {
   using Ge = Geo<K>;
   using Gd = GeoD<K, DIL == 1 ? 3 : DIL, NF>;
   constexpr int G = Ge::G, KR = CI * G, NSTEP = KR / 2, NPAIR = NSTEP / 2;
@@ -113,11 +167,10 @@
   constexpr int NITEM = NPR * RW4;
   constexpr int RAWBUF = CI * RW;
   constexpr int VBUF = KR * NT * 6;
-  __shared__ __attribute__((aligned(16))) float raw[2 * RAWBUF];
-  __shared__ __attribute__((aligned(16))) float Vs[2 * VBUF];
-  __shared__ __attribute__((aligned(16))) float bias_s[MAX_COUT];
   constexpr int OST = 256;
-  __shared__ __attribute__((aligned(16))) float ostage[DIL == 1 ? 4 : 4 * 8 * OST];
+  using Sh = WinoShape<K, DIL, CI, NF, MW>;
+  static_assert(Sh::RAW_FLOATS == 2 * RAWBUF && Sh::V_FLOATS == 2 * VBUF && Sh::NCOL == NCOL &&
+                    Sh::OST_FLOATS == (DIL == 1 ? 4 : 4 * 8 * OST), "WinoShape restates this geometry");
 
   const int tid = threadIdx.x;
   const int lane = tid & 63;
@@ -126,34 +179,7 @@
   const int nchunks = p.Cin / CI;
   const int ntiles = (L + NCOL - 1) / NCOL;
   const int mblocks = p.Cout / (32 * MW);
-  int total = ntiles * mblocks * p.B;
-  __shared__ int lim_pref[ovk::LIMIT_MAX_BATCH + 1];
   const bool limited = p.col_limit != nullptr;
-  if (limited) {
-    if (wave == 0) {
-      int carry = 0;
-      for (int base = 0; base < p.B; base += 64) {
-        const int bb = base + lane;
-        int nb = 0;
-        if (bb < p.B) {
-          long long c = (long long)p.col_limit[bb] * p.col_limit_scale;
-          c = c < 0 ? 0 : (c > L ? L : c);
-          nb = ((int)c + NCOL - 1) / NCOL;
-        }
-        int sc = nb;
-#pragma unroll
-        for (int d = 1; d < 64; d <<= 1) {
-          const int v = __shfl_up(sc, d, 64);
-          if (lane >= d) sc += v;
-        }
-        if (bb < p.B) lim_pref[bb + 1] = carry + sc;
-        carry += __shfl(sc, 63, 64);
-      }
-      if (lane == 0) lim_pref[0] = 0;
-    }
-    __syncthreads();
-    total = __builtin_amdgcn_readfirstlane(lim_pref[p.B]) * mblocks;
-  }
   auto decode = [&](int w, int& ub, int& utile, int& umblk) {
     const int g = w / mblocks;
     umblk = w - g * mblocks;
@@ -170,14 +196,6 @@
     ub = lo;
     utile = g - __builtin_amdgcn_readfirstlane(lim_pref[lo]);
   };
-  int wid0 = blockIdx.x, wend = total, wstride = gridDim.x;
-  if ((gridDim.x & 7u) == 0) {
-    const int xcd = blockIdx.x & 7;
-    const int lo = (int)(((long long)xcd * total) >> 3);
-    wend = (int)(((long long)(xcd + 1) * total) >> 3);
-    wid0 = lo + (int)(blockIdx.x >> 3);
-    wstride = gridDim.x >> 3;
-  }
   if (wid0 >= wend) return;
   const int nitems = (wend - wid0 + wstride - 1) / wstride;
   const int nstream = nitems * nchunks;
@@ -636,6 +654,120 @@
   }
 }
 
+__device__ __forceinline__ bool wino_xcd_eighth(int total, int& lo, int& hi) {
+  if ((gridDim.x & 7u) != 0) return false;
+  const int xcd = blockIdx.x & 7;
+  lo = (int)(((long long)xcd * total) >> 3);
+  hi = (int)(((long long)(xcd + 1) * total) >> 3);
+  return true;
+}
+
+template <int K, int DIL, int CI, int NF, int MW, bool DBG>
+__global__ __launch_bounds__(64 * (4 + 2 * NF), NF == 1 ? 3 : 2) void conv1d_wino_kernel(const ov_conv1d_wino_params p) {
+  using Sh = WinoShape<K, DIL, CI, NF, MW>;
+  __shared__ __attribute__((aligned(16))) float raw[Sh::RAW_FLOATS];
+  __shared__ __attribute__((aligned(16))) float Vs[Sh::V_FLOATS];
+  __shared__ __attribute__((aligned(16))) float bias_s[MAX_COUT];
+  __shared__ __attribute__((aligned(16))) float ostage[Sh::OST_FLOATS];
+  __shared__ int lim_pref[ovk::LIMIT_MAX_BATCH + 1];
+  const int total = wino_total<Sh::NCOL, MW>(p, lim_pref);
+  int wid0 = blockIdx.x, wend = total, wstride = gridDim.x;
+  int lo, hi;
+  if (wino_xcd_eighth(total, lo, hi)) {
+    wend = hi;
+    wid0 = lo + (int)(blockIdx.x >> 3);
+    wstride = gridDim.x >> 3;
+  }
+  wino_body<K, DIL, CI, NF, MW, DBG>(p, wid0, wend, wstride, raw, Vs, bias_s, ostage, lim_pref);
+}
+
+struct wino_multi_args {
+  ov_conv1d_wino_params seg[3];
+  long long cost[3];
+  int present;
+  int balance;
+};
+
+struct wino_range { int wid0, wend, wstride; };
+__device__ __forceinline__ void wino_multi_ranges(const wino_multi_args& a, int total, wino_range (&rg)[3]) {
+#pragma unroll
+  for (int s = 0; s < 3; ++s) rg[s] = wino_range{(int)blockIdx.x, total, (int)gridDim.x};
+  int lo, hi;
+  if (!wino_xcd_eighth(total, lo, hi)) return;
+  const int m = gridDim.x >> 3, j = blockIdx.x >> 3, n = hi - lo;
+#pragma unroll
+  for (int s = 0; s < 3; ++s) rg[s] = wino_range{lo + j, hi, m};
+  const int pr = a.present & 7, nseg = __builtin_popcount(pr);
+  const int q = n / m, r = n - q * m;
+  if (!a.balance || nseg < 2 || r == 0) return;
+  const int last = (pr & 4) ? 2 : 1;
+  const int head = (pr & 1) ? 0 : 1;
+  const long long c0 = head == 0 ? a.cost[0] : a.cost[1];
+  const long long c1 = nseg == 3 ? a.cost[1] : 0;
+  const long long cl = last == 2 ? a.cost[2] : a.cost[1];
+  const long long W = (long long)n * (c0 + c1 + cl);
+  if (cl <= 0 || W < (long long)m * (q + 1) * (c0 + c1)) return;
+  auto start = [&](int jj) {
+    const int over = jj - (m - r);
+    const long long S = (long long)jj * q * (c0 + c1) + c0 * (jj < r ? jj : r) + c1 * (over > 0 ? over : 0);
+    return (int)(((long long)jj * W - (long long)m * S) / ((long long)m * cl));
+  };
+  const wino_range cut = wino_range{lo + start(j), lo + start(j + 1), 1};
+  if (nseg == 3) {
+    const int pos = j + r < m ? j + r : j + r - m;
+    rg[1] = wino_range{lo + pos, hi, m};
+  }
+  if (last == 2) rg[2] = cut; else rg[1] = cut;
+}
+
+template <int DIL, int NF, int MW>
+__global__ __launch_bounds__(64 * (4 + 2 * NF), 2) void conv1d_wino_multi_kernel(const wino_multi_args a) {
+  using S11 = WinoShape<11, DIL, wino_ci(11, MW), NF, MW>;
+  using S7 = WinoShape<7, DIL, wino_ci(7, MW), NF, MW>;
+  using S3 = WinoShape<3, DIL, wino_ci(3, MW), NF, MW>;
+  constexpr int F11 = S11::RAW_FLOATS + S11::V_FLOATS + S11::OST_FLOATS, F7 = S7::RAW_FLOATS + S7::V_FLOATS + S7::OST_FLOATS,
+                F3 = S3::RAW_FLOATS + S3::V_FLOATS + S3::OST_FLOATS;
+  constexpr int FMAX = F11 > F7 ? (F11 > F3 ? F11 : F3) : (F7 > F3 ? F7 : F3);
+  static_assert(S11::NCOL == S7::NCOL && S11::NCOL == S3::NCOL, "one work list geometry for all kernel sizes");
+  static_assert(S11::RAW_FLOATS % 4 == 0 && S7::RAW_FLOATS % 4 == 0 && S3::RAW_FLOATS % 4 == 0 && S11::V_FLOATS % 4 == 0 &&
+                    S7::V_FLOATS % 4 == 0 && S3::V_FLOATS % 4 == 0, "16-byte aligned regions");
+  __shared__ __attribute__((aligned(16))) float lds[FMAX];
+  __shared__ __attribute__((aligned(16))) float bias_s[MAX_COUT];
+  __shared__ int lim_pref[ovk::LIMIT_MAX_BATCH + 1];
+  const int first = (a.present & 1) ? 0 : ((a.present & 2) ? 1 : 2);
+  const int total = wino_total<S11::NCOL, MW>(a.seg[first], lim_pref);
+  wino_range rg[3];
+  wino_multi_ranges(a, total, rg);
+  if (a.present & 1)
+    wino_body<11, DIL, wino_ci(11, MW), NF, MW, false>(a.seg[0], rg[0].wid0, rg[0].wend, rg[0].wstride, lds, lds + S11::RAW_FLOATS,
+                                                        bias_s, lds + S11::RAW_FLOATS + S11::V_FLOATS, lim_pref);
+  __syncthreads();
+  if (a.present & 2)
+    wino_body<7, DIL, wino_ci(7, MW), NF, MW, false>(a.seg[1], rg[1].wid0, rg[1].wend, rg[1].wstride, lds, lds + S7::RAW_FLOATS,
+                                                      bias_s, lds + S7::RAW_FLOATS + S7::V_FLOATS, lim_pref);
+  __syncthreads();
+  if (a.present & 4)
+    wino_body<3, DIL, wino_ci(3, MW), NF, MW, false>(a.seg[2], rg[2].wid0, rg[2].wend, rg[2].wstride, lds, lds + S3::RAW_FLOATS,
+                                                      bias_s, lds + S3::RAW_FLOATS + S3::V_FLOATS, lim_pref);
+}
+
+template <int DIL, int NF, int MW>
+int wino_multi_launch(const wino_multi_args* a, int nwg_forced, hipStream_t stream) {
+  constexpr int NCOL = WinoShape<11, DIL, wino_ci(11, MW), NF, MW>::NCOL, NHELP = 2 * NF;
+  const ov_conv1d_wino_params* p = &a->seg[(a->present & 1) ? 0 : ((a->present & 2) ? 1 : 2)];
+  const int ntiles = (p->L + NCOL - 1) / NCOL;
+  const long total = (long)ntiles * (p->Cout / (32 * MW)) * p->B;
+  auto kernel = conv1d_wino_multi_kernel<DIL, NF, MW>;
+  static std::atomic<int> slot_cache[ovk::OV_MAX_DEVICES];
+  const int slots = ovk::resident_workgroups(reinterpret_cast<const void*>(kernel), 64 * (4 + NHELP), slot_cache);
+  long nwg = nwg_forced > 0 ? nwg_forced : slots;
+  if (nwg > total) nwg = total;
+  if (nwg >= 8) nwg = (nwg + 7) / 8 * 8;
+  hipLaunchKernelGGL(kernel, dim3((unsigned)nwg), dim3(64 * (4 + NHELP)), 0, stream, *a);
+  return hipGetLastError() == hipSuccess ? OV_OK : OV_E_LAUNCH;
+}
+int wino_multi_dispatch(const wino_multi_args* a, int nwg, hipStream_t stream);
+
 template <int K, int DIL, int CI, int NF, int MW, bool DBG>
 int wino_launch(const ov_conv1d_wino_params* p, hipStream_t stream) {
   constexpr int NCOL = (DIL == 1 ? 128 * NF : GeoD<K, DIL == 1 ? 3 : DIL, NF>::NCOL) * (4 / MW), NHELP = 2 * NF;
@@ -651,11 +783,6 @@
   return hipGetLastError() == hipSuccess ? OV_OK : OV_E_LAUNCH;
 }
 
-constexpr int wino_ci(int K, int mw = 4) {
-  return mw == 1 ? (K == 11 ? 2 : 0) : K == 3 ? (mw == 4 ? 16 : 8) : (K == 7 || K == 11) ? (mw == 4 ? 8 : 4) : 0;
-}
-constexpr int wino_mw(int Cout) { return Cout % 128 == 0 ? 4 : (Cout % 64 == 0 ? 2 : (Cout % 32 == 0 ? 1 : 0)); }
-
 int wino_dispatch_k3(const ov_conv1d_wino_params* p, int nf, hipStream_t stream);
 int wino_dispatch_k7(const ov_conv1d_wino_params* p, int nf, hipStream_t stream);
 int wino_dispatch_k11(const ov_conv1d_wino_params* p, int nf, hipStream_t stream);
diff --git a/openvoice_amd/csrc/conv1d_wino.hip b/openvoice_amd/csrc/conv1d_wino.hip
--- a/openvoice_amd/csrc/conv1d_wino.hip
+++ b/openvoice_amd/csrc/conv1d_wino.hip
@@ -52,9 +52,7 @@
   return OV_OK;
 }
 
-int ov_conv1d_wino_f32(const ov_conv1d_wino_params* pin, ov_stream_t stream) {
-  if (!pin) return OV_E_BADARG;
-  ov_conv1d_wino_params q = *pin;
+static int wino_check(ov_conv1d_wino_params& q) {
   if (!q.x || !q.w || !q.bias || !q.out) return OV_E_BADARG;
   if (q.B <= 0 || q.L <= 0 || q.nwg < 0) return OV_E_BADARG;
   if (q.col_limit && (q.col_limit_scale <= 0 || (reinterpret_cast<uintptr_t>(q.col_limit) & 3))) return OV_E_BADARG;
@@ -78,10 +76,17 @@
   if (q.B > 1 && (q.x_bstride < (int64_t)q.Cin * q.x_ld || q.out_bstride < (int64_t)q.Cout * q.out_ld ||
                   (q.res && q.res_bstride < (int64_t)q.Cout * q.out_ld) || (q.add && q.add_bstride < (int64_t)q.Cout * q.out_ld)))
     return OV_E_BADARG;
+  if (q.frags < 0 || q.frags > 2) return OV_E_BADARG;
+  if (q.dil != 1 && (q.frags ? q.frags : 2) != 2) return OV_E_UNSUPPORTED;
+  return OV_OK;
+}
+
+int ov_conv1d_wino_f32(const ov_conv1d_wino_params* pin, ov_stream_t stream) {
+  if (!pin) return OV_E_BADARG;
+  ov_conv1d_wino_params q = *pin;
+  if (const int rc = wino_check(q)) return rc;
   hipStream_t st = static_cast<hipStream_t>(stream);
-  if (q.frags < 0 || q.frags > 2) return OV_E_BADARG;
   const int nf = q.frags ? q.frags : 2;
-  if (q.dil != 1 && nf != 2) return OV_E_UNSUPPORTED;
   switch (q.K) {
     case 3: return wino_dispatch_k3(&q, nf, st);
     case 7: return wino_dispatch_k7(&q, nf, st);
@@ -90,4 +95,34 @@
   return OV_E_UNSUPPORTED;
 }
 
+int ov_conv1d_wino_multi_f32(const ov_conv1d_wino_params* convs, int n, ov_stream_t stream) {
+  if (!convs || n < 1 || n > 3) return OV_E_BADARG;
+  if (n == 1) return ov_conv1d_wino_f32(convs, stream);
+  wino_multi_args a;
+  std::memset(&a, 0, sizeof(a));
+  for (int i = 0; i < n; ++i) {
+    ov_conv1d_wino_params q = convs[i];
+    if (const int rc = wino_check(q)) return rc;
+    const int slot = q.K == 11 ? 0 : (q.K == 7 ? 1 : 2);
+    a.seg[slot] = q;
+  }
+  for (int i = 1; i < n; ++i) {
+    const ov_conv1d_wino_params &u = convs[0], &v = convs[i];
+    if (u.B != v.B || u.L != v.L || u.Cin != v.Cin || u.Cout != v.Cout || u.dil != v.dil || u.col_limit != v.col_limit ||
+        (u.col_limit && u.col_limit_scale != v.col_limit_scale))
+      return OV_E_BADARG;
+  }
+  for (int i = 0; i < n; ++i) {
+    const ov_conv1d_wino_params& v = convs[i];
+    const int bit = 1 << (v.K == 11 ? 0 : (v.K == 7 ? 1 : 2));
+    if (a.present & bit) return OV_E_UNSUPPORTED;
+    a.present |= bit;
+    if (v.dbg || v.frags == 1 || wino_mw(v.Cout) < 2) return OV_E_UNSUPPORTED;
+  }
+  const int kk[3] = {11, 7, 3};
+  for (int s = 0; s < 3; ++s) a.cost[s] = (long long)wino_products(kk[s]) * convs[0].Cin + 380;
+  a.balance = 1;
+  return wino_multi_dispatch(&a, convs[0].nwg, static_cast<hipStream_t>(stream));
 }
+
+}
diff --git a/openvoice_amd/csrc/conv1d_wino_multi.hip b/openvoice_amd/csrc/conv1d_wino_multi.hip
--- /dev/null
+++ b/openvoice_amd/csrc/conv1d_wino_multi.hip
@@ -0,0 +1,16 @@
+#include "conv1d_wino.h"
+
+int ovkw::wino_multi_dispatch(const wino_multi_args* a, int nwg, hipStream_t st) {
+  const ov_conv1d_wino_params* p = &a->seg[(a->present & 1) ? 0 : ((a->present & 2) ? 1 : 2)];
+  const int mw = wino_mw(p->Cout);
+  if (mw == 4) {
+    if (p->dil == 1) return wino_multi_launch<1, 2, 4>(a, nwg, st);
+    if (p->dil == 3) return wino_multi_launch<3, 2, 4>(a, nwg, st);
+    if (p->dil == 5) return wino_multi_launch<5, 2, 4>(a, nwg, st);
+  } else if (mw == 2) {
+    if (p->dil == 1) return wino_multi_launch<1, 2, 2>(a, nwg, st);
+    if (p->dil == 3) return wino_multi_launch<3, 2, 2>(a, nwg, st);
+    if (p->dil == 5) return wino_multi_launch<5, 2, 2>(a, nwg, st);
+  }
+  return OV_E_UNSUPPORTED;
+}
diff --git a/openvoice_amd/csrc/torch_shim.cpp b/openvoice_amd/csrc/torch_shim.cpp
--- a/openvoice_amd/csrc/torch_shim.cpp
+++ b/openvoice_amd/csrc/torch_shim.cpp
@@ -342,6 +342,33 @@
   finish(ov_conv1d_wino_f32(&p, c.stream()), "ov_conv1d_wino_f32");
 }
 
+void conv1d_wino_multi_f32(const OptTensor& x0, const OptTensor& w0, const OptTensor& b0, const OptTensor& o0, const OptTensor& r0,
+                           const OptTensor& a0, const OptTensor& x1, const OptTensor& w1, const OptTensor& b1, const OptTensor& o1,
+                           const OptTensor& r1, const OptTensor& a1, const OptTensor& x2, const OptTensor& w2, const OptTensor& b2,
+                           const OptTensor& o2, const OptTensor& r2, const OptTensor& a2, const OptTensor& col_limit, int64_t n,
+                           at::IntArrayRef ip, at::ArrayRef<double> fp) {
+  TORCH_CHECK(n >= 1 && n <= 3 && (int64_t)ip.size() == 15 * n && (int64_t)fp.size() == 3 * n,
+              "openvoice_amd::conv1d_wino_multi_f32: 1 .. 3 convs, 15 integer and 3 float parameters each");
+  Ctx c{"conv1d_wino_multi_f32", false};
+  const OptTensor* t[3][6] = {{&x0, &w0, &b0, &o0, &r0, &a0}, {&x1, &w1, &b1, &o1, &r1, &a1}, {&x2, &w2, &b2, &o2, &r2, &a2}};
+  ov_conv1d_wino_params ps[3] = {};
+  const int32_t* lim = sptr<int32_t>(col_limit, c, 18);
+  for (int64_t i = 0; i < n; ++i) {
+    ov_conv1d_wino_params& p = ps[i];
+    const int64_t* q = ip.data() + 15 * i;
+    const int k = 6 * (int)i;
+    p.x = sptr<float>(*t[i][0], c, k); p.w = sptr<float>(*t[i][1], c, k + 1); p.bias = sptr<float>(*t[i][2], c, k + 2);
+    p.out = sptr<float>(*t[i][3], c, k + 3); p.res = sptr<float>(*t[i][4], c, k + 4); p.add = sptr<float>(*t[i][5], c, k + 5);
+    p.col_limit = lim; p.col_limit_scale = (int32_t)q[14];
+    p.B = (int32_t)q[0]; p.Cin = (int32_t)q[1]; p.Cout = (int32_t)q[2]; p.L = (int32_t)q[3];
+    p.x_ld = (int32_t)q[4]; p.out_ld = (int32_t)q[5]; p.K = (int32_t)q[6]; p.dil = (int32_t)q[7]; p.nwg = (int32_t)q[8];
+    p.x_bstride = q[9]; p.out_bstride = q[10]; p.res_bstride = q[11]; p.add_bstride = q[12]; p.frags = (int32_t)q[13];
+    p.in_slope = (float)fp[3 * i]; p.scale = (float)fp[3 * i + 1]; p.out_slope = (float)fp[3 * i + 2];
+  }
+  DeviceScope scope(c);
+  finish(ov_conv1d_wino_multi_f32(ps, (int)n, c.stream()), "ov_conv1d_wino_multi_f32");
+}
+
 }
 
 TORCH_LIBRARY(openvoice_amd, m) {
@@ -364,6 +391,10 @@
   m.def("conv1d_wino_f32(Tensor? x, Tensor? w, Tensor? bias, Tensor(a!)? out, Tensor? res, Tensor? add, Tensor(b!)? dbg, "
         "Tensor? col_limit, int[] ip, float[] fp) -> ()",
         &conv1d_wino_f32);
+  m.def("conv1d_wino_multi_f32(Tensor? x0, Tensor? w0, Tensor? b0, Tensor(a!)? o0, Tensor? r0, Tensor? a0, Tensor? x1, Tensor? w1, "
+        "Tensor? b1, Tensor(b!)? o1, Tensor? r1, Tensor? a1, Tensor? x2, Tensor? w2, Tensor? b2, Tensor(c!)? o2, Tensor? r2, "
+        "Tensor? a2, Tensor? col_limit, int n, int[] ip, float[] fp) -> ()",
+        &conv1d_wino_multi_f32);
   bind_device<&ov_frame_hops_f32>(m, "frame_hops_f32");
   bind_device<&ov_frame_hops_windows_f32>(m, "frame_hops_windows_f32");
   bind_device<&ov_frame_hops_multi_f32>(m, "frame_hops_multi_f32");
diff --git a/openvoice_amd/engine.py b/openvoice_amd/engine.py
--- a/openvoice_amd/engine.py
+++ b/openvoice_amd/engine.py
@@ -219,6 +219,8 @@
 
 WINO_MIN_ITEMS = 136
 
+USE_MULTI_LAUNCH = True
+
 SPLIT_MIN_CHANNELS = 128
 
 
@@ -372,6 +374,10 @@
             full = torch.cat([forder + 2 * hidden * i for i in range(n_layers)])
             self.cond_w_fused = wc[full].contiguous().to(device)
             self.cond_b_fused = bc[full].contiguous().to(device)
+
+
+def multi_launch_scratch_buffers(cfg):
+    return 2 * (len(cfg["resblock_kernel_sizes"]) - 1)
 
 
 _DEC_BUFFERS = 5
@@ -475,6 +481,8 @@
         self.wn_row_split = 0
         self.fuse_pairs = True
         self.use_winograd = True
+        self.use_multi_launch = USE_MULTI_LAUNCH
+        self._cus = None
         self._state_dict_for_bf16 = sd
         self.generator_bf16 = None
         self._bf16_on = False
@@ -507,6 +515,12 @@
         alg = 2.0 * layer.cout * layer.cin * layer.K * L * B
         self._timed("mrf", alg, lambda: wino.launch_conv_wino(layer, x, bs, out, bs, B, L, **kw),
                     alg * wino.PRODUCTS_PER_TILE[layer.K] / (4.0 * layer.K))
+
+    def _wino_multi(self, convs, B, L, **lim):
+        from . import wino
+        alg = [2.0 * c["layer"].cout * c["layer"].cin * c["layer"].K * L * B for c in convs]
+        exe = sum(a * wino.PRODUCTS_PER_TILE[c["layer"].K] / (4.0 * c["layer"].K) for a, c in zip(alg, convs))
+        self._timed("mrf", sum(alg), lambda: wino.launch_convs_wino(convs, B, L, **lim), exe)
 
     def _pair(self, c1, c2, x, out, bs, B, L, add, scale, **lim):
         self._timed("mrf", 2 * 2.0 * c1.rows * c1.cin * c1.K * L * B,
@@ -541,12 +555,13 @@
             ws["pre"] = f(B, self.stages[0].cin, Tp)
             dec = _workspace_elems(self.cfg, B, T)[1]
             ws["dec"] = [torch.empty(dec, dtype=torch.float32, device=dev) for _ in range(_DEC_BUFFERS)]
+            self._chain_scratch(ws, self._multi_launch_scratch(B, T))
             self._ws[key] = ws
         return ws
 
     def workspace_bytes(self, B, T):
         frame_rate, dec = _workspace_elems(self.cfg, B, T)
-        return 4 * (frame_rate + _DEC_BUFFERS * dec)
+        return 4 * (frame_rate + (_DEC_BUFFERS + self._multi_launch_scratch(B, T)) * dec)
 
     def _zeros_like_cached(self, t):
         key = tuple(t.shape)
@@ -814,6 +829,8 @@
                                    add=add, add_bs=bs, scale=scale, tag="mrf", **lim(rate))
                 cur = dst
 
+        if not concurrent and self._mrf_multi(i, u, t1, ra, acc, ws, B, ch, L, lim(rate)):
+            return
         if not concurrent:
             for j, pairs in enumerate(self.resblocks[i]):
                 chain(j, pairs)
@@ -831,6 +848,51 @@
                     done[j].record(side[j])
             for j in range(nk):
                 main.wait_event(done[j])
+
+    def _multi_launch_stage(self, i, B, ch, L):
+        blocks = self.resblocks[i]
+        nk = len(blocks)
+        ks = [pairs[0][0].K for pairs in blocks]
+        dils = [[c1.dil for c1, _ in pairs] for pairs in blocks]
+        if not (self.use_multi_launch and self.use_winograd and 2 <= nk <= 3 and len(set(ks)) == nk and set(ks) <= {3, 7, 11}
+                and ch % 64 == 0 and all(d == dils[0] for d in dils)):
+            return False
+        if self._cus is None:
+            self._cus = torch.cuda.get_device_properties(self.device).multi_processor_count
+        if wino_items(ch, 1, B, L) <= self._cus:
+            return False
+        fams = [resblock_families(ch, k, d, B, L, self.use_winograd, self.fuse_pairs) for k, d in zip(ks, dils)]
+        return all(f == ("wino", "wino") for fam in fams for f in fam)
+
+    def _multi_launch_scratch(self, B, T):
+        return (multi_launch_scratch_buffers(self.cfg)
+                if any(self._multi_launch_stage(st.index, B, st.ch, T * st.rate_out) for st in self.stages) else 0)
+
+    def _mrf_multi(self, i, u, t1, ra, acc, ws, B, ch, L, lim):
+        cfg = self.cfg
+        blocks, wn = self.resblocks[i], self.wino_resblocks[i]
+        nk = len(blocks)
+        dils = [[c1.dil for c1, _ in pairs] for pairs in blocks]
+        if not self._multi_launch_stage(i, B, ch, L):
+            return False
+        need = multi_launch_scratch_buffers(cfg)
+        if torch.cuda.is_current_stream_capturing() and len(ws.get("dec_extra", [])) < need:
+            return False
+        extra = self._chain_scratch(ws, need)
+        ts, ras = [t1] + extra[0:need:2], [ra] + extra[1:need:2]
+        bs, npairs = ch * L, len(dils[0])
+        cur = [u] * nk
+        for n in range(npairs):
+            self._wino_multi([dict(layer=wn[j][n][0], x=cur[j], out=ts[j], bs=bs, in_slope=LRELU_SLOPE, out_slope=LRELU_SLOPE)
+                              for j in range(nk)], B, L, **lim)
+            if n < npairs - 1:
+                self._wino_multi([dict(layer=wn[j][n][1], x=ts[j], out=ras[j], bs=bs, res=cur[j]) for j in range(nk)], B, L, **lim)
+                cur = list(ras)
+            else:
+                for j in range(nk):
+                    self._wino(wn[j][n][1], ts[j], acc, bs, B, L, res=cur[j], add=acc if j > 0 else None,
+                               scale=1.0 / nk if j == nk - 1 else 1.0, in_slope=1.0, **lim)
+        return True
 
     def _stage(self, st, x, x_ld, x_bs, bufs, out, ws, B, L, cond_d=None, limits=None, keep=None):
         lim = lambda scale: dict(col_limit=limits, col_limit_scale=scale) if limits is not None else {}
diff --git a/openvoice_amd/wino.py b/openvoice_amd/wino.py
--- a/openvoice_amd/wino.py
+++ b/openvoice_amd/wino.py
@@ -53,3 +53,30 @@
     p.col_limit, p.col_limit_scale = vp(col_limit), col_limit_scale
     stream = ctypes.c_void_p(torch.cuda.current_stream(x.device).cuda_stream)
     _lib.check(_lib.load().ov_conv1d_wino_f32(ctypes.byref(p), stream), "ov_conv1d_wino_f32")
+
+
+def launch_convs_wino(convs, B, L, nwg=0, col_limit=None, col_limit_scale=1):
+    n = len(convs)
+    get = lambda c, k, d=None: c.get(k, d)
+    ints = lambda c: [B, c["layer"].cin, c["layer"].cout, L, 0, 0, c["layer"].K, c["layer"].dil, nwg, c["bs"], c["bs"],
+                      c["bs"] if get(c, "res") is not None else 0, c["bs"] if get(c, "add") is not None else 0, 0, col_limit_scale]
+    floats = lambda c: [get(c, "in_slope", 1.0), get(c, "scale", 1.0), get(c, "out_slope", 1.0)]
+    if _lib.use_torch_binding():
+        tensors = []
+        for i in range(3):
+            c = convs[i] if i < n else None
+            tensors += [None] * 6 if c is None else [c["x"], c["layer"].w, c["layer"].bias, c["out"], get(c, "res"), get(c, "add")]
+        _lib.torch_op("conv1d_wino_multi_f32", *tensors, col_limit, n, [v for c in convs for v in ints(c)],
+                      [v for c in convs for v in floats(c)])
+        return
+    ps = (_lib.ConvWinoParams * n)()
+    vp = lambda t: ctypes.c_void_p(t.data_ptr()) if t is not None else None
+    for p, c in zip(ps, convs):
+        layer = c["layer"]
+        p.x, p.w, p.bias, p.out, p.res, p.add = vp(c["x"]), vp(layer.w), vp(layer.bias), vp(c["out"]), vp(get(c, "res")), vp(get(c, "add"))
+        (p.B, p.Cin, p.Cout, p.L, p.x_ld, p.out_ld, p.K, p.dil, p.nwg, p.x_bstride, p.out_bstride, p.res_bstride, p.add_bstride,
+         p.frags, p.col_limit_scale) = ints(c)
+        p.in_slope, p.scale, p.out_slope = floats(c)
+        p.col_limit = vp(col_limit)
+    stream = ctypes.c_void_p(torch.cuda.current_stream(convs[0]["x"].device).cuda_stream)
+    _lib.check(_lib.load().ov_conv1d_wino_multi_f32(ps, n, stream), "ov_conv1d_wino_multi_f32")
```

After: 3157 x real-time (audio s / wall s), median of 6. 1.7% higher.
